# rogerhh/gaussian-splatting-lm

Hardware: AMD Instinct MI355X
Metric: CG matvecs/sec + raster Mpix/s, 1M Gaussians @1080p, 1/2/4/8 GPU (higher is better)
Workload: dtype f32; 1 GPU; LM CG iteration, 1000000 Gaussians SH3, 1x1920x1080 view(s) per GPU (BASELINE configs[2]; configs[3] at 8 GPUs); P=1000000, sh_degree=3, width=1920, height=1080, views_total=1, parallelism=views sharded x1, exchange=none, sh_rest_projected=True

## Files before the change

### gaussian-splatting-lm_amd/csrc/api.hip

```cpp
#include <cstring>
#include <string>
#include "gslm_kernels.hpp"

namespace gslm {

static thread_local std::string g_last_error;
void set_error(const std::string& msg) { g_last_error = msg; }

thread_local DebugSync g_debug;

int launch_failed(hipError_t e, const char* file, int line) {
  const char* base = std::strrchr(file, '/');
  set_error(std::string(g_debug.on ? "kernel failed (debug mode: stream synchronised after the launch at " : "kernel launch (") +
            (base ? base + 1 : file) + ":" + std::to_string(line) + "): " + hipGetErrorString(e));
  return GSLM_ERR_HIP;
}

namespace {

struct Carver {
  char* base;
  size_t off = 0;
  template <typename T>
  T* take(size_t count) {
// ... 600 lines not shown
  if (st) return st;
  if ((st = make_gauss(gi, &b->v, &b->g, false))) return st;
  if (scratch_bytes < gslm_scratch_bytes(b->g.P, N)) {
    set_error("scratch workspace too small");
    return GSLM_ERR_CAPACITY;
  }
  geom_layout(b->g.P, const_cast<void*>(geom), &b->gb);
  bin_layout(N, b->v.gx * b->v.gy, const_cast<void*>(binning), &b->bb);
  img_layout(b->v.H, b->v.W, const_cast<void*>(image), &b->ib);
  scratch_layout(b->g.P, N, scratch, &b->sb);
  return GSLM_OK;
}

int gslm_backward(const gslm_view* view, const gslm_gaussians* gi, const void* geom, const void* binning, int64_t N,
                  const void* image, const float* dL_dcolor, const float* dL_dinvdepth, void* scratch,
                  size_t scratch_bytes, const gslm_grads* out, void* stream) {
  DebugScope dbg_scope(view != nullptr && view->debug != 0, stream);
  Bound b;
  int st = bind_all(view, gi, geom, binning, N, image, scratch, scratch_bytes, &b);
  if (st) return st;
  if (!out || !dL_dcolor) { set_error("backward: NULL dL_dcolor or outputs"); return GSLM_ERR_INVALID; }
  hipStream_t s = (hipStream_t)stream;
  if ((st = launch_render_bwd(b.v, b.gb, b.bb, b.ib, N, dL_dcolor, dL_dinvdepth, b.sb, s))) return st;
  return launch_preprocess_bwd(b.v, b.g, b.gb, b.bb, b.sb, make_gradk(out), true, s);
}

int gslm_jvp(const gslm_view* view, const gslm_gaussians* gi, const gslm_gaussians* tangent,
             const float* means2D_tangent, const void* geom, const void* binning, int64_t N, const void* image,
             void* scratch, size_t scratch_bytes, float* out_color_t, float* out_invdepth_t, void* stream) {
  DebugScope dbg_scope(view != nullptr && view->debug != 0, stream);
  Bound b;
  int st = bind_all(view, gi, geom, binning, N, image, scratch, scratch_bytes, &b);
  if (st) return st;
  if (!out_color_t) { set_error("jvp: NULL out_color_t"); return GSLM_ERR_INVALID; }
  GaussK t;
  if ((st = make_gauss(tangent, &b.v, &t, true))) return st;
  t.P = b.g.P;
  t.raw = b.g.raw;
  t.M = b.g.M;
  return launch_jvp(b.v, b.g, t, means2D_tangent, b.gb, b.bb, b.ib, b.sb, out_color_t, out_invdepth_t,
                    (hipStream_t)stream);
}

static int build_xpby(const gslm_matvec_opts* opts, const gslm_grads* vin, int R, bool mask_xyz, XpbyK* out) {
  const gslm_grads* sv = opts->xpby_s;
  if (!opts->beta_num || !opts->beta_den) {
    set_error("matvec: xpby needs the TANGENT stage and beta_num / beta_den");
    return GSLM_ERR_INVALID;
  }
  if (vin->sh_dc_stride != 3 || sv->sh_dc_stride != 3 || (R > 0 && (vin->sh_rest_stride != R || sv->sh_rest_stride != R))) {
    set_error("matvec: xpby needs contiguous SH groups (dc stride 3, rest stride 3(M-1), or 3 projected)");
    return GSLM_ERR_INVALID;
  }
  XpbyK xp{};
  float* pp[6] = {vin->means3D, vin->sh_dc, vin->sh_rest, vin->scales, vin->rotations, vin->opacities};
  const float* ss[6] = {sv->means3D, sv->sh_dc, sv->sh_rest, sv->scales, sv->rotations, sv->opacities};
  const int ww[6] = {3, 3, R, 3, 4, 1};
  for (int k = 0; k < 6; ++k) {
    if ((pp[k] == nullptr) != (ss[k] == nullptr) || (ww[k] == 0 && pp[k])) {
      set_error("matvec: xpby groups of v and s must match");
      return GSLM_ERR_INVALID;
    }
    xp.p[k] = (ww[k] && !(k == 0 && mask_xyz)) ? pp[k] : nullptr;
    xp.s[k] = ss[k];
    xp.w[k] = ww[k];
  }
  xp.num = opts->beta_num;
  xp.den = opts->beta_den;
  xp.tail_p = opts->xpby_tail_n > 0 ? opts->xpby_tail_v : nullptr;
  xp.tail_s = opts->xpby_tail_s;
  xp.tail_n = opts->xpby_tail_n;
  if (xp.tail_p && !xp.tail_s) { set_error("matvec: xpby tail without s"); return GSLM_ERR_INVALID; }
  xp.anum = opts->alpha_num;
  xp.aden = opts->alpha_den;
  xp.xoff = opts->xpby_x_offset / (int64_t)sizeof(float);
  if (xp.anum && (!xp.aden || opts->xpby_x_offset % (int64_t)sizeof(float) != 0)) {
    set_error("matvec: deferred x update needs alpha_den and a float-aligned xpby_x_offset");
    return GSLM_ERR_INVALID;
  }
  *out = xp;
  return GSLM_OK;
}

static int matvec_view(const gslm_view* view, const gslm_gaussians* gi, const gslm_grads* vin,
                       const float* pixel_weight, int32_t mask_xyz, const void* geom, const void* binning,
                       int64_t N, const void* image, void* scratch, size_t scratch_bytes, const gslm_grads* y,
                       const gslm_matvec_opts* opts, const int32_t* ids, int64_t na, const uint32_t* hrow,
                       void* stream) {
  DebugScope dbg_scope(view != nullptr && view->debug != 0, stream);
  Bound b;
  int st = bind_all(view, gi, geom, binning, N, image, scratch, scratch_bytes, &b);
  if (st) return st;
  if (!vin || !y || !pixel_weight) { set_error("matvec: NULL argument"); return GSLM_ERR_INVALID; }
  const int32_t stages = (opts && opts->stages) ? opts->stages : GSLM_STAGE_ALL;
  const double* damp7 = opts ? opts->damp7 : nullptr;
  double* dot_out = opts ? opts->dot_vy : nullptr;
  const bool active = na >= 0;
  const int64_t rows = active ? na : b.g.P;
  if (active) {
    if (na > b.g.P || (na > 0 && (!ids || !hrow))) {
      set_error("matvec_view_active: 0 <= n_active <= P, a non-NULL list and its row offsets");
      return GSLM_ERR_INVALID;
    }
    if (!mask_xyz || !opts || !(opts->flags & GSLM_MV_TAIL_CLEAN) || (stages & GSLM_STAGE_SCREEN) || opts->trec_in) {
      set_error("matvec_view_active: needs mask_xyz and GSLM_MV_TAIL_CLEAN (the list comes from that row map); "
                "no SCREEN stage, no trec_in");
      return GSLM_ERR_INVALID;
    }
  }
  if (dot_out && (!opts->dot_scratch || opts->dot_scratch_bytes < gslm_dot_scratch_bytes(rows))) {
    set_error("matvec: dot scratch too small");
    return GSLM_ERR_CAPACITY;
  }
  if (!b.g.raw) { set_error("matvec: gaussians must be the raw GaussianModel leaves (raw = 1)"); return GSLM_ERR_INVALID; }
  hipStream_t s = (hipStream_t)stream;
  b.v.stop = opts ? opts->cg_ctl : nullptr;
  if (opts && opts->rest_basis) {
    set_error("matvec: rest_basis is an option of gslm_tangent_views / gslm_gather_screen");
    return GSLM_ERR_INVALID;
  }
  const bool proj = opts && (opts->flags & GSLM_MV_SH_REST_PROJECTED) && b.g.M > 1;
  GaussK t = tangent_from_grads(vin, b.g, mask_xyz != 0);
  if (proj) {
    if (vin->sh_rest && vin->sh_rest_stride != 3) {
      set_error("matvec: a projected SH-rest group has 3 floats per Gaussian (sh_rest_stride 3)");
      return GSLM_ERR_INVALID;
    }
    if (stages & GSLM_STAGE_SCREEN) {
      set_error("matvec: GSLM_MV_SH_REST_PROJECTED is a single-view mode (no SCREEN stage)");
      return GSLM_ERR_INVALID;
    }
    t.rest_proj = 1;
  }
  XpbyK xp{};
  const bool fused_xpby = opts && opts->xpby_s;
  if (fused_xpby) {
    if (!(stages & GSLM_STAGE_TANGENT)) {
      set_error("matvec: xpby needs the TANGENT stage and beta_num / beta_den");
      return GSLM_ERR_INVALID;
    }
    if ((st = build_xpby(opts, vin, proj ? 3 : 3 * (b.g.M - 1), mask_xyz != 0, &xp))) return st;
  }
  if (opts && opts->trec_in) {
    if (stages & GSLM_STAGE_TANGENT) {
      set_error("matvec: trec_in replaces the TANGENT stage");
      return GSLM_ERR_INVALID;
    }
    b.sb.trec = reinterpret_cast<float4*>(const_cast<float*>(opts->trec_in));
  }
  const float* seed = opts ? opts->pixel_seed : nullptr;
  if (seed && (!mask_xyz || fused_xpby || (stages & (GSLM_STAGE_TANGENT | GSLM_STAGE_SCREEN)))) {
    set_error("matvec: pixel_seed (J^T seed) needs mask_xyz and excludes TANGENT / SCREEN / xpby");
    return GSLM_ERR_INVALID;
  }
  if ((stages & GSLM_STAGE_TANGENT) &&
      (st = launch_tangent_pre(b.v, b.g, t, nullptr, b.gb, b.sb, fused_xpby ? &xp : nullptr, s, mask_xyz != 0, ids,
                               na)))
    return st;
  float* jv_out = opts ? opts->jv_out : nullptr;
  if (jv_out) {
    if (seed || (stages & (GSLM_STAGE_GATHER | GSLM_STAGE_SCREEN))) {
      set_error("matvec: jv_out excludes pixel_seed, GATHER and SCREEN");
      return GSLM_ERR_INVALID;
    }
    if (stages & GSLM_STAGE_RENDER) {
      if (N == 0) {
        GSLM_HIP_CHECK(hipMemsetAsync(jv_out, 0, (size_t)3 * b.v.H * b.v.W * sizeof(float), s));
      } else if ((st = launch_render_jv(b.v, t, b.gb, b.bb, b.ib, b.sb, mask_xyz != 0, jv_out, s))) {
        return st;
      }
    }
    return GSLM_OK;
  }
  if (seed) {
    if ((stages & GSLM_STAGE_RENDER) &&
        (st = launch_render_vjp_lm(b.v, b.gb, b.bb, b.ib, N, seed, b.sb, opts->flags & GSLM_MV_TAIL_CLEAN, s)))
      return st;
  } else if ((stages & GSLM_STAGE_RENDER) && N > 0 &&
      (st = launch_matvec_render(b.v, t, b.gb, b.bb, b.ib, b.sb, N, pixel_weight, mask_xyz != 0,
                                 opts && (opts->flags & GSLM_MV_TAIL_CLEAN), s)))
    return st;
  if (stages & GSLM_STAGE_SCREEN) {
    if (!mask_xyz || !opts->screen_out) {
      set_error("matvec: GSLM_STAGE_SCREEN needs mask_xyz and opts->screen_out");
      return GSLM_ERR_INVALID;
    }
    return launch_rowsum_screen(b.g, b.gb, b.sb, opts->screen_out, s);
  }
  if (!(stages & GSLM_STAGE_GATHER)) return GSLM_OK;
  double* part = dot_out ? (double*)opts->dot_scratch : nullptr;
  if ((st = launch_gather_lm(b.v, b.g, b.gb, b.sb, make_gradk(y), make_gradk(vin), damp7,
                             (stages & GSLM_STAGE_OVERWRITE) != 0, mask_xyz != 0, part, s, proj, ids, na, hrow)))
    return st;
  if (dot_out) return gslm_dot_finalize(part, (int32_t)((rows + 255) / 256), dot_out, stream);
  return GSLM_OK;
}

int gslm_matvec_view_ex(const gslm_view* view, const gslm_gaussians* gi, const gslm_grads* vin,
                        const float* pixel_weight, int32_t mask_xyz, const void* geom, const void* binning,
                        int64_t N, const void* image, void* scratch, size_t scratch_bytes, const gslm_grads* y,
                        const gslm_matvec_opts* opts, void* stream) {
  return matvec_view(view, gi, vin, pixel_weight, mask_xyz, geom, binning, N, image, scratch, scratch_bytes, y, opts,
                     nullptr, -1, nullptr, stream);
}

int gslm_matvec_view_active(const gslm_view* view, const gslm_gaussians* gi, const gslm_grads* vin,
                            const float* pixel_weight, int32_t mask_xyz, const void* geom, const void* binning,
                            int64_t N, const void* image, void* scratch, size_t scratch_bytes, const gslm_grads* y,
                            const gslm_matvec_opts* opts, const int32_t* active_ids, const uint32_t* active_rows,
                            int64_t n_active, void* stream) {
  if (n_active < 0) { set_error("matvec_view_active: negative n_active"); return GSLM_ERR_INVALID; }
  return matvec_view(view, gi, vin, pixel_weight, mask_xyz, geom, binning, N, image, scratch, scratch_bytes, y, opts,
                     active_ids, n_active, active_rows, stream);
}

static size_t active_work_layout(int64_t P, void* base, uint32_t** flags, uint32_t** tmp, uint32_t** total) {
  Carver c{(char*)base};
  uint32_t* f = c.take<uint32_t>(P > 0 ? P : 1);
  uint32_t* t = c.take<uint32_t>(scan_tmp_bytes(P > 0 ? P : 1) / 4);
  uint32_t* n = c.take<uint32_t>(4);
  if (flags) { *flags = f; *tmp = t; *total = n; }
  return c.off;
}

size_t gslm_active_list_bytes(int64_t P) { return active_work_layout(P, nullptr, nullptr, nullptr, nullptr); }

int gslm_active_list(const void* geom, int64_t P, int64_t N, const void* scratch, size_t scratch_bytes, void* work,
                     size_t work_bytes, int32_t* ids_dev, uint32_t* rows_dev, int64_t* count_dev, void* stream) {
  if (P < 0 || N < 0 || !geom || !scratch || !work || !count_dev || !rows_dev || (P > 0 && !ids_dev)) {
    set_error("active_list: NULL workspace / output or negative size");
    return GSLM_ERR_INVALID;
  }
  if (scratch_bytes < gslm_scratch_bytes(P, N) || work_bytes < gslm_active_list_bytes(P)) {
    set_error("active_list: scratch or work workspace too small");
    return GSLM_ERR_CAPACITY;
  }
  GeomBufs gb;
  ScratchBufs sb;
  geom_layout(P, const_cast<void*>(geom), &gb);
  scratch_layout(P, N, const_cast<void*>(scratch), &sb);
  uint32_t *flags, *tmp, *total;
  active_work_layout(P, work, &flags, &tmp, &total);
  return launch_active_list(P, N, gb, sb, flags, tmp, total, ids_dev, rows_dev, count_dev, (hipStream_t)stream);
}

int gslm_inspect_rowmap(const void* geom, int64_t P, int64_t N, const void* scratch, size_t scratch_bytes,
                        uint32_t* goff, uint32_t* hscan, void* stream) {
  if (P < 0 || N < 0 || !geom || !scratch) { set_error("inspect_rowmap: NULL workspace or negative size"); return GSLM_ERR_INVALID; }
  if (scratch_bytes < gslm_scratch_bytes(P, N)) { set_error("inspect_rowmap: scratch workspace too small"); return GSLM_ERR_CAPACITY; }
  GeomBufs gb;
  ScratchBufs sb;
  geom_layout(P, const_cast<void*>(geom), &gb);
  scratch_layout(P, N, const_cast<void*>(scratch), &sb);
  hipStream_t s = (hipStream_t)stream;
  if (goff && P > 0) GSLM_HIP_CHECK(hipMemcpyAsync(goff, gb.goff, (size_t)P * 4, hipMemcpyDeviceToDevice, s));
  if (hscan) GSLM_HIP_CHECK(hipMemcpyAsync(hscan, sb.hscan, (size_t)(N + 1) * 4, hipMemcpyDeviceToDevice, s));
  return GSLM_OK;
}

int gslm_active_pack(const float* src, float* dst, const int32_t* active_ids, int64_t n_active, int64_t P,
                     const int32_t* widths, int32_t ngroups, int64_t tail_n, void* stream) {
  return launch_active_pack(true, src, dst, active_ids, n_active, P, widths, ngroups, tail_n, (hipStream_t)stream);
}

int gslm_active_unpack(const float* src, float* dst, const int32_t* active_ids, int64_t n_active, int64_t P,
                       const int32_t* widths, int32_t ngroups, int64_t tail_n, void* stream) {
  return launch_active_pack(false, src, dst, active_ids, n_active, P, widths, ngroups, tail_n, (hipStream_t)stream);
}

int gslm_sh_rest_project(const gslm_view* view, const gslm_gaussians* gi, int32_t mode, const float* in,
                         int64_t in_stride, float* out, int64_t out_stride, void* stream) {
  ViewK v;
  GaussK g;
  int st;
  if (!view || !gi) { set_error("sh_rest_project: NULL view / gaussians"); return GSLM_ERR_INVALID; }
  if ((st = make_view(view, gi->max_coeffs, &v))) return st;
  if ((st = make_gauss(gi, &v, &g, false))) return st;
  if (mode != 0 && mode != 1) { set_error("sh_rest_project: mode must be 0 (expand) or 1 (project)"); return GSLM_ERR_INVALID; }
  if (g.P > 0 && g.M > 1 && (!in || !out || !g.means3D)) { set_error("sh_rest_project: NULL buffer"); return GSLM_ERR_INVALID; }
  const int64_t full = 3 * (int64_t)(g.M - 1);
  if ((mode == 0 && (in_stride < 3 || out_stride < full)) || (mode == 1 && (in_stride < full || out_stride < 3))) {
    set_error("sh_rest_project: strides too small for [P,3] / [P,M-1,3] rows");
    return GSLM_ERR_INVALID;
  }
  return launch_sh_rest_project(v, g, mode, in, in_stride, out, out_stride, (hipStream_t)stream);
}

static int rest_views(const char* who, const gslm_view* views, int32_t nviews, const gslm_gaussians* gi, ViewK* vk,
                      GaussK* g) {
  if (!views || !gi || nviews < 1 || nviews > GSLM_MAX_REST_VIEWS) {
    set_error(std::string(who) + ": NULL views / gaussians or nviews outside 1..GSLM_MAX_REST_VIEWS");
    return GSLM_ERR_INVALID;
  }
  int st;
  for (int b = 0; b < nviews; ++b) {
    if ((st = make_view(&views[b], gi->max_coeffs, &vk[b]))) return st;
// ... 219 lines not shown
```

### gaussian-splatting-lm_amd/csrc/cg.hip

```cpp
#include "gslm_internal.hpp"

namespace gslm {

constexpr int MAXG = 8;
struct Groups {
  int64_t bound[MAXG + 1];
  double damp[MAXG];
  int n;
};

constexpr int DOT_THREADS = 256;
constexpr int DOT_BLOCKS = 1024;

__device__ __forceinline__ double group_w(const Groups& g, int64_t i) {
  double w = 1.0;
  if (g.n > 0) {
    w = 0.0;
#pragma unroll
    for (int k = 0; k < MAXG; ++k)
      if (k < g.n && i >= g.bound[k] && i < g.bound[k + 1]) w = g.damp[k];
  }
  return w;
}

__device__ __forceinline__ double block_sum_d(double x, double* s) {
  const int tid = threadIdx.x, lane = tid & 63, w = tid >> 6;
#pragma unroll
  for (int o = 32; o > 0; o >>= 1) x += __shfl_down(x, o, 64);
  if (lane == 0) s[w] = x;
  __syncthreads();
  double t = 0.0;
  if (tid == 0)
    for (int k = 0; k < DOT_THREADS / 64; ++k) t += s[k];
  return t;
}

__global__ __launch_bounds__(DOT_THREADS) void k_dot_partial(const float* __restrict__ a, const float* __restrict__ b,
                                                             Groups g, int64_t n, double* __restrict__ part) {
  __shared__ double s[DOT_THREADS / 64];
  double acc = 0.0;
  const int64_t stride = (int64_t)gridDim.x * DOT_THREADS;
  if (g.n == 0) {
    for (int64_t i = (int64_t)blockIdx.x * DOT_THREADS + threadIdx.x; i < n; i += stride)
      acc += (double)a[i] * (double)b[i];
  } else {
    for (int k = 0; k < g.n; ++k) {
      double gacc = 0.0;
      const int64_t lo = g.bound[k], hi = min(g.bound[k + 1], n);
      for (int64_t i = lo + (int64_t)blockIdx.x * DOT_THREADS + threadIdx.x; i < hi; i += stride)
        gacc += (double)a[i] * (double)b[i];
      acc += g.damp[k] * gacc;
    }
  }
  const double t = block_sum_d(acc, s);
  if (threadIdx.x == 0) part[blockIdx.x] = t;
}

__global__ __launch_bounds__(DOT_THREADS) void k_dot_final(const double* __restrict__ part, int np,
                                                           double* __restrict__ out) {
  __shared__ double s[DOT_THREADS / 64];
  const double acc = strided_sum_in_order(part, np);
  const double t = block_sum_d(acc, s);
  if (threadIdx.x == 0) *out = t;
}

__global__ __launch_bounds__(DOT_THREADS) void k_dot_final3(const double* __restrict__ part, int np,
                                                            double* __restrict__ o0, double* __restrict__ o1,
                                                            double* __restrict__ o2) {
  __shared__ double s[DOT_THREADS / 64];
  const int b = blockIdx.x;
  const double acc = strided_sum_in_order(part + (int64_t)b * np, np);
  const double t = block_sum_d(acc, s);
  if (threadIdx.x == 0) *(b == 0 ? o0 : (b == 1 ? o1 : o2)) = t;
}

__global__ __launch_bounds__(256) void k_axpy_dev(int64_t n, const double* __restrict__ num,
                                                  const double* __restrict__ den, float sign,
                                                  const float* __restrict__ x, float* __restrict__ y) {
  const double a = den ? (*num) / (*den) : (*num);
  const float af = (float)(a * (double)sign);
  const int64_t stride = (int64_t)gridDim.x * blockDim.x;
  for (int64_t i = (int64_t)blockIdx.x * blockDim.x + threadIdx.x; i < n; i += stride) y[i] = y[i] + af * x[i];
}

__global__ __launch_bounds__(256) void k_xpby_dev(int64_t n, const float* __restrict__ s, const double* __restrict__ num,
                                                  const double* __restrict__ den, float* __restrict__ p) {
  const float b = (float)((*num) / (*den));
  const int64_t stride = (int64_t)gridDim.x * blockDim.x;
  for (int64_t i = (int64_t)blockIdx.x * blockDim.x + threadIdx.x; i < n; i += stride) p[i] = s[i] + b * p[i];
}

template <bool MONITOR>
__global__ __launch_bounds__(DOT_THREADS) void k_cg_update(int64_t n, const double* __restrict__ gam,
                                                           const double* __restrict__ del,
                                                           const float* __restrict__ p, const float* __restrict__ q,
                                                           float* __restrict__ x, float* __restrict__ s,
                                                           const float* __restrict__ g, double* __restrict__ part,
                                                           const double* __restrict__ ctl) {
  __shared__ double sm[DOT_THREADS / 64];
  if (ctl && (ctl[0] != 0.0 || *del < 1e-20 || !isfinite(*del))) return;
  const float a = (float)((*gam) / (*del));
  double acc = 0.0, axg = 0.0, axs = 0.0;
  const int64_t n4 = n / 4;
  const int64_t stride = (int64_t)gridDim.x * DOT_THREADS;
  const float4* p4 = reinterpret_cast<const float4*>(p);
  const float4* q4 = reinterpret_cast<const float4*>(q);
  const float4* g4 = reinterpret_cast<const float4*>(g);
  float4* x4 = reinterpret_cast<float4*>(x);
  float4* s4 = reinterpret_cast<float4*>(s);
  const bool do_x = x != nullptr;
  for (int64_t i = (int64_t)blockIdx.x * DOT_THREADS + threadIdx.x; i < n4; i += stride) {
    const float4 qv = q4[i];
    float4 xv = make_float4(0.f, 0.f, 0.f, 0.f), sv = s4[i];
    float4 gv;
    if (MONITOR) gv = g4[i];
    if (do_x) {
      const float4 pv = p4[i];
      xv = x4[i];
      xv.x += a * pv.x; xv.y += a * pv.y; xv.z += a * pv.z; xv.w += a * pv.w;
      x4[i] = xv;
    }
    sv.x -= a * qv.x; sv.y -= a * qv.y; sv.z -= a * qv.z; sv.w -= a * qv.w;
    s4[i] = sv;
    acc += (double)sv.x * sv.x + (double)sv.y * sv.y + (double)sv.z * sv.z + (double)sv.w * sv.w;
    if (MONITOR) {
      axg += (double)xv.x * gv.x + (double)xv.y * gv.y + (double)xv.z * gv.z + (double)xv.w * gv.w;
      axs += (double)xv.x * sv.x + (double)xv.y * sv.y + (double)xv.z * sv.z + (double)xv.w * sv.w;
    }
  }
  for (int64_t i = 4 * n4 + (int64_t)blockIdx.x * DOT_THREADS + threadIdx.x; i < n; i += stride) {
    float xv = 0.f;
    if (do_x) {
      xv = x[i] + a * p[i];
      x[i] = xv;
    }
    const float sv = s[i] - a * q[i];
    s[i] = sv;
    acc += (double)sv * sv;
    if (MONITOR) {
      axg += (double)xv * g[i];
      axs += (double)xv * sv;
    }
  }
  const double t = block_sum_d(acc, sm);
  if (threadIdx.x == 0) part[blockIdx.x] = t;
  if (MONITOR) {
    __syncthreads();
    const double t1 = block_sum_d(axg, sm);
    if (threadIdx.x == 0) part[gridDim.x + blockIdx.x] = t1;
    __syncthreads();
    const double t2 = block_sum_d(axs, sm);
    if (threadIdx.x == 0) part[2 * gridDim.x + blockIdx.x] = t2;
  }
}

__global__ void k_cg_monitor(const double* __restrict__ gam, const double* __restrict__ gamn,
                             const double* __restrict__ del, const double* __restrict__ xg,
                             const double* __restrict__ xs, const double* __restrict__ b2, double tol, double atol,
                             double* __restrict__ ctl, int max_hist) {
  if (threadIdx.x != 0 || ctl[0] != 0.0) return;
  if (!(isfinite(*gam) && isfinite(*del))) {
    ctl[0] = 4.0;
    return;
  }
  if (*del < 1e-20) {
    ctl[0] = 1.0;
    return;
  }
  if (!(isfinite(*gamn) && isfinite(*xg) && isfinite(*xs))) {
    ctl[0] = 4.0;
    return;
  }
  const double res = (*b2 - *xg) - *xs;
  const int nh = (int)ctl[3];
  if (nh < max_hist) ctl[4 + nh] = res;
  ctl[3] = (double)(nh + 1);
  if (res > ctl[2]) {
    ctl[0] = 2.0;
    return;
  }
  ctl[2] = res;
  if (*gamn < fmax(tol * sqrt(*gam), atol)) {
    ctl[0] = 3.0;
    return;
  }
  ctl[1] += 1.0;
}

__global__ __launch_bounds__(256) void k_damp_add(int64_t n, const float* __restrict__ x, Groups g,
                                                  float* __restrict__ y) {
  const int64_t stride = (int64_t)gridDim.x * blockDim.x;
  for (int64_t i = (int64_t)blockIdx.x * blockDim.x + threadIdx.x; i < n; i += stride)
    y[i] = y[i] + (float)group_w(g, i) * x[i];
}

static int make_groups(const int64_t* bounds, const double* damp, int ng, Groups* g) {
  if (ng < 0 || ng > MAXG) {
    set_error("at most 8 damping groups");
    return GSLM_ERR_INVALID;
  }
  g->n = ng;
  for (int k = 0; k <= MAXG; ++k) g->bound[k] = (k <= ng && bounds) ? bounds[k] : 0;
  for (int k = 0; k < MAXG; ++k) g->damp[k] = (k < ng && damp) ? damp[k] : 0.0;
  return GSLM_OK;
}

static unsigned grid_for(int64_t n) {
  int64_t b = (n + 255) / 256;
  if (b > 4096) b = 4096;
  if (b < 1) b = 1;
  return (unsigned)b;
}

}

using namespace gslm;

extern "C" {

size_t gslm_dot_scratch_bytes(int64_t n) {
  const int64_t per_block = (n + 255) / 256 + 16;
  return (size_t)(per_block > DOT_BLOCKS ? per_block : DOT_BLOCKS) * sizeof(double);
}

int gslm_cg_update(int64_t n, const double* gam_dev, const double* del_dev, const float* p, const float* q, float* x,
                   float* s, void* scratch, double* gam_new_dev, void* stream) {
  if ((reinterpret_cast<uintptr_t>(p) | reinterpret_cast<uintptr_t>(q) | reinterpret_cast<uintptr_t>(x) |
       reinterpret_cast<uintptr_t>(s)) & 15) {
    set_error("gslm_cg_update: vectors must be 16-byte aligned");
    return GSLM_ERR_INVALID;
  }
  hipStream_t st = (hipStream_t)stream;
  hipLaunchKernelGGL(k_cg_update<false>, dim3(DOT_BLOCKS), dim3(DOT_THREADS), 0, st, n, gam_dev, del_dev, p, q, x, s,
                     nullptr, (double*)scratch, (const double*)nullptr);
  hipLaunchKernelGGL(k_dot_final, dim3(1), dim3(DOT_THREADS), 0, st, (const double*)scratch, DOT_BLOCKS, gam_new_dev);
  GSLM_LAUNCH_CHECK();
  return GSLM_OK;
}

int gslm_cg_update_monitor(int64_t n, const double* gam_dev, const double* del_dev, const float* p, const float* q,
                           float* x, float* s, const float* g, void* scratch, size_t scratch_bytes,
                           double* gam_new_dev, double* xg_dev, double* xs_dev, const double* cg_ctl, void* stream) {
  if ((reinterpret_cast<uintptr_t>(p) | reinterpret_cast<uintptr_t>(q) | reinterpret_cast<uintptr_t>(x) |
       reinterpret_cast<uintptr_t>(s) | reinterpret_cast<uintptr_t>(g)) & 15) {
    set_error("gslm_cg_update_monitor: vectors must be 16-byte aligned");
    return GSLM_ERR_INVALID;
  }
  if (scratch_bytes < (size_t)3 * DOT_BLOCKS * sizeof(double)) {
    set_error("gslm_cg_update_monitor: scratch < 3 * 1024 doubles");
    return GSLM_ERR_CAPACITY;
  }
  hipStream_t st = (hipStream_t)stream;
  const double* part = (const double*)scratch;
  hipLaunchKernelGGL(k_cg_update<true>, dim3(DOT_BLOCKS), dim3(DOT_THREADS), 0, st, n, gam_dev, del_dev, p, q, x, s, g,
                     (double*)scratch, cg_ctl);
  hipLaunchKernelGGL(k_dot_final3, dim3(3), dim3(DOT_THREADS), 0, st, part, DOT_BLOCKS, gam_new_dev, xg_dev, xs_dev);
  GSLM_LAUNCH_CHECK();
  return GSLM_OK;
}

int gslm_cg_monitor(const double* gam_dev, const double* gam_new_dev, const double* del_dev, const double* xg_dev,
                    const double* xs_dev, const double* b2_dev, double tol, double atol, double* cg_ctl,
                    int32_t max_hist, void* stream) {
  if (!gam_dev || !gam_new_dev || !del_dev || !xg_dev || !xs_dev || !b2_dev || !cg_ctl || max_hist < 0) {
    set_error("gslm_cg_monitor: NULL scalar / control block or negative max_hist");
    return GSLM_ERR_INVALID;
  }
  hipLaunchKernelGGL(k_cg_monitor, dim3(1), dim3(64), 0, (hipStream_t)stream, gam_dev, gam_new_dev, del_dev, xg_dev,
                     xs_dev, b2_dev, tol, atol, cg_ctl, max_hist);
  GSLM_LAUNCH_CHECK();
  return GSLM_OK;
}

int gslm_dot_finalize(const void* partials, int32_t np, double* out_dev, void* stream) {
  hipLaunchKernelGGL(k_dot_final, dim3(1), dim3(DOT_THREADS), 0, (hipStream_t)stream, (const double*)partials, np,
                     out_dev);
  GSLM_LAUNCH_CHECK();
  return GSLM_OK;
}

int gslm_dot(const float* a, const float* b, const int64_t* group_bounds, const double* group_damp, int32_t ngroups,
             int64_t n, void* scratch, double* out_dev, void* stream) {
  Groups g;
  int st = make_groups(group_bounds, group_damp, ngroups, &g);
  if (st) return st;
  hipStream_t s = (hipStream_t)stream;
  hipLaunchKernelGGL(k_dot_partial, dim3(DOT_BLOCKS), dim3(DOT_THREADS), 0, s, a, b, g, n, (double*)scratch);
  hipLaunchKernelGGL(k_dot_final, dim3(1), dim3(DOT_THREADS), 0, s, (const double*)scratch, DOT_BLOCKS, out_dev);
  GSLM_LAUNCH_CHECK();
  return GSLM_OK;
}

int gslm_axpy_dev(int64_t n, const double* num_dev, const double* den_dev, float sign, const float* x, float* y,
                  void* stream) {
  if (n <= 0) return GSLM_OK;
  hipLaunchKernelGGL(k_axpy_dev, dim3(grid_for(n)), dim3(256), 0, (hipStream_t)stream, n, num_dev, den_dev, sign, x, y);
  GSLM_LAUNCH_CHECK();
  return GSLM_OK;
}

int gslm_xpby_dev(int64_t n, const float* s_, const double* num_dev, const double* den_dev, float* p, void* stream) {
  if (n <= 0) return GSLM_OK;
  hipLaunchKernelGGL(k_xpby_dev, dim3(grid_for(n)), dim3(256), 0, (hipStream_t)stream, n, s_, num_dev, den_dev, p);
  GSLM_LAUNCH_CHECK();
  return GSLM_OK;
}

int gslm_damp_add(int64_t n, const float* x, const int64_t* group_bounds, const double* group_damp, int32_t ngroups,
                  float* y, void* stream) {
  Groups g;
  int st = make_groups(group_bounds, group_damp, ngroups, &g);
  if (st) return st;
  if (n <= 0) return GSLM_OK;
  hipLaunchKernelGGL(k_damp_add, dim3(grid_for(n)), dim3(256), 0, (hipStream_t)stream, n, x, g, y);
  GSLM_LAUNCH_CHECK();
  return GSLM_OK;
}

}
```

### gaussian-splatting-lm_amd/csrc/gather.hip

```cpp
#include "gslm_tile.hpp"
#include "gslm_chain.hpp"
#include "gslm_gather.hpp"

namespace gslm {

template <int ROWF4>
__device__ __forceinline__ void sum_rows(const float4* __restrict__ rows, uint32_t off, uint32_t n, float G2[NV]) {
#pragma unroll
  for (int q = 0; q < NV; ++q) G2[q] = 0.f;
  for (uint32_t t = 0; t < n; ++t) {
    float r[NV];
    load_row<ROWF4>(rows, (size_t)off + t, r);
#pragma unroll
    for (int q = 0; q < NV; ++q) G2[q] += r[q];
  }
}

template <bool RAW>
__global__ __launch_bounds__(256) void k_preprocess_bwd(ViewK v, GaussK g, const uint32_t* __restrict__ clampw,
                                                         const uint32_t* __restrict__ tiles,
                                                         const uint32_t* __restrict__ goff,
                                                         const float4* __restrict__ rows, GradK out, int want_means) {
  extern __shared__ __attribute__((aligned(16))) float s_buf[];
  const int tid = threadIdx.x;
  const int64_t i0 = (int64_t)blockIdx.x * blockDim.x;
  const int64_t i = i0 + tid;
  const int64_t nvalid = min((int64_t)blockDim.x, g.P - i0);
  const uint32_t n = i < g.P ? tiles[i] : 0u;
  float G2[NV];
  {
    const int64_t il = i0 + nvalid - 1;
    const uint32_t R0 = goff[i0], R1 = goff[il] + tiles[il];
    block_sum_rows<3>(rows, R0, R1, i < g.P ? goff[i] : R1, n, reinterpret_cast<float4*>(s_buf), G2);
  }
  const int nc = (v.D + 1) * (v.D + 1);
  const bool sh_out = !g.colors && (out.dc || out.rest);
  const bool dir_term = want_means && out.means3D && !g.colors && v.D > 0;
  ChainOut co;
  if (i < g.P) {
    chain_vjp<RAW, true>(v, g, i, n != 0, n ? clampw[i] : 0u, G2, want_means != 0, co);
    write_grads(g, out, i, co, v.M, nc, want_means != 0 && !dir_term, true);
  }
  if (!sh_out && !dir_term) return;
  float* s_d = s_buf + 256 * SHB_STRIDE;
  float* s_w = s_d + 256 * 4;
  if (i < g.P) {
#pragma unroll
    for (int k = 0; k < 16; ++k) s_buf[tid * SHB_STRIDE + k] = co.shB[k];
#pragma unroll
    for (int ch = 0; ch < 3; ++ch) s_d[tid * 4 + ch] = co.dres[ch];
  }
  __syncthreads();
  if (dir_term) {
    for (int e = tid; e < (int)nvalid * 16; e += blockDim.x) {
      const int ii = e >> 4, k = e & 15;
      float w = 0.f;
      if (k >= 1 && k < nc) {
        const int64_t gi = i0 + ii;
        const float s0 = g.sh(gi, k, 0), s1 = g.sh(gi, k, 1), s2 = g.sh(gi, k, 2);
        w = s_d[ii * 4 + 0] * s0 + s_d[ii * 4 + 1] * s1 + s_d[ii * 4 + 2] * s2;
      }
      s_w[ii * SHB_STRIDE + k] = w;
    }
    __syncthreads();
    if (i < g.P && n != 0) {
      float dm[3] = {co.dmean[0], co.dmean[1], co.dmean[2]};
      add_dir_term(v.D, co.dir, co.dirlen, s_w + tid * SHB_STRIDE, dm);
#pragma unroll
      for (int k = 0; k < 3; ++k) put(&out.means3D[3 * i + k], dm[k], out.accumulate);
    } else if (i < g.P) {
#pragma unroll
      for (int k = 0; k < 3; ++k) put(&out.means3D[3 * i + k], co.dmean[k], out.accumulate);
    }
  }
  if (!sh_out) return;
  const int acc = out.accumulate;
  const int R = 3 * v.M;
  const float invR = 1.0f / (float)R;
  for (int e = tid; e < (int)nvalid * R; e += blockDim.x) {
    const int ii = (int)(((float)e + 0.5f) * invR);
    const int r = e - ii * R, k = r / 3, ch = r - 3 * k;
    const float val = k < nc ? s_buf[ii * SHB_STRIDE + k] * s_d[ii * 4 + ch] : 0.f;
    const int64_t gi = i0 + ii;
    if (k == 0) {
      if (out.dc) put(&out.dc[gi * out.dc_stride + ch], val, acc);
    } else if (out.rest) {
      put(&out.rest[gi * out.rest_stride + 3 * (k - 1) + ch], val, acc);
    }
  }
}

template <bool WANT_MEANS, int ROWF4, bool PROJ, bool ACTIVE = false>
__global__ __launch_bounds__(256, PROJ ? 5 : 1) void k_gather_lm(ViewK v, GaussK g, const uint32_t* __restrict__ clampw,
                                                    const uint32_t* __restrict__ tiles,
                                                    const uint32_t* __restrict__ goff,
                                                    const uint32_t* __restrict__ hscan,
                                                    const float4* __restrict__ rows, FlatK o,
                                                    const int32_t* __restrict__ ids, int64_t na,
                                                    const uint32_t* __restrict__ hrow) {
  o.rest_proj = PROJ ? 1 : 0;
  if (cg_stopped(v)) return;
  extern __shared__ __attribute__((aligned(16))) float s_rest[];
  __shared__ double s_dot[4];
  const int tid = threadIdx.x;
  const int64_t j0 = (int64_t)blockIdx.x * blockDim.x;
  const int64_t j = j0 + tid;
  const int64_t nrows = ACTIVE ? na : g.P;
  const int64_t nvalid = min((int64_t)blockDim.x, nrows - j0);
  const bool valid = j < nrows;
  const int64_t i = ACTIVE ? (valid ? (int64_t)ids[j] : 0) : j;
  const uint32_t n = ACTIVE ? (valid ? 1u : 0u) : (valid ? tiles[i] : 0u);
  float G2[NV];
  if (ACTIVE) {
    const uint32_t R0 = hrow[j0], R1 = hrow[j0 + nvalid];
    const uint32_t h0 = valid ? hrow[j] : R1, h1 = valid ? hrow[j + 1] : R1;
    block_sum_rows<ROWF4>(rows, R0, R1, h0, h1 - h0, reinterpret_cast<float4*>(s_rest), G2);
  } else {
    const int64_t il = j0 + nvalid - 1;
    const uint32_t R0 = hscan[goff[j0]], R1 = hscan[goff[il] + tiles[il]];
    const uint32_t h0 = valid ? hscan[goff[i]] : R1, h1 = valid ? hscan[goff[i] + n] : R1;
    block_sum_rows<ROWF4>(rows, R0, R1, h0, h1 - h0, reinterpret_cast<float4*>(s_rest), G2);
  }
  ChainOut co;
  if (valid) chain_vjp<true>(v, g, i, n != 0, n ? clampw[i] : 0u, G2, WANT_MEANS, co);
  if (ACTIVE) g.P = na;
  lm_epilogue<WANT_MEANS, true>((v.D + 1) * (v.D + 1), g, co, o, s_rest, s_dot);
}

__global__ __launch_bounds__(256) void k_sh_rest_project(ViewK v, GaussK g, int mode, const float* __restrict__ in,
                                                         int64_t in_stride, float* __restrict__ out,
                                                         int64_t out_stride) {
  extern __shared__ __attribute__((aligned(16))) float s_rows[];
  const int R = 3 * (g.M - 1);
  const int64_t i0 = (int64_t)blockIdx.x * blockDim.x;
  const int64_t nv = min((int64_t)blockDim.x, g.P - i0);
  const int64_t i = i0 + threadIdx.x;
  if (mode == 1) {
    for (int64_t e = threadIdx.x; e < nv * R; e += blockDim.x) {
      const int64_t ii = e / R, r = e - ii * R;
      s_rows[e] = in[(i0 + ii) * in_stride + r];
    }
    __syncthreads();
  }
  if (i < g.P) {
    const float x = g.means3D[3 * i + 0], y = g.means3D[3 * i + 1], z = g.means3D[3 * i + 2];
    const float dx = x - v.campos[0], dy = y - v.campos[1], dz = z - v.campos[2];
    const float len = sqrtf((dx * dx + dy * dy) + dz * dz);
    float B[16];
    sh_basis(v.D, dx / len, dy / len, dz / len, B);
    const int nc = (v.D + 1) * (v.D + 1);
    const float nb = sh_rest_norm(B, nc);
    const float inv = nb > 0.f ? 1.f / nb : 0.f;
    float* row = s_rows + (int64_t)threadIdx.x * R;
    if (mode == 0) {
      for (int k = 1; k < g.M; ++k)
#pragma unroll
        for (int c = 0; c < 3; ++c) row[3 * (k - 1) + c] = k < nc ? (B[k] * inv) * in[i * in_stride + c] : 0.f;
    } else {
      float acc[3] = {0.f, 0.f, 0.f};
      for (int k = 1; k < g.M && k < nc; ++k)
#pragma unroll
        for (int c = 0; c < 3; ++c) acc[c] += (B[k] * inv) * row[3 * (k - 1) + c];
#pragma unroll
      for (int c = 0; c < 3; ++c) out[i * out_stride + c] = acc[c];
    }
  }
  if (mode == 0) {
    __syncthreads();
    for (int64_t e = threadIdx.x; e < nv * R; e += blockDim.x) {
      const int64_t ii = e / R, r = e - ii * R;
      out[(i0 + ii) * out_stride + r] = s_rows[e];
    }
  }
}

int launch_sh_rest_project(const ViewK& v, const GaussK& g, int mode, const float* in, int64_t in_stride, float* out,
                           int64_t out_stride, hipStream_t s) {
  if (g.P == 0 || g.M < 2) return GSLM_OK;
  const size_t lds = (size_t)256 * 3 * (g.M - 1) * sizeof(float);
  hipLaunchKernelGGL(k_sh_rest_project, dim3((unsigned)((g.P + 255) / 256)), dim3(256), lds, s, v, g, mode, in,
                     in_stride, out, out_stride);
  GSLM_LAUNCH_CHECK();
  return GSLM_OK;
}

int launch_preprocess_bwd(const ViewK& v, const GaussK& g, const GeomBufs& gb, const BinBufs& bb,
                          const ScratchBufs& sb, const GradK& out, bool want_means, hipStream_t s) {
  (void)bb;
  if (g.P == 0) return GSLM_OK;
  const unsigned nb = (unsigned)((g.P + 255) / 256);
  const size_t sh_lds = (sh_stage_floats<true>(g.M) + (size_t)256 * SHB_STRIDE) * sizeof(float);
  const size_t chunk_lds = (size_t)GATHER_CHUNK * 3 * sizeof(float4);
  const size_t lds = sh_lds > chunk_lds ? sh_lds : chunk_lds;
  if (g.raw)
    hipLaunchKernelGGL(k_preprocess_bwd<true>, dim3(nb), dim3(256), lds, s, v, g, gb.clampw, gb.tiles, gb.goff,
                       sb.contrib, out, want_means ? 1 : 0);
  else
    hipLaunchKernelGGL(k_preprocess_bwd<false>, dim3(nb), dim3(256), lds, s, v, g, gb.clampw, gb.tiles, gb.goff,
                       sb.contrib, out, want_means ? 1 : 0);
  GSLM_LAUNCH_CHECK();
  return GSLM_OK;
}

int launch_gather_lm(const ViewK& v, const GaussK& g, const GeomBufs& gb, const ScratchBufs& sb, const GradK& y,
                     const GradK& vin, const double* damp7, bool overwrite, bool mask_xyz, double* dot_part,
                     hipStream_t s, bool rest_proj, const int32_t* ids, int64_t na, const uint32_t* hrow) {
  const bool active = na >= 0;
  const int64_t nrows = active ? na : g.P;
  if (nrows == 0) return GSLM_OK;
  FlatK o;
  const int st = make_flatk(g, y, vin, damp7, overwrite, dot_part, &o, rest_proj);
  if (st) return st;
  if (active && (!mask_xyz || !ids || !hrow)) {
    set_error("internal: the active-list gather runs on the LM rows (mask_xyz)");
    return GSLM_ERR_INVALID;
  }
  const unsigned nb = (unsigned)((nrows + 255) / 256);
  const size_t rest_lds = sh_stage_floats<true>(g.M) * sizeof(float);
  const size_t chunk_lds = (size_t)GATHER_CHUNK * (mask_xyz ? 2 : 3) * sizeof(float4);
  const size_t lds = (rest_lds > chunk_lds ? rest_lds : chunk_lds) + 16;
  if (active && o.rest_proj)
    hipLaunchKernelGGL((k_gather_lm<false, 2, true, true>), dim3(nb), dim3(256), lds, s, v, g, gb.clampw, gb.tiles,
                       gb.goff, sb.hscan, sb.contrib, o, ids, na, hrow);
  else if (active)
    hipLaunchKernelGGL((k_gather_lm<false, 2, false, true>), dim3(nb), dim3(256), lds, s, v, g, gb.clampw, gb.tiles,
                       gb.goff, sb.hscan, sb.contrib, o, ids, na, hrow);
  else if (mask_xyz && o.rest_proj)
    hipLaunchKernelGGL((k_gather_lm<false, 2, true>), dim3(nb), dim3(256), lds, s, v, g, gb.clampw, gb.tiles, gb.goff,
                       sb.hscan, sb.contrib, o, nullptr, -1, nullptr);
  else if (mask_xyz)
    hipLaunchKernelGGL((k_gather_lm<false, 2, false>), dim3(nb), dim3(256), lds, s, v, g, gb.clampw, gb.tiles, gb.goff,
                       sb.hscan, sb.contrib, o, nullptr, -1, nullptr);
  else if (o.rest_proj)
    hipLaunchKernelGGL((k_gather_lm<true, 3, true>), dim3(nb), dim3(256), lds, s, v, g, gb.clampw, gb.tiles, gb.goff,
                       sb.hscan, sb.contrib, o, nullptr, -1, nullptr);
  else
    hipLaunchKernelGGL((k_gather_lm<true, 3, false>), dim3(nb), dim3(256), lds, s, v, g, gb.clampw, gb.tiles, gb.goff,
                       sb.hscan, sb.contrib, o, nullptr, -1, nullptr);
  GSLM_LAUNCH_CHECK();
  return GSLM_OK;
}

struct PackK {
  int w[8];
  int64_t poff[8];
  int64_t aoff[8];
  int n;
  int wsum;
};
template <bool TO_ACTIVE>
__global__ __launch_bounds__(256) void k_active_pack(PackK k, const int32_t* __restrict__ ids, int64_t na,
                                                      const float* __restrict__ src, float* __restrict__ dst) {
  const int64_t e = (int64_t)blockIdx.x * blockDim.x + threadIdx.x;
  if (e >= na * k.wsum) return;
  const int64_t j = e / k.wsum;
  int c = (int)(e - j * k.wsum), grp = 0;
  while (grp < k.n - 1 && c >= k.w[grp]) c -= k.w[grp++];
  const int64_t full = k.poff[grp] + (int64_t)ids[j] * k.w[grp] + c;
  const int64_t act = k.aoff[grp] + j * k.w[grp] + c;
  if (TO_ACTIVE) dst[act] = src[full];
  else dst[full] = src[act];
}

int launch_active_pack(bool to_active, const float* src, float* dst, const int32_t* ids, int64_t na, int64_t P,
                       const int32_t* widths, int ngroups, int64_t tail_n, hipStream_t s) {
  if (ngroups < 1 || ngroups > 8 || !widths || na < 0 || na > P || tail_n < 0 || !src || !dst || (na > 0 && !ids)) {
    set_error("active pack: 1..8 groups, 0 <= n_active <= P, non-NULL buffers");
    return GSLM_ERR_INVALID;
  }
  PackK k{};
  int64_t po = 0, ao = 0;
  for (int q = 0; q < ngroups; ++q) {
    if (widths[q] < 0) { set_error("active pack: negative group width"); return GSLM_ERR_INVALID; }
    k.w[q] = widths[q];
    k.poff[q] = po;
    k.aoff[q] = ao;
    po += P * widths[q];
    ao += na * widths[q];
    k.wsum += widths[q];
  }
  k.n = ngroups;
  const int64_t src_n = to_active ? po : ao, dst_n = to_active ? ao : po;
  if (!to_active) GSLM_HIP_CHECK(hipMemsetAsync(dst, 0, (size_t)dst_n * sizeof(float), s));
  if (tail_n > 0)
    GSLM_HIP_CHECK(hipMemcpyAsync(dst + dst_n, src + src_n, (size_t)tail_n * sizeof(float), hipMemcpyDeviceToDevice, s));
  const int64_t total = na * k.wsum;
  if (total == 0) return GSLM_OK;
  const unsigned nb = (unsigned)((total + 255) / 256);
  if (to_active) hipLaunchKernelGGL(k_active_pack<true>, dim3(nb), dim3(256), 0, s, k, ids, na, src, dst);
  else hipLaunchKernelGGL(k_active_pack<false>, dim3(nb), dim3(256), 0, s, k, ids, na, src, dst);
  GSLM_LAUNCH_CHECK();
  return GSLM_OK;
}

}
```

### gaussian-splatting-lm_amd/csrc/gslm_device.hpp

```cpp
#pragma once
#include <hip/hip_runtime.h>
#include <stdint.h>
#include "gslm.h"

#if defined(GSLM_EXPERIMENT_COUNT) || defined(GSLM_EXPERIMENT_TIMELINE) || defined(GSLM_EXPERIMENT_SKIP_JVP) || \
    defined(GSLM_EXPERIMENT_SKIP_VJP) || defined(GSLM_EXPERIMENT_NOSYNC)
#error "GSLM_EXPERIMENT_* flags are not part of the product build (libgslm.so)"
#endif

namespace gslm {

constexpr int TILE_X = 16;
constexpr int TILE_Y = 16;
constexpr int TILE_PIX = TILE_X * TILE_Y;
constexpr int REC_F4 = 3;
constexpr int RECS = 4;

__constant__ static const float SH_C0 = 0.28209479177387814f;
__constant__ static const float SH_C1 = 0.4886025119029199f;

struct f3 { float x, y, z; };
__device__ __forceinline__ f3 mk3(float x, float y, float z) { return {x, y, z}; }

struct ViewK {
  int H, W, gx, gy;
  float focal_x, focal_y, limx, limy;
  float view[16];
  float proj[16];
  float campos[3];
  float bg[3];
  float scale_mod;
  int D;
  int M;
  int antialiasing;
  int exhaustive;
  const double* stop = nullptr;
};

template <typename F>
__device__ __forceinline__ F strided_sum_in_order(const F* __restrict__ x, int64_t n) {
  F acc = F(0);
  const int64_t T = blockDim.x;
  for (int64_t i = threadIdx.x; i < n; i += 8 * T) {
    F v[8];
#pragma unroll
    for (int k = 0; k < 8; ++k) v[k] = i + k * T < n ? x[i + k * T] : F(0);
#pragma unroll
    for (int k = 0; k < 8; ++k)
      if (i + k * T < n) acc += v[k];
  }
  return acc;
}

__device__ __forceinline__ float clamp01(float x) { return x < 0.0f ? 0.0f : (x > 1.0f ? 1.0f : x); }

__device__ __forceinline__ bool cg_stopped(const ViewK& v) { return v.stop != nullptr && *v.stop != 0.0; }

__device__ __forceinline__ float tp_row(const float* m, float x, float y, float z, int r) {
  return ((x * m[r] + y * m[4 + r]) + z * m[8 + r]) + m[12 + r];
}

__device__ __forceinline__ void quat_rot(float r, float x, float y, float z, float R[9]) {
  R[0] = 1.f - 2.f * (y * y + z * z); R[1] = 2.f * (x * y - r * z); R[2] = 2.f * (x * z + r * y);
  R[3] = 2.f * (x * y + r * z); R[4] = 1.f - 2.f * (x * x + z * z); R[5] = 2.f * (y * z - r * x);
  R[6] = 2.f * (x * z - r * y); R[7] = 2.f * (y * z + r * x); R[8] = 1.f - 2.f * (x * x + y * y);
}

__device__ __forceinline__ void cov3d_from(float sx, float sy, float sz, const float R[9], float c[6]) {
  const float s[3] = {sx, sy, sz};
  float L[9];
#pragma unroll
  for (int i = 0; i < 3; ++i)
#pragma unroll
    for (int j = 0; j < 3; ++j) L[i * 3 + j] = R[i * 3 + j] * s[j];
  auto dotrow = [&](int a, int b) { return (L[a * 3 + 0] * L[b * 3 + 0] + L[a * 3 + 1] * L[b * 3 + 1]) + L[a * 3 + 2] * L[b * 3 + 2]; };
  c[0] = dotrow(0, 0); c[1] = dotrow(0, 1); c[2] = dotrow(0, 2);
  c[3] = dotrow(1, 1); c[4] = dotrow(1, 2); c[5] = dotrow(2, 2);
}

struct Proj2 {
  float A0[3], A1[3];
  float J00, J02, J11, J12;
  float tz, tcx, tcy;
  bool inx, iny;
};

__device__ __forceinline__ void ewa_jacobian(const ViewK& v, float tx, float ty, float tz, Proj2& p) {
  const float txtz = tx / tz, tytz = ty / tz;
  p.inx = (txtz >= -v.limx) && (txtz <= v.limx);
  p.iny = (tytz >= -v.limy) && (tytz <= v.limy);
  p.tcx = fminf(v.limx, fmaxf(-v.limx, txtz)) * tz;
  p.tcy = fminf(v.limy, fmaxf(-v.limy, tytz)) * tz;
  p.tz = tz;
  p.J00 = v.focal_x / tz;
  p.J02 = -(v.focal_x * p.tcx) / (tz * tz);
  p.J11 = v.focal_y / tz;
  p.J12 = -(v.focal_y * p.tcy) / (tz * tz);
#pragma unroll
  for (int k = 0; k < 3; ++k) {
    p.A0[k] = p.J00 * v.view[4 * k + 0] + p.J02 * v.view[4 * k + 2];
    p.A1[k] = p.J11 * v.view[4 * k + 1] + p.J12 * v.view[4 * k + 2];
  }
}

__device__ __forceinline__ float quad_form(const float a[3], const float c[6], const float b[3]) {
  const float S0[3] = {c[0], c[1], c[2]}, S1[3] = {c[1], c[3], c[4]}, S2[3] = {c[2], c[4], c[5]};
  const float r0 = (S0[0] * b[0] + S0[1] * b[1]) + S0[2] * b[2];
  const float r1 = (S1[0] * b[0] + S1[1] * b[1]) + S1[2] * b[2];
  const float r2 = (S2[0] * b[0] + S2[1] * b[1]) + S2[2] * b[2];
  return (a[0] * r0 + a[1] * r1) + a[2] * r2;
}

__device__ __forceinline__ void sh_basis(int D, float x, float y, float z, float B[16]) {
  B[0] = SH_C0;
  if (D > 0) { B[1] = -SH_C1 * y; B[2] = SH_C1 * z; B[3] = -SH_C1 * x; }
  if (D > 1) {
    const float xx = x * x, yy = y * y, zz = z * z, xy = x * y, yz = y * z, xz = x * z;
    B[4] = 1.0925484305920792f * xy;
    B[5] = -1.0925484305920792f * yz;
    B[6] = 0.31539156525252005f * (2.0f * zz - xx - yy);
    B[7] = -1.0925484305920792f * xz;
    B[8] = 0.5462742152960396f * (xx - yy);
    if (D > 2) {
      B[9] = -0.5900435899266435f * y * (3.0f * xx - yy);
      B[10] = 2.890611442640554f * xy * z;
      B[11] = -0.4570457994644658f * y * (4.0f * zz - xx - yy);
      B[12] = 0.3731763325901154f * z * (2.0f * zz - 3.0f * xx - 3.0f * yy);
      B[13] = -0.4570457994644658f * x * (4.0f * zz - xx - yy);
      B[14] = 1.445305721320277f * z * (xx - yy);
      B[15] = -0.5900435899266435f * x * (xx - 3.0f * yy);
    }
  }
}

// ... 74 lines not shown
```

### gaussian-splatting-lm_amd/csrc/gslm_internal.hpp

```cpp
#pragma once
#include <hip/hip_runtime.h>
#include <stdint.h>
#include <stddef.h>
#include <string>
#include "gslm.h"
#include "gslm_device.hpp"

namespace gslm {

void set_error(const std::string& msg);

#define GSLM_HIP_CHECK(expr)                                                                  \
  do {                                                                                        \
    hipError_t _e = (expr);                                                                   \
    if (_e != hipSuccess) {                                                                   \
      ::gslm::set_error(std::string(#expr) + ": " + hipGetErrorString(_e));                   \
      return GSLM_ERR_HIP;                                                                    \
    }                                                                                         \
  } while (0)

struct DebugSync {
  hipStream_t s = nullptr;
  bool on = false;
};
extern thread_local DebugSync g_debug;
struct DebugScope {
  DebugSync prev;
  DebugScope(bool on, void* stream) : prev(g_debug) {
    if (on) g_debug = DebugSync{(hipStream_t)stream, true};
  }
  ~DebugScope() { g_debug = prev; }
};
int launch_failed(hipError_t e, const char* file, int line);

#define GSLM_LAUNCH_CHECK()                                                                   \
  do {                                                                                        \
    hipError_t _e = hipGetLastError();                                                        \
    if (_e == hipSuccess && ::gslm::g_debug.on) _e = hipStreamSynchronize(::gslm::g_debug.s);  \
    if (_e != hipSuccess) return ::gslm::launch_failed(_e, __FILE__, __LINE__);               \
  } while (0)

inline size_t align_up(size_t x, size_t a = 256) { return (x + a - 1) / a * a; }

constexpr int SORT_THREADS = 256;
constexpr int SORT_ITEMS = 16;
constexpr int SORT_TILE = SORT_THREADS * SORT_ITEMS;
#ifndef GSLM_SORT_ITEMS_SMALL
#define GSLM_SORT_ITEMS_SMALL 8
#endif
constexpr int SORT_ITEMS_SMALL = GSLM_SORT_ITEMS_SMALL;
constexpr int64_t SORT_FULL_BLOCKS = 1024;
constexpr int RADIX = 256;

inline int sort_items(int64_t n, bool payload = false) {
  return !payload && (n + SORT_TILE - 1) / SORT_TILE >= SORT_FULL_BLOCKS ? SORT_ITEMS : SORT_ITEMS_SMALL;
}
inline int64_t sort_blocks(int64_t n, bool payload = false) {
  const int64_t t = (int64_t)SORT_THREADS * sort_items(n, payload);
  return (n + t - 1) / t;
}
inline size_t sort_hist_bytes(int64_t n, bool payload = false) {
  const size_t nb = (size_t)sort_blocks(n, payload);
  return (size_t)RADIX * nb * 4 + 4 * RADIX + 16 + 8 * nb;
}

int radix_sort_pairs(uint32_t* k0, uint32_t* v0, uint32_t* k1, uint32_t* v1, int64_t n, int end_bit,
                     uint32_t* hist, bool* result_in_alt, hipStream_t s, bool iota_values = false,
                     const uint32_t* last_gather = nullptr, const uint32_t* n_dev = nullptr, uint32_t* p0 = nullptr,
                     uint32_t* p1 = nullptr, bool key_range = false);

constexpr int SCAN_THREADS = 256;
#ifndef GSLM_SCAN_ITEMS
#define GSLM_SCAN_ITEMS 8
#endif
constexpr int SCAN_ITEMS = GSLM_SCAN_ITEMS;
constexpr int SCAN_TILE = SCAN_THREADS * SCAN_ITEMS;
inline int64_t scan_blocks(int64_t n) { return (n + SCAN_TILE - 1) / SCAN_TILE; }
#ifndef GSLM_SCAN_INLINE_MAX_BLOCKS
#define GSLM_SCAN_INLINE_MAX_BLOCKS 4096
#endif
constexpr int64_t SCAN_INLINE_MAX_BLOCKS = GSLM_SCAN_INLINE_MAX_BLOCKS;
inline size_t scan_tmp_bytes(int64_t n) { return align_up((size_t)scan_blocks(n) * 8 + 64); }
int exclusive_scan_u32(const uint32_t* in, const uint32_t* idx, uint32_t* out, int64_t n, uint32_t* tmp,
                       uint32_t* total, hipStream_t s, int64_t inline_max_blocks = SCAN_INLINE_MAX_BLOCKS);
int exclusive_scan_u32_dual(const uint32_t* in, const uint32_t* idx, uint32_t* out_a, uint32_t* out_b, int64_t n,
                            uint32_t* tmp, uint32_t* total_a, uint32_t* total_b, hipStream_t s,
                            const uint32_t* in_b = nullptr, int64_t inline_max_blocks = SCAN_INLINE_MAX_BLOCKS);

}
```

### gaussian-splatting-lm_amd/csrc/gslm_kernels.hpp

```cpp
#pragma once
#include "gslm_internal.hpp"

namespace gslm {

struct GaussK {
  int64_t P;
  int raw;
  int M;
  const float* means3D;
  const float* opac;
  const float* scales;
  const float* rot;
  const float* cov3D;
  const float* dc;
  int64_t dc_stride;
  const float* rest;
  int64_t rest_stride;
  const float* colors;
  int64_t rest_base = 0;
  int rest_proj = 0;
  const float* rest_R = nullptr;
  int rest_V = 0;
  int rest_col = 0;
  __device__ __forceinline__ float sh(int64_t i, int k, int c) const {
// ... 365 lines not shown
constexpr int MAX_PRE_VIEWS = 8;
struct PreOutBufs {
  float4* rec;
  uint32_t* depth_key;
  uint32_t* tiles;
  uint2* rect;
  uint32_t* clampw;
  const uint32_t* pos;
};
struct PreViewsK {
  ViewK v[MAX_PRE_VIEWS];
  PreOutBufs out[MAX_PRE_VIEWS];
  int n;
};
int launch_preprocess_views(const PreViewsK& pv, const GaussK& g, const GeomBufs* gbs, hipStream_t s);
int launch_binning(const ViewK& v, int64_t P, const GeomBufs& gb, const BinBufs& bb, int64_t N, hipStream_t s,
                   bool device_count = false, uint32_t* n_out = nullptr);
int launch_ranges(int64_t N, const uint32_t* keys_sorted, uint2* ranges, const uint32_t* n_dev, uint32_t* n_out,
                  hipStream_t s);
constexpr int TILE_ORDER_FLAT = 0, TILE_ORDER_XCD = 1;
int launch_tile_order_form(int form, int ntiles, const uint2* ranges, uint32_t* order, const uint32_t* cost,
                           hipStream_t s);
int launch_lm_rowmap(const ViewK& v, const GeomBufs& gb, const BinBufs& bb, const ImgBufs& ib, const ScratchBufs& sb,
                     int64_t N, hipStream_t s);
int launch_active_list(int64_t P, int64_t N, const GeomBufs& gb, const ScratchBufs& sb, uint32_t* flags,
                       uint32_t* scan_tmp, uint32_t* total, int32_t* ids, uint32_t* hrow, int64_t* count,
                       hipStream_t s);
int launch_point_ids(const uint32_t* point_list, int64_t N, uint32_t* out, hipStream_t s);
int launch_render_loss(const ViewK& v, const GeomBufs& gb, const BinBufs& bb, const float* gt, const float* mask,
                       double* part, double* loss, int accumulate, hipStream_t s, const uint32_t* amask = nullptr,
                       int shift = 0, const uint32_t* nsets = nullptr);
constexpr int MAX_UNION_SETS = 8;
struct UnionSets {
  const float4* rec[MAX_UNION_SETS];
  const uint32_t* tiles[MAX_UNION_SETS];
  const uint2* rect[MAX_UNION_SETS];
  int n;
};
struct UnionMasks {
  uint32_t* m0;
  uint32_t* m1;
  uint32_t* sorted;
  uint32_t* hist;
  uint32_t* nsets;
};
size_t union_masks_layout(int64_t N, int ntiles, void* binning, UnionMasks* out);
struct SetRecsK {
  const float4* rec[MAX_UNION_SETS];
};
struct LossPtrsK {
  double* loss[MAX_UNION_SETS];
};
int launch_render_loss_sets(const ViewK& v, const SetRecsK& sr, int nsets, const BinBufs& bb, const uint32_t* amask,
                            const float* gt, const float* mask, double* part, const LossPtrsK& lp, int accumulate,
                            hipStream_t s, int first_set = 0, const uint32_t* nsets_dev = nullptr);
int launch_union_rect(int64_t P, const UnionSets& u, const GeomBufs& ug, hipStream_t s);
int launch_depth_positions(int64_t P, const uint32_t* order, uint32_t* pos, hipStream_t s);
int launch_union_binning(const ViewK& v, int64_t P, const GeomBufs& ug, const BinBufs& bb, const UnionMasks& um,
                         int64_t N, const UnionSets& u, hipStream_t s);
int launch_render_fwd(const ViewK& v, const GeomBufs& gb, const BinBufs& bb, const ImgBufs& ib, float* out_color,
                      float* out_invdepth, hipStream_t s);

}

namespace gslm {
int launch_render_bwd(const ViewK& v, const GeomBufs& gb, const BinBufs& bb, const ImgBufs& ib, int64_t N,
                      const float* dL_dcolor, const float* dL_dinv, const ScratchBufs& sb, hipStream_t s);
int launch_render_vjp_lm(const ViewK& v, const GeomBufs& gb, const BinBufs& bb, const ImgBufs& ib, int64_t N,
                         const float* dL_dcolor, const ScratchBufs& sb, bool tail_clean, hipStream_t s);
int launch_preprocess_bwd(const ViewK& v, const GaussK& g, const GeomBufs& gb, const BinBufs& bb,
                          const ScratchBufs& sb, const GradK& out, bool want_means, hipStream_t s);
struct XpbyK {
  float* p[6];
  const float* s[6];
  int w[6];
  const double* num;
  const double* den;
  float* tail_p;
  const float* tail_s;
  int64_t tail_n;
  const double* anum;
  const double* aden;
  int64_t xoff;
};
int launch_tangent_pre(const ViewK& v, const GaussK& g, const GaussK& t, const float* m2t, const GeomBufs& gb,
                       const ScratchBufs& sb, const XpbyK* xp, hipStream_t s, bool compact,
                       const int32_t* ids = nullptr, int64_t na = -1);
int launch_rowsum_screen(const GaussK& g, const GeomBufs& gb, const ScratchBufs& sb, float* out, hipStream_t s);
constexpr int MAX_SCREEN_VIEWS = 16;
constexpr int MAX_REST_VIEWS = GSLM_MAX_REST_VIEWS;
__host__ __device__ constexpr int rest_basis_floats(int V) { return V * (V + 1) / 2; }
struct RestK {
  const float* R = nullptr;
  int V = 0;
  int view_base = 0;
};
struct ViewsK {
  ViewK v[MAX_SCREEN_VIEWS];
  int n;
};
int launch_gather_screen(const ViewK* views, int nviews, const GaussK& g, const float* screen, int64_t sstride,
                         const GradK& y, const GradK& vin, const double* damp7, bool overwrite, double* dot_part,
                         hipStream_t s, const RestK& rc = RestK{});
int launch_gather_views(const ViewK* views, const GeomBufs* gbs, const ScratchBufs* sbs, const int64_t* nr,
                        int nviews, const GaussK& g, const GradK& y, const GradK& vin, const double* damp7,
                        bool overwrite, double* dot_part, double* dot_out, hipStream_t s, const RestK& rc = RestK{});
int launch_rest_basis(const ViewK* views, int nviews, const GaussK& g, float* R, hipStream_t s);
int launch_rest_coords(const ViewK* views, int nviews, const GaussK& g, const float* R, int mode, const float* in,
                       int64_t in_stride, float* out, int64_t out_stride, hipStream_t s);
int launch_view_flags(int64_t P, const GeomBufs& gb, uint32_t* out, hipStream_t s);
int launch_tangent_views(const ViewK* views, int nviews, const GaussK& g, const GaussK& t, const uint32_t* vflags,
                         int64_t fstride, float* out, int64_t ostride, const XpbyK* xp, hipStream_t s, bool compact,
                         int view_base = 0);
int launch_jvp(const ViewK& v, const GaussK& g, const GaussK& t, const float* m2t, const GeomBufs& gb,
               const BinBufs& bb, const ImgBufs& ib, const ScratchBufs& sb, float* out_color_t, float* out_inv_t,
               hipStream_t s);
int launch_render_jv(const ViewK& v, const GaussK& t, const GeomBufs& gb, const BinBufs& bb, const ImgBufs& ib,
                     const ScratchBufs& sb, bool mask_xyz, float* jv_out, hipStream_t s);
int launch_matvec_render(const ViewK& v, const GaussK& t, const GeomBufs& gb, const BinBufs& bb, const ImgBufs& ib,
                         const ScratchBufs& sb, int64_t N, const float* weight, bool mask_xyz, bool tail_clean,
                         hipStream_t s);
int launch_gather_lm(const ViewK& v, const GaussK& g, const GeomBufs& gb, const ScratchBufs& sb, const GradK& y,
                     const GradK& vin, const double* damp7, bool overwrite, bool mask_xyz, double* dot_part,
                     hipStream_t s, bool rest_proj = false, const int32_t* ids = nullptr, int64_t na = -1,
                     const uint32_t* hrow = nullptr);
int launch_active_pack(bool to_active, const float* src, float* dst, const int32_t* ids, int64_t na, int64_t P,
                       const int32_t* widths, int ngroups, int64_t tail_n, hipStream_t s);
int launch_sh_rest_project(const ViewK& v, const GaussK& g, int mode, const float* in, int64_t in_stride, float* out,
                           int64_t out_stride, hipStream_t s);
}
```

### gaussian-splatting-lm_amd/csrc/tangent.hip

```cpp
#include "gslm_tile.hpp"
#include "gslm_chain.hpp"

namespace gslm {

__device__ __forceinline__ void block_xpby(const XpbyK& xp, int64_t P, float* s_rest) {
  const float b = (float)((*xp.num) / (*xp.den));
  const bool with_x = xp.anum != nullptr;
  const float a = with_x ? (float)((*xp.anum) / (*xp.aden)) : 0.f;
  const int64_t i0 = (int64_t)blockIdx.x * blockDim.x;
  const int64_t nv = min((int64_t)blockDim.x, P - i0);
  const int tid = threadIdx.x;
  constexpr int MAXW[6] = {3, 3, 3, 3, 4, 1};
  const bool rest_narrow = xp.w[2] <= 3;
  float sv[17], pv[17], xv[17];
  int n = 0;
#pragma unroll
  for (int k = 0; k < 6; ++k) {
#pragma unroll
    for (int j = 0; j < MAXW[k]; ++j, ++n) {
      const int64_t e = (int64_t)j * blockDim.x + tid;
      const bool on = xp.p[k] && (k != 2 || rest_narrow) && e < nv * xp.w[k];
      const int64_t gi = i0 * xp.w[k] + e;
      sv[n] = on ? xp.s[k][gi] : 0.f;
      pv[n] = on ? xp.p[k][gi] : 0.f;
      xv[n] = (on && with_x) ? xp.p[k][xp.xoff + gi] : 0.f;
    }
  }
  n = 0;
#pragma unroll
  for (int k = 0; k < 6; ++k) {
#pragma unroll
    for (int j = 0; j < MAXW[k]; ++j, ++n) {
      const int64_t e = (int64_t)j * blockDim.x + tid;
      const bool on = xp.p[k] && (k != 2 || rest_narrow) && e < nv * xp.w[k];
      if (on) {
        const int64_t gi = i0 * xp.w[k] + e;
        if (with_x) xp.p[k][xp.xoff + gi] = xv[n] + a * pv[n];
        const float r = sv[n] + b * pv[n];
        xp.p[k][gi] = r;
        if (k == 2) s_rest[e] = r;
      }
    }
  }
  if (xp.p[2] && !rest_narrow) {
    float* p = xp.p[2] + i0 * xp.w[2];
    const float* s = xp.s[2] + i0 * xp.w[2];
    const int64_t len = nv * xp.w[2];
    constexpr int U = 8;
    for (int64_t e0 = 0; e0 < len; e0 += (int64_t)U * blockDim.x) {
      float su[U], pu[U], xu[U];
#pragma unroll
      for (int u = 0; u < U; ++u) {
        const int64_t e = e0 + (int64_t)u * blockDim.x + tid;
        su[u] = e < len ? s[e] : 0.f;
        pu[u] = e < len ? p[e] : 0.f;
        xu[u] = (e < len && with_x) ? p[xp.xoff + e] : 0.f;
      }
#pragma unroll
      for (int u = 0; u < U; ++u) {
        const int64_t e = e0 + (int64_t)u * blockDim.x + tid;
        if (e < len) {
          if (with_x) p[xp.xoff + e] = xu[u] + a * pu[u];
          const float r = su[u] + b * pu[u];
          p[e] = r;
          s_rest[e] = r;
        }
      }
    }
  }
  if (blockIdx.x == 0 && xp.tail_p)
    for (int64_t e = threadIdx.x; e < xp.tail_n; e += blockDim.x) {
      const float pvt = xp.tail_p[e];
      if (with_x) xp.tail_p[xp.xoff + e] = xp.tail_p[xp.xoff + e] + a * pvt;
      xp.tail_p[e] = xp.tail_s[e] + b * pvt;
    }
}

__device__ __forceinline__ void store_trec(float4* __restrict__ out, int64_t i, const float T2[10], bool compact) {
  if (compact) {
    out[2 * i + 0] = make_float4(T2[2], T2[3], T2[4], T2[5]);
    out[2 * i + 1] = make_float4(T2[6], T2[7], T2[8], 0.f);
  } else {
    out[3 * i + 0] = make_float4(T2[0], T2[1], T2[2], T2[3]);
    out[3 * i + 1] = make_float4(T2[4], T2[5], T2[6], T2[7]);
    out[3 * i + 2] = make_float4(T2[8], T2[9], 0.f, 0.f);
  }
}

template <bool RAW, bool XPBY, bool ACTIVE = false>
__global__ __launch_bounds__(256) void k_preprocess_jvp(ViewK v, GaussK g, GaussK t, const float* __restrict__ m2t,
                                                         const uint32_t* __restrict__ clampw,
                                                         const uint32_t* __restrict__ tiles,
                                                         float4* __restrict__ trec, XpbyK xp, int compact,
                                                         int lead, const int32_t* __restrict__ ids, int64_t na) {
  extern __shared__ __attribute__((aligned(16))) float s_rest[];
  if (cg_stopped(v)) return;
  const int64_t j = (int64_t)blockIdx.x * blockDim.x + threadIdx.x;
  const int64_t n = ACTIVE ? na : g.P;
  if (!XPBY && !ACTIVE && lead >= 0) {
    stage_sh_rows(g, lead, s_rest);
  }
  if (XPBY) {
    block_xpby(xp, n, s_rest);
    __syncthreads();
    if (t.rest) {
      t.rest = s_rest;
      t.rest_base = (int64_t)blockIdx.x * blockDim.x;
    }
  }
  if (j >= n) return;
  const int64_t i = ACTIVE ? (int64_t)ids[j] : j;
  if (!ACTIVE && tiles[i] == 0) return;
  float T2[10];
  chain_jvp<RAW>(v, g, t, m2t, i, j, clampw[i], T2);
  store_trec(trec, i, T2, compact != 0);
}

int launch_tangent_pre(const ViewK& v, const GaussK& g, const GaussK& t, const float* m2t, const GeomBufs& gb,
                       const ScratchBufs& sb, const XpbyK* xp, hipStream_t s, bool compact, const int32_t* ids,
                       int64_t na) {
  const bool active = na >= 0;
  const int64_t n = active ? na : g.P;
  if (n == 0 && !(xp && xp->tail_p)) return GSLM_OK;
  const unsigned nb = (unsigned)((n + 255) / 256) + (n == 0 ? 1u : 0u);
  XpbyK none{};
  const XpbyK& x = xp ? *xp : none;
  if (active && (!g.raw || m2t || (na > 0 && !ids))) {
    set_error("internal: the active-list tangent runs on raw leaves without a means2D tangent");
    return GSLM_ERR_INVALID;
  }
  if (xp) {
    if (t.rest && (t.rest != xp->p[2] || t.rest_stride != xp->w[2])) {
      set_error("internal: fused xpby expects the tangent's SH-rest group to be p's");
      return GSLM_ERR_INVALID;
    }
    const size_t lds = (size_t)256 * xp->w[2] * sizeof(float);
    if (active)
      hipLaunchKernelGGL((k_preprocess_jvp<true, true, true>), dim3(nb), dim3(256), lds, s, v, g, t, m2t, gb.clampw,
                         gb.tiles, sb.trec, x, compact ? 1 : 0, -1, ids, na);
    else if (g.raw)
      hipLaunchKernelGGL((k_preprocess_jvp<true, true>), dim3(nb), dim3(256), lds, s, v, g, t, m2t, gb.clampw, gb.tiles,
                         sb.trec, x, compact ? 1 : 0, -1, nullptr, -1);
    else
      hipLaunchKernelGGL((k_preprocess_jvp<false, true>), dim3(nb), dim3(256), lds, s, v, g, t, m2t, gb.clampw, gb.tiles,
                         sb.trec, x, compact ? 1 : 0, -1, nullptr, -1);
  } else if (active) {
    hipLaunchKernelGGL((k_preprocess_jvp<true, false, true>), dim3(nb), dim3(256), 0, s, v, g, t, m2t, gb.clampw,
                       gb.tiles, sb.trec, x, compact ? 1 : 0, -1, ids, na);
  } else {
    const int lead = g.P > 0 ? stage_lead(g) : -1;
    const size_t lds = lead >= 0 ? (size_t)256 * g.rest_stride * sizeof(float) : 0;
    if (g.raw)
      hipLaunchKernelGGL((k_preprocess_jvp<true, false>), dim3(nb), dim3(256), lds, s, v, g, t, m2t, gb.clampw, gb.tiles,
                         sb.trec, x, compact ? 1 : 0, lead, nullptr, -1);
    else
      hipLaunchKernelGGL((k_preprocess_jvp<false, false>), dim3(nb), dim3(256), lds, s, v, g, t, m2t, gb.clampw, gb.tiles,
                         sb.trec, x, compact ? 1 : 0, lead, nullptr, -1);
  }
  GSLM_LAUNCH_CHECK();
  return GSLM_OK;
}

template <bool XPBY>
__global__ __launch_bounds__(256) void k_tangent_views(ViewsK vs, GaussK g, GaussK t, const uint32_t* __restrict__ vflags,
                                                        int64_t fstride, float4* __restrict__ out, int64_t ostride,
                                                        XpbyK xp, int compact, int view_base) {
  extern __shared__ __attribute__((aligned(16))) float s_rest[];
  if (cg_stopped(vs.v[0])) return;
  const int64_t i0 = (int64_t)blockIdx.x * blockDim.x;
  const int64_t i = i0 + threadIdx.x;
  if (XPBY) {
    block_xpby(xp, g.P, s_rest);
  } else if (t.rest) {
    const int64_t len = min((int64_t)blockDim.x, g.P - i0) * t.rest_stride;
    const float* src = t.rest + i0 * t.rest_stride;
    for (int64_t e = threadIdx.x; e < len; e += blockDim.x) s_rest[e] = src[e];
  }
  __syncthreads();
  if (t.rest) {
    t.rest = s_rest;
    t.rest_base = i0;
  }
  if (i >= g.P) return;
#pragma unroll 1
  for (int b = 0; b < vs.n; ++b) {
    const uint32_t f = vflags[(int64_t)b * fstride + i];
    if (!(f >> 31)) continue;
    t.rest_col = view_base + b;
    float T2[10];
    chain_jvp<true>(vs.v[b], g, t, nullptr, i, i, f & 7u, T2);
    store_trec(out, (int64_t)b * ostride + i, T2, compact != 0);
  }
}

int launch_tangent_views(const ViewK* views, int nviews, const GaussK& g, const GaussK& t, const uint32_t* vflags,
                         int64_t fstride, float* out, int64_t ostride, const XpbyK* xp, hipStream_t s, bool compact,
                         int view_base) {
  if (nviews < 1 || nviews > MAX_SCREEN_VIEWS) {
    set_error("tangent_views: 1..16 views per call");
    return GSLM_ERR_INVALID;
  }
  if (g.P == 0 && !(xp && xp->tail_p)) return GSLM_OK;
  if (xp && t.rest && (t.rest != xp->p[2] || t.rest_stride != xp->w[2])) {
    set_error("internal: fused xpby expects the tangent's SH-rest group to be p's");
    return GSLM_ERR_INVALID;
  }
  ViewsK vs;
  for (int b = 0; b < nviews; ++b) vs.v[b] = views[b];
  vs.n = nviews;
  const unsigned nb = (unsigned)((g.P + 255) / 256) + (g.P == 0 ? 1u : 0u);
  const size_t lds = t.rest ? (size_t)256 * t.rest_stride * sizeof(float) : 0;
  XpbyK none{};
  float4* o = reinterpret_cast<float4*>(out);
  if (xp)
    hipLaunchKernelGGL(k_tangent_views<true>, dim3(nb), dim3(256), lds, s, vs, g, t, vflags, fstride, o, ostride, *xp,
                       compact ? 1 : 0, view_base);
  else
    hipLaunchKernelGGL(k_tangent_views<false>, dim3(nb), dim3(256), lds, s, vs, g, t, vflags, fstride, o, ostride, none,
                       compact ? 1 : 0, view_base);
  GSLM_LAUNCH_CHECK();
  return GSLM_OK;
}

}
```

### gaussian-splatting-lm_amd/gslm/_lib.py

```python
import ctypes
import math
import os

import torch

_HERE = os.path.dirname(os.path.abspath(__file__))
_DEFAULT_LIB = os.path.join(os.path.dirname(_HERE), "build", "libgslm.so")
LIB_PATH = os.environ.get("GSLM_LIB", _DEFAULT_LIB)

GSLM_OK = 0
GSLM_ERR_INVALID = -1
GSLM_ERR_HIP = -2
GSLM_ERR_CAPACITY = -3
GSLM_MAX_REST_VIEWS = 8


class GslmView(ctypes.Structure):
    _fields_ = [
        ("image_height", ctypes.c_int32), ("image_width", ctypes.c_int32),
        ("tanfovx", ctypes.c_double), ("tanfovy", ctypes.c_double), ("scale_modifier", ctypes.c_double),
        ("viewmatrix", ctypes.c_float * 16), ("projmatrix", ctypes.c_float * 16),
        ("campos", ctypes.c_float * 3), ("bg", ctypes.c_float * 3),
        ("sh_degree", ctypes.c_int32), ("prefiltered", ctypes.c_int32),
        ("antialiasing", ctypes.c_int32), ("debug", ctypes.c_int32),
    ]


class GslmGaussians(ctypes.Structure):
    _fields_ = [
        ("P", ctypes.c_int64), ("max_coeffs", ctypes.c_int32), ("raw", ctypes.c_int32),
        ("means3D", ctypes.c_void_p), ("opacities", ctypes.c_void_p), ("scales", ctypes.c_void_p),
        ("rotations", ctypes.c_void_p), ("cov3D_precomp", ctypes.c_void_p),
        ("sh_dc", ctypes.c_void_p), ("sh_dc_stride", ctypes.c_int64),
        ("sh_rest", ctypes.c_void_p), ("sh_rest_stride", ctypes.c_int64),
        ("colors_precomp", ctypes.c_void_p),
    ]


class GslmGrads(ctypes.Structure):
    _fields_ = [
        ("means2D", ctypes.c_void_p), ("means3D", ctypes.c_void_p), ("opacities", ctypes.c_void_p),
        ("scales", ctypes.c_void_p), ("rotations", ctypes.c_void_p), ("cov3D", ctypes.c_void_p),
        ("sh_dc", ctypes.c_void_p), ("sh_dc_stride", ctypes.c_int64),
        ("sh_rest", ctypes.c_void_p), ("sh_rest_stride", ctypes.c_int64),
        ("colors", ctypes.c_void_p), ("accumulate", ctypes.c_int32),
    ]


class GslmMatvecOpts(ctypes.Structure):
    _fields_ = [
        ("stages", ctypes.c_int32), ("flags", ctypes.c_int32),
        ("damp7", ctypes.POINTER(ctypes.c_double)), ("dot_vy", ctypes.c_void_p),
        ("dot_scratch", ctypes.c_void_p), ("dot_scratch_bytes", ctypes.c_size_t),
        ("xpby_s", ctypes.c_void_p), ("beta_num", ctypes.c_void_p), ("beta_den", ctypes.c_void_p),
        ("xpby_tail_v", ctypes.c_void_p), ("xpby_tail_s", ctypes.c_void_p), ("xpby_tail_n", ctypes.c_int64),
        ("screen_out", ctypes.c_void_p), ("pixel_seed", ctypes.c_void_p), ("jv_out", ctypes.c_void_p),
        ("alpha_num", ctypes.c_void_p), ("alpha_den", ctypes.c_void_p), ("xpby_x_offset", ctypes.c_int64),
        ("trec_in", ctypes.c_void_p), ("screen_stride", ctypes.c_int64),
        ("cg_ctl", ctypes.c_void_p),
        ("rest_basis", ctypes.c_void_p), ("rest_views", ctypes.c_int32), ("view_base", ctypes.c_int32),
    ]


class GslmViewWs(ctypes.Structure):
    _fields_ = [
        ("geom", ctypes.c_void_p), ("scratch", ctypes.c_void_p), ("scratch_bytes", ctypes.c_size_t),
        ("num_rendered", ctypes.c_int64),
    ]


class GslmAdamGroup(ctypes.Structure):
    _fields_ = [
        ("param", ctypes.c_void_p), ("grad", ctypes.c_void_p), ("exp_avg", ctypes.c_void_p),
        ("exp_avg_sq", ctypes.c_void_p), ("n", ctypes.c_int64), ("floats_per_gaussian", ctypes.c_int32),
        ("_pad", ctypes.c_int32), ("lr", ctypes.c_double), ("step", ctypes.c_int64),
    ]


ADAM_MAX_GROUPS = 8


EXPORTS = {
    "gslm_geom_bytes": (ctypes.c_size_t, [ctypes.c_int64]),
    "gslm_image_bytes": (ctypes.c_size_t, [ctypes.c_int32, ctypes.c_int32]),
    "gslm_binning_bytes": (ctypes.c_size_t, [ctypes.c_int64, ctypes.c_int32, ctypes.c_int32]),
    "gslm_scratch_bytes": (ctypes.c_size_t, [ctypes.c_int64, ctypes.c_int64]),
    "gslm_preprocess": (ctypes.c_int, [ctypes.POINTER(GslmView), ctypes.POINTER(GslmGaussians), ctypes.c_void_p,
                                       ctypes.c_size_t, ctypes.c_void_p, ctypes.c_void_p]),
    "gslm_num_rendered": (ctypes.c_int, [ctypes.c_void_p, ctypes.c_int64, ctypes.POINTER(ctypes.c_int64),
                                         ctypes.c_void_p]),
    "gslm_preprocess_ordered": (ctypes.c_int, [ctypes.POINTER(GslmView), ctypes.POINTER(GslmGaussians),
                                               ctypes.c_void_p, ctypes.c_size_t, ctypes.c_void_p, ctypes.c_void_p,
                                               ctypes.c_int32, ctypes.c_void_p]),
    "gslm_preprocess_views": (ctypes.c_int, [ctypes.POINTER(GslmView), ctypes.c_int32, ctypes.POINTER(GslmGaussians),
                                             ctypes.POINTER(ctypes.c_void_p), ctypes.c_size_t,
                                             ctypes.POINTER(ctypes.c_void_p), ctypes.c_void_p]),
    "gslm_depth_positions": (ctypes.c_int, [ctypes.c_void_p, ctypes.c_int64, ctypes.c_void_p, ctypes.c_void_p]),
    "gslm_num_rendered_many": (ctypes.c_int, [ctypes.POINTER(ctypes.c_void_p), ctypes.POINTER(ctypes.c_int64),
                                              ctypes.c_int32, ctypes.POINTER(ctypes.c_int64), ctypes.c_void_p]),
    "gslm_rasterize": (ctypes.c_int, [ctypes.POINTER(GslmView), ctypes.c_int64, ctypes.c_void_p, ctypes.c_void_p,
                                      ctypes.c_size_t, ctypes.c_int64, ctypes.c_void_p, ctypes.c_size_t,
                                      ctypes.c_void_p, ctypes.c_void_p, ctypes.c_void_p]),
    "gslm_loss_scratch_bytes": (ctypes.c_size_t, [ctypes.c_int32, ctypes.c_int32]),
    "gslm_rasterize_loss": (ctypes.c_int, [ctypes.POINTER(GslmView), ctypes.c_int64, ctypes.c_void_p, ctypes.c_void_p,
                                           ctypes.c_size_t, ctypes.c_int64, ctypes.c_void_p, ctypes.c_void_p,
                                           ctypes.c_void_p, ctypes.c_size_t, ctypes.c_void_p, ctypes.c_int32,
                                           ctypes.c_void_p]),
    "gslm_binning_capacity": (ctypes.c_int64, [ctypes.c_size_t, ctypes.c_int32, ctypes.c_int32]),
    "gslm_rasterize_dev": (ctypes.c_int, [ctypes.POINTER(GslmView), ctypes.c_int64, ctypes.c_void_p, ctypes.c_void_p,
                                          ctypes.c_size_t, ctypes.c_void_p, ctypes.c_size_t, ctypes.c_void_p,
                                          ctypes.c_void_p, ctypes.c_void_p, ctypes.c_void_p]),
    "gslm_rasterize_loss_dev": (ctypes.c_int, [ctypes.POINTER(GslmView), ctypes.c_int64, ctypes.c_void_p,
                                               ctypes.c_void_p, ctypes.c_size_t, ctypes.c_void_p, ctypes.c_void_p,
                                               ctypes.c_void_p, ctypes.c_size_t, ctypes.c_void_p, ctypes.c_int32,
                                               ctypes.c_void_p, ctypes.c_void_p]),
    "gslm_num_rendered_copy": (ctypes.c_int, [ctypes.c_void_p, ctypes.c_int64, ctypes.c_void_p, ctypes.c_void_p]),
    "gslm_union_binning_bytes": (ctypes.c_size_t, [ctypes.c_int64, ctypes.c_int32, ctypes.c_int32]),
    "gslm_depth_records_bytes": (ctypes.c_size_t, [ctypes.c_int64]),
    "gslm_union_geometry": (ctypes.c_int, [ctypes.POINTER(GslmView), ctypes.c_int64, ctypes.POINTER(ctypes.c_void_p),
                                           ctypes.c_int32, ctypes.c_size_t, ctypes.c_void_p, ctypes.c_size_t,
                                           ctypes.c_void_p]),
    "gslm_union_binning": (ctypes.c_int, [ctypes.POINTER(GslmView), ctypes.c_int64, ctypes.c_void_p, ctypes.c_void_p,
                                          ctypes.c_size_t, ctypes.c_int64, ctypes.POINTER(ctypes.c_void_p),
                                          ctypes.c_int32, ctypes.c_size_t, ctypes.c_void_p]),
    "gslm_rasterize_loss_slot": (ctypes.c_int, [ctypes.POINTER(GslmView), ctypes.c_int64, ctypes.c_void_p,
                                                ctypes.c_size_t, ctypes.c_void_p, ctypes.c_size_t, ctypes.c_int64,
                                                ctypes.c_int32, ctypes.c_int32, ctypes.c_void_p, ctypes.c_void_p,
                                                ctypes.c_void_p, ctypes.c_size_t, ctypes.c_void_p, ctypes.c_int32,
                                                ctypes.c_void_p]),
    "gslm_loss_sets_scratch_bytes": (ctypes.c_size_t, [ctypes.c_int32, ctypes.c_int32, ctypes.c_int32]),
    "gslm_rasterize_loss_sets": (ctypes.c_int, [ctypes.POINTER(GslmView), ctypes.c_int64,
                                                ctypes.POINTER(ctypes.c_void_p), ctypes.c_int32, ctypes.c_int32,
                                                ctypes.c_size_t,
                                                ctypes.c_void_p, ctypes.c_size_t, ctypes.c_int64, ctypes.c_void_p,
                                                ctypes.c_void_p, ctypes.c_void_p, ctypes.c_size_t,
                                                ctypes.POINTER(ctypes.c_void_p), ctypes.c_int32, ctypes.c_void_p]),
    "gslm_forward": (ctypes.c_int, [ctypes.POINTER(GslmView), ctypes.POINTER(GslmGaussians), ctypes.c_void_p,
                                    ctypes.c_size_t, ctypes.c_void_p, ctypes.c_size_t, ctypes.c_void_p,
                                    ctypes.c_size_t, ctypes.c_void_p, ctypes.c_void_p, ctypes.c_void_p,
                                    ctypes.POINTER(ctypes.c_int64), ctypes.c_void_p]),
    "gslm_backward": (ctypes.c_int, [ctypes.POINTER(GslmView), ctypes.POINTER(GslmGaussians), ctypes.c_void_p,
                                     ctypes.c_void_p, ctypes.c_int64, ctypes.c_void_p, ctypes.c_void_p,
                                     ctypes.c_void_p, ctypes.c_void_p, ctypes.c_size_t,
                                     ctypes.POINTER(GslmGrads), ctypes.c_void_p]),
    "gslm_jvp": (ctypes.c_int, [ctypes.POINTER(GslmView), ctypes.POINTER(GslmGaussians),
                                ctypes.POINTER(GslmGaussians), ctypes.c_void_p, ctypes.c_void_p, ctypes.c_void_p,
                                ctypes.c_int64, ctypes.c_void_p, ctypes.c_void_p, ctypes.c_size_t,
                                ctypes.c_void_p, ctypes.c_void_p, ctypes.c_void_p]),
    "gslm_matvec_view": (ctypes.c_int, [ctypes.POINTER(GslmView), ctypes.POINTER(GslmGaussians),
                                        ctypes.POINTER(GslmGrads), ctypes.c_void_p, ctypes.c_int32,
                                        ctypes.c_void_p, ctypes.c_void_p, ctypes.c_int64, ctypes.c_void_p,
                                        ctypes.c_void_p, ctypes.c_size_t, ctypes.POINTER(GslmGrads),
                                        ctypes.c_void_p]),
    "gslm_matvec_view_ex": (ctypes.c_int, [ctypes.POINTER(GslmView), ctypes.POINTER(GslmGaussians),
                                           ctypes.POINTER(GslmGrads), ctypes.c_void_p, ctypes.c_int32,
                                           ctypes.c_void_p, ctypes.c_void_p, ctypes.c_int64, ctypes.c_void_p,
                                           ctypes.c_void_p, ctypes.c_size_t, ctypes.POINTER(GslmGrads),
                                           ctypes.c_void_p, ctypes.c_void_p]),
    "gslm_sh_rest_project": (ctypes.c_int, [ctypes.POINTER(GslmView), ctypes.POINTER(GslmGaussians), ctypes.c_int32,
                                            ctypes.c_void_p, ctypes.c_int64, ctypes.c_void_p, ctypes.c_int64,
                                            ctypes.c_void_p]),
    "gslm_active_list_bytes": (ctypes.c_size_t, [ctypes.c_int64]),
    "gslm_active_list": (ctypes.c_int, [ctypes.c_void_p, ctypes.c_int64, ctypes.c_int64, ctypes.c_void_p,
                                        ctypes.c_size_t, ctypes.c_void_p, ctypes.c_size_t, ctypes.c_void_p,
                                        ctypes.c_void_p, ctypes.c_void_p, ctypes.c_void_p]),
    "gslm_matvec_view_active": (ctypes.c_int, [ctypes.POINTER(GslmView), ctypes.POINTER(GslmGaussians),
                                               ctypes.POINTER(GslmGrads), ctypes.c_void_p, ctypes.c_int32,
                                               ctypes.c_void_p, ctypes.c_void_p, ctypes.c_int64, ctypes.c_void_p,
                                               ctypes.c_void_p, ctypes.c_size_t, ctypes.POINTER(GslmGrads),
                                               ctypes.c_void_p, ctypes.c_void_p, ctypes.c_void_p, ctypes.c_int64,
                                               ctypes.c_void_p]),
    "gslm_active_pack": (ctypes.c_int, [ctypes.c_void_p, ctypes.c_void_p, ctypes.c_void_p, ctypes.c_int64,
                                        ctypes.c_int64, ctypes.POINTER(ctypes.c_int32), ctypes.c_int32,
                                        ctypes.c_int64, ctypes.c_void_p]),
    "gslm_active_unpack": (ctypes.c_int, [ctypes.c_void_p, ctypes.c_void_p, ctypes.c_void_p, ctypes.c_int64,
                                          ctypes.c_int64, ctypes.POINTER(ctypes.c_int32), ctypes.c_int32,
                                          ctypes.c_int64, ctypes.c_void_p]),
    "gslm_rest_basis": (ctypes.c_int, [ctypes.POINTER(GslmView), ctypes.c_int32, ctypes.POINTER(GslmGaussians),
                                       ctypes.c_void_p, ctypes.c_void_p]),
    "gslm_rest_coords": (ctypes.c_int, [ctypes.POINTER(GslmView), ctypes.c_int32, ctypes.POINTER(GslmGaussians),
                                        ctypes.c_void_p, ctypes.c_int32, ctypes.c_void_p, ctypes.c_int64,
                                        ctypes.c_void_p, ctypes.c_int64, ctypes.c_void_p]),
    "gslm_gather_screen": (ctypes.c_int, [ctypes.POINTER(GslmView), ctypes.c_int32, ctypes.POINTER(GslmGaussians),
                                          ctypes.c_void_p, ctypes.POINTER(GslmGrads), ctypes.POINTER(GslmGrads),
                                          ctypes.c_void_p, ctypes.c_void_p]),
    "gslm_gather_views": (ctypes.c_int, [ctypes.POINTER(GslmView), ctypes.POINTER(GslmViewWs), ctypes.c_int32,
                                         ctypes.POINTER(GslmGaussians), ctypes.POINTER(GslmGrads),
                                         ctypes.POINTER(GslmGrads), ctypes.c_void_p, ctypes.c_void_p]),
    "gslm_view_flags": (ctypes.c_int, [ctypes.c_void_p, ctypes.c_int64, ctypes.c_void_p, ctypes.c_void_p]),
    "gslm_tangent_views": (ctypes.c_int, [ctypes.POINTER(GslmView), ctypes.c_int32, ctypes.POINTER(GslmGaussians),
                                          ctypes.POINTER(GslmGrads), ctypes.c_int32, ctypes.c_void_p, ctypes.c_int64,
                                          ctypes.c_void_p, ctypes.c_int64, ctypes.c_void_p, ctypes.c_void_p]),
    "gslm_cg_update": (ctypes.c_int, [ctypes.c_int64, ctypes.c_void_p, ctypes.c_void_p, ctypes.c_void_p,
                                      ctypes.c_void_p, ctypes.c_void_p, ctypes.c_void_p, ctypes.c_void_p,
                                      ctypes.c_void_p, ctypes.c_void_p]),
    "gslm_cg_update_monitor": (ctypes.c_int, [ctypes.c_int64, ctypes.c_void_p, ctypes.c_void_p, ctypes.c_void_p,
                                              ctypes.c_void_p, ctypes.c_void_p, ctypes.c_void_p, ctypes.c_void_p,
                                              ctypes.c_void_p, ctypes.c_size_t, ctypes.c_void_p, ctypes.c_void_p,
                                              ctypes.c_void_p, ctypes.c_void_p, ctypes.c_void_p]),
    "gslm_cg_monitor": (ctypes.c_int, [ctypes.c_void_p, ctypes.c_void_p, ctypes.c_void_p, ctypes.c_void_p,
                                       ctypes.c_void_p, ctypes.c_void_p, ctypes.c_double, ctypes.c_double,
                                       ctypes.c_void_p, ctypes.c_int32, ctypes.c_void_p]),
    "gslm_dot_finalize": (ctypes.c_int, [ctypes.c_void_p, ctypes.c_int32, ctypes.c_void_p, ctypes.c_void_p]),
    "gslm_dot_scratch_bytes": (ctypes.c_size_t, [ctypes.c_int64]),
    "gslm_dot": (ctypes.c_int, [ctypes.c_void_p, ctypes.c_void_p, ctypes.POINTER(ctypes.c_int64),
                                ctypes.POINTER(ctypes.c_double), ctypes.c_int32, ctypes.c_int64, ctypes.c_void_p,
                                ctypes.c_void_p, ctypes.c_void_p]),
    "gslm_axpy_dev": (ctypes.c_int, [ctypes.c_int64, ctypes.c_void_p, ctypes.c_void_p, ctypes.c_float,
                                     ctypes.c_void_p, ctypes.c_void_p, ctypes.c_void_p]),
    "gslm_xpby_dev": (ctypes.c_int, [ctypes.c_int64, ctypes.c_void_p, ctypes.c_void_p, ctypes.c_void_p,
                                     ctypes.c_void_p, ctypes.c_void_p]),
    "gslm_damp_add": (ctypes.c_int, [ctypes.c_int64, ctypes.c_void_p, ctypes.POINTER(ctypes.c_int64),
                                     ctypes.POINTER(ctypes.c_double), ctypes.c_int32, ctypes.c_void_p,
                                     ctypes.c_void_p]),
    "gslm_comm_id_bytes": (ctypes.c_int32, []),
    "gslm_comm_unique_id": (ctypes.c_int, [ctypes.c_void_p]),
    "gslm_comm_init": (ctypes.c_int, [ctypes.c_void_p, ctypes.c_int32, ctypes.c_int32,
                                      ctypes.POINTER(ctypes.c_void_p)]),
    "gslm_comm_destroy": (ctypes.c_int, [ctypes.c_void_p]),
    "gslm_allreduce_sum_f32": (ctypes.c_int, [ctypes.c_void_p, ctypes.c_void_p, ctypes.c_int64, ctypes.c_void_p]),
    "gslm_allreduce_sum_f64": (ctypes.c_int, [ctypes.c_void_p, ctypes.c_void_p, ctypes.c_int64, ctypes.c_void_p]),
    "gslm_alltoall": (ctypes.c_int, [ctypes.c_void_p, ctypes.c_void_p, ctypes.c_void_p, ctypes.c_int64,
                                     ctypes.c_void_p]),
    "gslm_allgather": (ctypes.c_int, [ctypes.c_void_p, ctypes.c_void_p, ctypes.c_void_p, ctypes.c_int64,
                                      ctypes.c_void_p]),
    "gslm_residual_scratch_bytes": (ctypes.c_size_t, [ctypes.c_int32, ctypes.c_int32]),
    "gslm_lm_residual": (ctypes.c_int, [ctypes.c_int32, ctypes.c_int32, ctypes.c_void_p, ctypes.c_void_p,
                                        ctypes.c_void_p, ctypes.c_void_p, ctypes.c_void_p, ctypes.c_void_p,
                                        ctypes.c_void_p, ctypes.c_size_t, ctypes.c_void_p, ctypes.c_int32,
                                        ctypes.c_void_p]),
    "gslm_ssim_state_bytes": (ctypes.c_size_t, [ctypes.c_int32, ctypes.c_int32]),
    "gslm_ssim_residual": (ctypes.c_int, [ctypes.c_int32, ctypes.c_int32, ctypes.c_void_p, ctypes.c_void_p,
                                          ctypes.c_void_p, ctypes.c_float, ctypes.c_void_p, ctypes.c_size_t,
                                          ctypes.c_void_p, ctypes.c_void_p, ctypes.c_void_p, ctypes.c_void_p,
                                          ctypes.c_int32, ctypes.c_void_p]),
    "gslm_ssim_normal": (ctypes.c_int, [ctypes.c_int32, ctypes.c_int32, ctypes.c_void_p, ctypes.c_void_p,
                                        ctypes.c_void_p, ctypes.c_void_p, ctypes.c_void_p]),
    "gslm_ssim_mean_state_bytes": (ctypes.c_size_t, [ctypes.c_int32, ctypes.c_int32, ctypes.c_int32]),
    "gslm_ssim_mean": (ctypes.c_int, [ctypes.c_int32, ctypes.c_int32, ctypes.c_int32, ctypes.c_void_p, ctypes.c_void_p,
                                      ctypes.c_void_p, ctypes.c_size_t, ctypes.c_void_p, ctypes.c_void_p]),
    "gslm_ssim_mean_backward": (ctypes.c_int, [ctypes.c_int32, ctypes.c_int32, ctypes.c_int32, ctypes.c_void_p,
                                               ctypes.c_void_p, ctypes.c_void_p, ctypes.c_void_p, ctypes.c_void_p,
                                               ctypes.c_void_p]),
    "gslm_knn_scratch_bytes": (ctypes.c_size_t, [ctypes.c_int64]),
    "gslm_knn3_mean_dist": (ctypes.c_int, [ctypes.c_int64, ctypes.c_void_p, ctypes.c_void_p, ctypes.c_void_p,
                                           ctypes.c_size_t, ctypes.c_void_p]),
    "gslm_adam_step": (ctypes.c_int, [ctypes.POINTER(GslmAdamGroup), ctypes.c_int32, ctypes.c_double, ctypes.c_double,
                                      ctypes.c_double, ctypes.c_void_p, ctypes.c_int64, ctypes.c_int32,
                                      ctypes.c_void_p]),
    "gslm_densify_stats": (ctypes.c_int, [ctypes.c_int64, ctypes.c_void_p, ctypes.c_int64, ctypes.c_void_p,
                                          ctypes.c_void_p, ctypes.c_void_p, ctypes.c_void_p, ctypes.c_void_p]),
    "gslm_inspect": (ctypes.c_int, [ctypes.c_void_p, ctypes.c_int64, ctypes.c_void_p, ctypes.c_int64, ctypes.c_int32,
                                    ctypes.c_int32, ctypes.c_void_p, ctypes.c_void_p, ctypes.c_void_p,
                                    ctypes.c_void_p, ctypes.c_void_p, ctypes.c_void_p, ctypes.c_void_p,
                                    ctypes.c_void_p]),
    "gslm_inspect_rowmap": (ctypes.c_int, [ctypes.c_void_p, ctypes.c_int64, ctypes.c_int64, ctypes.c_void_p,
                                           ctypes.c_size_t, ctypes.c_void_p, ctypes.c_void_p, ctypes.c_void_p]),
    "gslm_selftest": (ctypes.c_int, [ctypes.c_int32, ctypes.c_void_p, ctypes.c_void_p, ctypes.c_void_p]),
    "gslm_selftest_scan": (ctypes.c_int, [ctypes.c_void_p, ctypes.c_void_p, ctypes.c_int64, ctypes.c_int32,
                                          ctypes.c_void_p, ctypes.c_size_t, ctypes.c_void_p, ctypes.c_void_p]),
# ... 163 lines not shown
```

### gaussian-splatting-lm_amd/gslm/lm.py

```python
import copy
import ctypes
import math
import os

import torch

from gslm import _lib
from gslm._lib import check, lib
from gslm.params import GROUPS, ParamLayout, raw_gaussians

STAGE_ALL = 7
STAGE_OVERWRITE = 8
MV_TAIL_CLEAN = 1
MV_SH_REST_PROJECTED = 2

DEFAULT_DAMP = {"xyz": 5e2, "features_dc": 5e-2, "features_rest": 5e-2, "scaling": 5e-2, "rotation": 5e-2,
                "opacity": 5e-2, "exposure": 1e1}


class ViewRaster:

    def __init__(self, view, device):
        self.view = view
        self.H, self.W = view.image_height, view.image_width
        self.device = device
        self.N = 0
        self.geom = self.binning = self.image = self.scratch = None
        self._active = None
        self.tail_clean = False
        self.epoch = 0

    @property
    def tail_clean(self):
        return self._tail_clean

    @tail_clean.setter
    def tail_clean(self, value):
        self._tail_clean = bool(value)
        if not value:
            self._active = None

    def active_list(self, P, stream):
        if not self.tail_clean or self.N is None:
            raise RuntimeError("active_list: no current LM row map (run a product or rhs() on this geometry first)")
        if self._active is None:
            dev = self.device
            ids = torch.empty(max(P, 1), dtype=torch.int32, device=dev)
            rows = torch.empty(P + 1, dtype=torch.int32, device=dev)
            count = torch.zeros(1, dtype=torch.int64, device=dev)
            work = _lib.u8(lib.gslm_active_list_bytes(P), dev)
            check(lib.gslm_active_list(self.geom.data_ptr(), P, self.N, self.scratch.data_ptr(), self.scratch.numel(),
                                       work.data_ptr(), work.numel(), ids.data_ptr(), rows.data_ptr(),
                                       count.data_ptr(), stream), "gslm_active_list")
            n = int(count.item())
            self._active = (ids[:n], n)
            self.active_rows = rows[:n + 1]
        return self._active

    def forward(self, g, stream, want_invdepth=True):
        P = g.P
        dev = self.device
        self.tail_clean = False
        self.epoch += 1
        if self.geom is None or self.geom.numel() < lib.gslm_geom_bytes(P):
            self.geom = _lib.u8(lib.gslm_geom_bytes(P), dev)
            self.image = _lib.u8(lib.gslm_image_bytes(self.H, self.W), dev)
            self.color = torch.empty(3, self.H, self.W, dtype=torch.float32, device=dev)
            self.invdepth = torch.empty(1, self.H, self.W, dtype=torch.float32, device=dev)
            self.radii = torch.empty(P, dtype=torch.int32, device=dev)
        check(lib.gslm_preprocess(ctypes.byref(self.view), ctypes.byref(g), self.geom.data_ptr(), self.geom.numel(),
                                  self.radii.data_ptr(), stream), "gslm_preprocess")
        n = ctypes.c_int64(0)
        check(lib.gslm_num_rendered(self.geom.data_ptr(), P, ctypes.byref(n), stream), "gslm_num_rendered")
        self.N = int(n.value)
        need = lib.gslm_binning_bytes(self.N, self.H, self.W)
        if self.binning is None or self.binning.numel() < need:
            self.binning = _lib.u8(int(need * 1.25) + 4096, dev)
        check(lib.gslm_rasterize(ctypes.byref(self.view), P, self.geom.data_ptr(), self.binning.data_ptr(),
                                 self.binning.numel(), self.N, self.image.data_ptr(), self.image.numel(),
                                 self.color.data_ptr(), self.invdepth.data_ptr() if want_invdepth else None, stream),
              "gslm_rasterize")
        need = lib.gslm_scratch_bytes(P, self.N)
        if self.scratch is None or self.scratch.numel() < need:
            self.scratch = _lib.u8(int(need * 1.25) + 4096, dev)
        return self.color


    def forward_dev(self, g, stream, want_invdepth=True, n_out=None):
        if self.binning is None or self.geom is None or self.geom.numel() < lib.gslm_geom_bytes(g.P):
            raise RuntimeError("forward_dev: the workspaces of an earlier forward() at this P are required")
        P = g.P
        self.tail_clean = False
        self.epoch += 1
        self.N = None
        check(lib.gslm_preprocess(ctypes.byref(self.view), ctypes.byref(g), self.geom.data_ptr(), self.geom.numel(),
                                  self.radii.data_ptr(), stream), "gslm_preprocess")
        check(lib.gslm_rasterize_dev(ctypes.byref(self.view), P, self.geom.data_ptr(), self.binning.data_ptr(),
                                     self.binning.numel(), self.image.data_ptr(), self.image.numel(),
                                     self.color.data_ptr(), self.invdepth.data_ptr() if want_invdepth else None,
                                     n_out, stream), "gslm_rasterize_dev")
        return self.color

    def capacity(self):
        return 0 if self.binning is None else int(lib.gslm_binning_capacity(self.binning.numel(), self.H, self.W))


class LMProblem:

    def __init__(self, model, cams, bg, gts=None, alpha_masks=None, mask_xyz=True, damp=None, device="cuda",
                 ssim=False, lambda_dssim=0.2, sh_projection=False):
        self.model = model
        self.ssim, self.lambda_dssim = bool(ssim), float(lambda_dssim)
        if self.ssim and not mask_xyz:
            raise ValueError("the SSIM residual path runs on the LM rows (mask_xyz=True, train_jvp.py:221-227)")
        self.cams = cams
        self.device = device
        self.bg = bg
        self.mask_xyz = bool(mask_xyz)
        P = model._xyz.shape[0]
        K = 1 + model._features_rest.shape[1]
        if sh_projection == "auto":
            sh_projection = len(cams) == 1 and K > 1 and model.active_sh_degree > 0
        if sh_projection and len(cams) != 1:
            raise ValueError("sh_projection is a single-view mode (the Krylov space of one view's J)")
        self.full_layout = ParamLayout(P, K, model._exposure.shape[0])
        self.layout = ParamLayout(P, K, model._exposure.shape[0], rest_projected=bool(sh_projection))
        self.mv_flags = MV_SH_REST_PROJECTED if self.layout.rest_projected else 0
        self.damp = DEFAULT_DAMP if damp is None else damp
        self._bounds, self._damps = self.layout.group_damp_arrays(self.damp)
        self.gts = [c.original_image.to(device) for c in cams] if gts is None else gts
        self.masks = [c.alpha_mask.to(device) for c in cams] if alpha_masks is None else alpha_masks
        self.views = [ViewRaster(_lib.view_from_camera(c, bg, model.active_sh_degree), device) for c in cams]
        self.stream = _lib.stream_handle(device)
        self.dot_scratch = torch.empty(max(lib.gslm_dot_scratch_bytes(max(P, self.layout.numel)) // 8, 3 * 1024) + 8,
                                       dtype=torch.float64, device=device)
        self.weights = [None] * len(cams)
        self.residuals = [None] * len(cams)
        self.seeds = [None] * len(cams)
        self.ssim_state = [None] * len(cams)
        self._jv = [None] * len(cams)
# ... 68 lines not shown

    def _mark_rhs(self, out, fused=True):
        self._rhs_token = (out.data_ptr(), out._version)
        self._rhs_epochs = [vr.epoch for vr in self.views] if fused else None
        return out

    def exposure_is_zero(self, g):
        if self.rhs_is_mine(g):
            return True
        e0, e1 = self.layout.offsets["exposure"]
        return not bool(g[e0:e1].any())

    def rhs_is_mine(self, g):
        return getattr(self, "_rhs_token", None) == (g.data_ptr(), g._version)

    def rhs_full(self, out):
        g = raw_gaussians(self.model)
        out.zero_()
        grads = self.full_layout.grads_struct(out, accumulate=True)
        for b, vr in enumerate(self.views):
            dL = self.seeds[b]
            check(lib.gslm_backward(ctypes.byref(vr.view), ctypes.byref(g), vr.geom.data_ptr(), vr.binning.data_ptr(),
                                    vr.N, vr.image.data_ptr(), dL.data_ptr(), None, vr.scratch.data_ptr(),
                                    vr.scratch.numel(), ctypes.byref(grads), self.stream), "gslm_backward")
            vr.tail_clean = False
        self._apply_mask(out, self.full_layout)
        return out

    def _rest_convert(self, mode, src, dst, src_layout, dst_layout):
        if self.layout.K < 2:
            return
        g = raw_gaussians(self.model)
        a0 = src_layout.offsets["features_rest"][0]
        b0 = dst_layout.offsets["features_rest"][0]
        src_w = 3 * src_layout.shapes["features_rest"][1]
        dst_w = 3 * dst_layout.shapes["features_rest"][1]
        check(lib.gslm_sh_rest_project(ctypes.byref(self.views[0].view), ctypes.byref(g), mode,
                                       src.data_ptr() + 4 * a0, src_w, dst.data_ptr() + 4 * b0, dst_w, self.stream),
              "gslm_sh_rest_project")

    def _copy_other_groups(self, src, dst, src_layout, dst_layout):
        for name in GROUPS:
            if name == "features_rest":
                continue
            a0, a1 = src_layout.offsets[name]
            b0, b1 = dst_layout.offsets[name]
            dst[b0:b1].copy_(src[a0:a1])

    def expand(self, x, out=None):
        if not self.layout.rest_projected:
            return x
        out = torch.empty(self.full_layout.numel, dtype=torch.float32, device=x.device) if out is None else out
        self._copy_other_groups(x, out, self.layout, self.full_layout)
        self._rest_convert(0, x, out, self.layout, self.full_layout)
        return out

    def project(self, x_full, out=None):
        if not self.layout.rest_projected:
            return x_full if out is None else out.copy_(x_full)
        out = torch.empty(self.layout.numel, dtype=torch.float32, device=x_full.device) if out is None else out
        self._copy_other_groups(x_full, out, self.full_layout, self.layout)
        self._rest_convert(1, x_full, out, self.full_layout, self.layout)
        return out

    def _apply_mask(self, vec, layout=None):
        o = (layout or self.layout).offsets
        if self.mask_xyz:
            vec[o["xyz"][0]:o["xyz"][1]].zero_()
        vec[o["exposure"][0]:o["exposure"][1]].zero_()

    def matvec(self, v, y, cg_ctl=None):
        self.matvec_dot(v, y, None, cg_ctl=cg_ctl)
        return y

    supports_exposure_zero = True
    supports_cg_ctl = True

    def matvec_dot(self, v, y, dot_out, pre=None, exposure_zero=False, cg_ctl=None):
        fuse = dot_out is not None and len(self.views) == 1
        self.local_normal_matvec(v, y, damp=True, dot_out=dot_out if fuse else None, pre=pre,
                                 exposure_zero=exposure_zero, cg_ctl=cg_ctl)
        return fuse

    def local_normal_matvec(self, v, y, damp=False, dot_out=None, pre=None, exposure_zero=False, cg_ctl=None):
        g = raw_gaussians(self.model)
        vs = self.layout.grads_struct(v)
        ys = self.layout.grads_struct(y)
        if pre is not None and not self.views:
            self._pre_without_views(v, pre)
            pre = None
        if not self.views:
            y.zero_()
            if damp:
                self.damp_add(v, y)
            return y
        last = len(self.views) - 1
        e0, e1 = self.layout.offsets["exposure"]
        for b, vr in enumerate(self.views):
            opts = _lib.GslmMatvecOpts()
            opts.stages = STAGE_ALL | (STAGE_OVERWRITE if b == 0 else 0)
            opts.flags = (MV_TAIL_CLEAN if vr.tail_clean else 0) | self.mv_flags
            opts.damp7 = self._damps if (damp and b == 0) else None
            opts.cg_ctl = cg_ctl
            if pre is not None and b == 0:
                ss = self._pre_opts(opts, v, pre)
            if dot_out is not None and b == last:
                opts.dot_vy = dot_out
                opts.dot_scratch = self.dot_scratch.data_ptr()
                opts.dot_scratch_bytes = self.dot_scratch.numel() * 8
            if self.ssim:
                self._ssim_product(b, vr, g, vs, ys, opts)
                continue
            self._view_product(vr, g, vs, self.weights[b].data_ptr(), ys, opts, "gslm_matvec_view_ex")
            vr.tail_clean = True
        if exposure_zero:
            pass
        elif damp:
            torch.mul(v[e0:e1], float(self._damps[6]), out=y[e0:e1])
        else:
            y[e0:e1].zero_()
        return y

    def _view_product(self, vr, g, vs, weight, ys, opts, what):
        if self._active is not None:
            ids, na = self._active
            check(lib.gslm_matvec_view_active(ctypes.byref(vr.view), ctypes.byref(g), ctypes.byref(vs), weight,
                                              int(self.mask_xyz), vr.geom.data_ptr(), vr.binning.data_ptr(), vr.N,
                                              vr.image.data_ptr(), vr.scratch.data_ptr(), vr.scratch.numel(),
                                              ctypes.byref(ys), ctypes.byref(opts), ids.data_ptr() if na else None,
                                              vr.active_rows.data_ptr(), na, self.stream),
                  what.replace("_ex", "_active"))
            return
        check(lib.gslm_matvec_view_ex(ctypes.byref(vr.view), ctypes.byref(g), ctypes.byref(vs), weight,
                                      int(self.mask_xyz), vr.geom.data_ptr(), vr.binning.data_ptr(), vr.N,
                                      vr.image.data_ptr(), vr.scratch.data_ptr(), vr.scratch.numel(), ctypes.byref(ys),
                                      ctypes.byref(opts), self.stream), what)

    def _pre_opts(self, opts, v, pre):
        s, num, den = pre[:3]
        e0, e1 = self.layout.offsets["exposure"]
        ss = self.layout.grads_struct(s)
        opts.xpby_s = ctypes.addressof(ss)
        opts.beta_num, opts.beta_den = num, den
        opts.xpby_tail_v = v.data_ptr() + 4 * e0
        opts.xpby_tail_s = s.data_ptr() + 4 * e0
        opts.xpby_tail_n = e1 - e0
        if len(pre) > 3 and pre[3] is not None:
            x, anum, aden = pre[3:]
            opts.alpha_num, opts.alpha_den = anum, aden
            opts.xpby_x_offset = x.data_ptr() - v.data_ptr()
        return ss

    def _pre_without_views(self, v, pre):
        s, num, den = pre[:3]
        if len(pre) > 3 and pre[3] is not None:
            x, anum, aden = pre[3:]
            check(lib.gslm_axpy_dev(v.numel(), anum, aden, 1.0, v.data_ptr(), x.data_ptr(), self.stream),
                  "gslm_axpy_dev")
        check(lib.gslm_xpby_dev(v.numel(), s.data_ptr(), num, den, v.data_ptr(), self.stream), "gslm_xpby_dev")

    def _ssim_product(self, b, vr, g, vs, ys, opts):
        jv, u = self._jv[b], self._u[b]
        o1 = _lib.GslmMatvecOpts()
        o1.stages = 1 | 2
        o1.flags = (MV_TAIL_CLEAN if vr.tail_clean else 0) | self.mv_flags
        o1.jv_out = jv.data_ptr()
        o1.xpby_s, o1.beta_num, o1.beta_den = opts.xpby_s, opts.beta_num, opts.beta_den
        o1.xpby_tail_v, o1.xpby_tail_s, o1.xpby_tail_n = opts.xpby_tail_v, opts.xpby_tail_s, opts.xpby_tail_n
        o1.alpha_num, o1.alpha_den, o1.xpby_x_offset = opts.alpha_num, opts.alpha_den, opts.xpby_x_offset
        o1.cg_ctl = opts.cg_ctl
        self._view_product(vr, g, vs, jv.data_ptr(), ys, o1, "gslm_matvec_view_ex(jv)")
        check(lib.gslm_ssim_normal(vr.H, vr.W, self.gts[b].data_ptr(), self.ssim_state[b].data_ptr(), jv.data_ptr(),
                                   u.data_ptr(), self.stream), "gslm_ssim_normal")
        o2 = _lib.GslmMatvecOpts()
        o2.stages = 2 | 4 | (opts.stages & STAGE_OVERWRITE)
        o2.flags = (MV_TAIL_CLEAN if vr.tail_clean else 0) | self.mv_flags
        o2.pixel_seed = u.data_ptr()
        o2.damp7 = opts.damp7
        o2.dot_vy, o2.dot_scratch, o2.dot_scratch_bytes = opts.dot_vy, opts.dot_scratch, opts.dot_scratch_bytes
        o2.cg_ctl = opts.cg_ctl
        self._view_product(vr, g, vs, u.data_ptr(), ys, o2, "gslm_matvec_view_ex(seed)")
        vr.tail_clean = True

    def views_for(self, cams, pad_to=None):
        vs = [_lib.view_from_camera(c, self.bg, self.model.active_sh_degree) for c in cams]
        vs += [vs[-1]] * max(0, (pad_to or len(vs)) - len(vs))
        arr = (_lib.GslmView * len(vs))()
        for k, vw in enumerate(vs):
            arr[k] = vw
        return arr

    def screen_products(self, v, screen, pre=None, cg_ctl=None):
        g = raw_gaussians(self.model)
        vs = self.layout.grads_struct(v)
        ys = self.layout.grads_struct(v)
        e0, e1 = self.layout.offsets["exposure"]
        if pre is not None and not self.views:
            self._pre_without_views(v, pre)
        for b, vr in enumerate(self.views):
            opts = _lib.GslmMatvecOpts()
            opts.stages = 1 | 2 | 16
            opts.flags = MV_TAIL_CLEAN if vr.tail_clean else 0
            opts.screen_out = screen[b].data_ptr()
            opts.cg_ctl = cg_ctl
            if pre is not None and b == 0:
                ss = self._pre_opts(opts, v, pre)
# ... 292 lines not shown
        self._mark(0)
        for c0 in range(0, V, self.CHUNK):
            c1 = min(V, c0 + self.CHUNK)
            opts = None
            if (pre is not None and c0 == 0) or R is not None or cg_ctl is not None:
                opts = _lib.GslmMatvecOpts()
                opts.cg_ctl = cg_ctl
                if pre is not None and c0 == 0:
                    keep.append(self._pre_opts(opts, v, pre))
                if R is not None:
                    opts.rest_basis, opts.rest_views, opts.view_base = R.data_ptr(), self.rest_views, c0
            check(lib.gslm_tangent_views(self._view_ptr(c0), c1 - c0, ctypes.byref(g), ctypes.byref(vs), 1,
                                         self._flags.data_ptr() + 4 * c0 * P, P,
                                         self._trec.data_ptr() + 32 * c0 * P, P,
                                         None if opts is None else ctypes.byref(opts), self.stream),
                  "gslm_tangent_views")
        self._mark(1)
        for b, vr in enumerate(self.views):
            opts = _lib.GslmMatvecOpts()
            opts.stages = 2
            opts.flags = MV_TAIL_CLEAN if vr.tail_clean else 0
            opts.trec_in = self._trec[b].data_ptr()
            opts.cg_ctl = cg_ctl
            check(lib.gslm_matvec_view_ex(ctypes.byref(vr.view), ctypes.byref(g), ctypes.byref(vs),
                                          self.weights[b].data_ptr(), 1, vr.geom.data_ptr(), vr.binning.data_ptr(),
                                          vr.N, vr.image.data_ptr(), vr.scratch.data_ptr(), vr.scratch.numel(),
                                          ctypes.byref(vs), ctypes.byref(opts), self.stream), "gslm_matvec_view_ex")
            vr.tail_clean = True
        self._mark(2)
        self._gather(g, vs, ys, damp, dot_out, cg_ctl)
        self._mark(3)
        e0, e1 = self.layout.offsets["exposure"]
        if exposure_zero:
            pass
        elif damp:
            torch.mul(v[e0:e1], float(self._damps[6]), out=y[e0:e1])
        else:
            y[e0:e1].zero_()
        return y


class NonFiniteError(AssertionError):
    """A NaN or Inf reached the normal equations.  The reference's only failure detection on the LM path is
    matvec_T's `assert not torch.isnan(self.gaussians._<group>.grad).any(), "NaN detected in gaussians._<group>.grad"`
    (solver/solver_functions.py:125-130), which aborts the step before the parameters move; this is raised at the
    same point of the fused solve (an AssertionError, with the reference's message), before update_params."""


CG_STOP_NONFINITE = 4


def raise_nonfinite(prob, g, what="the normal-equations product (J^T J + D) p"):
    names = []
    try:
        for k, v in prob.layout.views(g).items():
            if k != "exposure" and v.numel() and not bool(torch.isfinite(v).all()):
                names.append(k)
    except (AttributeError, RuntimeError, TypeError):
        pass
    if names:
        raise NonFiniteError("; ".join(f"NaN detected in gaussians._{k}.grad" for k in names))
    raise NonFiniteError(f"NaN detected in {what} during CGLS (J^T b is finite)")


def _active_view_for(prob, g, callback):
    if callback is not None or os.environ.get("GSLM_CG_ACTIVE", "1") == "0":
        return None
    local = prob
    if not isinstance(local, LMProblem):
        from gslm import parallel
        if not (isinstance(local, parallel.ShardedOperator) and not parallel.collectives_on(local.world_size)):
            return None
        local = local.local
        if not isinstance(local, LMProblem):
            return None
    if g.numel() != local.layout.numel:
        return None
    act = local.active_view()
    if act is None or not act.zero_off_active(g):
        return None
    return act


def cgls_fused(prob, g, max_iter=10, restart_iter=10, tol=1e-10, atol=0.0, check_every=True, verbose=False,
               callback=None, host_checks=None):
    act = _active_view_for(prob, g, callback)
    if act is not None:
        gp = act.pack(g)
        if prob.exposure_is_zero(g):
            act._mark_rhs(gp)
        x, info = cgls_fused(act, gp, max_iter=max_iter, restart_iter=restart_iter, tol=tol, atol=atol,
                             check_every=check_every, verbose=verbose, callback=None, host_checks=host_checks)
        return act.unpack(x), info
    n = prob.layout.numel
    dev = prob.device
    st = prob.stream
    lo = (3 * prob.layout.P // 4) * 4 if getattr(prob, "mask_xyz", False) else 0
    na = n - lo
    off = lambda t: t.data_ptr() + 4 * lo
    sc = torch.zeros(16, dtype=torch.float64, device=dev)
    ptr = lambda i: sc.data_ptr() + 8 * i
    GAM, GAMN, DEL, XG, XS = 0, 1, 2, 3, 4
    x = torch.zeros(n, dtype=torch.float32, device=dev)
    s = torch.empty_like(x)
    p = torch.empty_like(x)
    q = torch.zeros_like(x)
    if host_checks is None:
        host_checks = verbose or callback is not None
    on_device = check_every and not host_checks
    ctl = None
    if on_device:
        ctl = torch.full((4 + max_iter,), math.nan, dtype=torch.float64, device=dev)
        ctl[:4] = torch.tensor([0.0, 0.0, math.inf, 0.0], dtype=torch.float64)
        loss = prob.loss
        b2_dev = loss if (torch.is_tensor(loss) and loss.is_cuda and loss.dtype == torch.float64 and
                          loss.numel() == 1) else torch.tensor(float(loss), dtype=torch.float64, device=dev)
    cg_ctl = ctl.data_ptr() if ctl is not None else None
    ctl_kw = {"cg_ctl": cg_ctl} if (cg_ctl is not None and getattr(prob, "supports_cg_ctl", False)) else {}
    b2 = float(prob.loss) if (check_every and not on_device) else None
    iter_total, last_res, history = 0, math.inf, []
    defer = not check_every and callback is None
    pend = None
    red = getattr(prob, "allreduce_scalars", None)

    def reduce(*slots):
        if red is not None:
            red(sc, slots)

    def flush():
        nonlocal pend
        if pend is not None:
            check(lib.gslm_axpy_dev(na, pend[0], pend[1], 1.0, off(p), off(x), st), "gslm_axpy_dev")
            pend = None

    ez = {"exposure_zero": True} if (getattr(prob, "supports_exposure_zero", False) and
                                     prob.exposure_is_zero(g)) else {}
    first = True
    while iter_total < max_iter:
        if first:
            s.copy_(g)
            first = False
        else:
            flush()
            prob.matvec(x, q, **ctl_kw)
            torch.sub(g, q, out=s)
        p.copy_(s)
        prob.dot(s[lo:], s[lo:], ptr(GAM))
        reduce(GAM)
        stop = False
        pre = None
        for _ in range(restart_iter):
            full = None if pre is None else pre + ((x, pend[0], pend[1]) if pend is not None else (None, None, None))
            if full is not None:
                pend = None
            if not prob.matvec_dot(p, q, ptr(DEL), pre=full, **ez, **ctl_kw):
                prob.dot(p[lo:], q[lo:], ptr(DEL))
            reduce(DEL)
            if check_every and not on_device and not math.isfinite(sc[DEL].item()):
                raise_nonfinite(prob, g)
            if check_every and not on_device and sc[DEL].item() < 1e-20:
                if verbose:
                    print("Early termination: delta is too small.")
                stop = True
                break
            if check_every:
                check(lib.gslm_cg_update_monitor(na, ptr(GAM), ptr(DEL), off(p), off(q), off(x), off(s), off(g),
                                                 prob.dot_scratch.data_ptr(), prob.dot_scratch.numel() * 8,
                                                 ptr(GAMN), ptr(XG), ptr(XS), cg_ctl, st))
                reduce(GAMN, XG, XS)
# ... 582 lines not shown
```

### include/gslm.h

```cpp
#ifndef GSLM_H
#define GSLM_H

#include <stddef.h>
#include <stdint.h>

#ifdef __cplusplus
extern "C" {
#endif

#define GSLM_OK 0
#define GSLM_ERR_INVALID (-1)
#define GSLM_ERR_HIP (-2)
#define GSLM_ERR_CAPACITY (-3)

#define GSLM_ABI_VERSION 9

typedef struct gslm_view {
  int32_t image_height;
  int32_t image_width;
  double tanfovx;
  double tanfovy;
  double scale_modifier;
  float viewmatrix[16];
  float projmatrix[16];
// ... 78 lines not shown
                             const float* alpha_mask, void* scratch, size_t scratch_bytes, double* loss_dev,
                             int32_t accumulate, void* stream);
size_t gslm_loss_sets_scratch_bytes(int32_t n, int32_t H, int32_t W);
int gslm_rasterize_loss_sets(const gslm_view* view, int64_t P, const void* const* geoms, int32_t n, int32_t first_set,
                             size_t set_bytes, const void* binning, size_t binning_bytes, int64_t num_rendered,
                             const float* gt, const float* alpha_mask, void* scratch, size_t scratch_bytes,
                             double* const* loss_dev, int32_t accumulate, void* stream);
int gslm_forward(const gslm_view* view, const gslm_gaussians* g, void* geom, size_t geom_bytes,
                 void* binning, size_t binning_bytes, void* image, size_t image_bytes,
                 float* out_color, float* out_invdepth, int32_t* out_radii,
                 int64_t* out_num_rendered, void* stream);

int gslm_backward(const gslm_view* view, const gslm_gaussians* g, const void* geom, const void* binning,
                  int64_t num_rendered, const void* image, const float* dL_dcolor,
                  const float* dL_dinvdepth, void* scratch, size_t scratch_bytes,
                  const gslm_grads* out, void* stream);

int gslm_jvp(const gslm_view* view, const gslm_gaussians* g, const gslm_gaussians* tangent,
             const float* means2D_tangent, const void* geom, const void* binning, int64_t num_rendered,
             const void* image, void* scratch, size_t scratch_bytes, float* out_color_t,
             float* out_invdepth_t, void* stream);

int gslm_matvec_view(const gslm_view* view, const gslm_gaussians* g, const gslm_grads* v,
                     const float* pixel_weight, int32_t mask_xyz, const void* geom, const void* binning,
                     int64_t num_rendered, const void* image, void* scratch, size_t scratch_bytes,
                     const gslm_grads* y, void* stream);

#define GSLM_STAGE_TANGENT 1
#define GSLM_STAGE_RENDER 2
#define GSLM_STAGE_GATHER 4
#define GSLM_STAGE_ALL 7
#define GSLM_STAGE_OVERWRITE 8
#define GSLM_STAGE_SCREEN 16
#define GSLM_MV_TAIL_CLEAN 1
#define GSLM_MV_SH_REST_PROJECTED 2
typedef struct gslm_matvec_opts {
  int32_t stages;
  int32_t flags;
  const double* damp7;
  double* dot_vy;
  void* dot_scratch;
  size_t dot_scratch_bytes;
  const gslm_grads* xpby_s;
  const double* beta_num;
  const double* beta_den;
  float* xpby_tail_v;
  const float* xpby_tail_s;
  int64_t xpby_tail_n;
  float* screen_out;
  const float* pixel_seed;
  float* jv_out;
  const double* alpha_num;
  const double* alpha_den;
  int64_t xpby_x_offset;
  const float* trec_in;
  int64_t screen_stride;
  const double* cg_ctl;
  const float* rest_basis;
  int32_t rest_views;
  int32_t view_base;
} gslm_matvec_opts;
int gslm_matvec_view_ex(const gslm_view* view, const gslm_gaussians* g, const gslm_grads* v,
                        const float* pixel_weight, int32_t mask_xyz, const void* geom, const void* binning,
                        int64_t num_rendered, const void* image, void* scratch, size_t scratch_bytes,
                        const gslm_grads* y, const gslm_matvec_opts* opts, void* stream);

int gslm_sh_rest_project(const gslm_view* view, const gslm_gaussians* g, int32_t mode, const float* in,
                         int64_t in_stride, float* out, int64_t out_stride, void* stream);

size_t gslm_active_list_bytes(int64_t P);
int gslm_active_list(const void* geom, int64_t P, int64_t num_rendered, const void* scratch, size_t scratch_bytes,
                     void* work, size_t work_bytes, int32_t* ids_dev, uint32_t* rows_dev, int64_t* count_dev,
                     void* stream);
int gslm_matvec_view_active(const gslm_view* view, const gslm_gaussians* g, const gslm_grads* v,
                            const float* pixel_weight, int32_t mask_xyz, const void* geom, const void* binning,
                            int64_t num_rendered, const void* image, void* scratch, size_t scratch_bytes,
                            const gslm_grads* y, const gslm_matvec_opts* opts, const int32_t* active_ids,
                            const uint32_t* active_rows, int64_t n_active, void* stream);
int gslm_active_pack(const float* src, float* dst, const int32_t* active_ids, int64_t n_active, int64_t P,
                     const int32_t* widths, int32_t ngroups, int64_t tail_n, void* stream);
int gslm_active_unpack(const float* src, float* dst, const int32_t* active_ids, int64_t n_active, int64_t P,
                       const int32_t* widths, int32_t ngroups, int64_t tail_n, void* stream);

int gslm_gather_screen(const gslm_view* views, int32_t nviews, const gslm_gaussians* g, const float* screen,
                       const gslm_grads* v, const gslm_grads* y, const gslm_matvec_opts* opts, void* stream);

typedef struct gslm_view_ws {
  const void* geom;
  const void* scratch;
  size_t scratch_bytes;
  int64_t num_rendered;
} gslm_view_ws;
int gslm_gather_views(const gslm_view* views, const gslm_view_ws* ws, int32_t nviews, const gslm_gaussians* g,
                      const gslm_grads* v, const gslm_grads* y, const gslm_matvec_opts* opts, void* stream);

int gslm_view_flags(const void* geom, int64_t P, uint32_t* out, void* stream);
int gslm_tangent_views(const gslm_view* views, int32_t nviews, const gslm_gaussians* g, const gslm_grads* v,
                       int32_t mask_xyz, const uint32_t* vflags, int64_t flags_stride, float* trec_out,
                       int64_t trec_stride, const gslm_matvec_opts* opts, void* stream);

#define GSLM_MAX_REST_VIEWS 8
int gslm_rest_basis(const gslm_view* views, int32_t nviews, const gslm_gaussians* g, float* R_out, void* stream);
int gslm_rest_coords(const gslm_view* views, int32_t nviews, const gslm_gaussians* g, const float* R, int32_t mode,
                     const float* in, int64_t in_stride, float* out, int64_t out_stride, void* stream);

size_t gslm_dot_scratch_bytes(int64_t n);
int gslm_dot(const float* a, const float* b, const int64_t* group_bounds, const double* group_damp,
             int32_t ngroups, int64_t n, void* scratch, double* out_dev, void* stream);
int gslm_axpy_dev(int64_t n, const double* num_dev, const double* den_dev, float sign, const float* x,
                  float* y, void* stream);
int gslm_xpby_dev(int64_t n, const float* s, const double* num_dev, const double* den_dev, float* p,
                  void* stream);
int gslm_cg_update(int64_t n, const double* gam_dev, const double* del_dev, const float* p, const float* q,
                   float* x, float* s, void* scratch, double* gam_new_dev, void* stream);
int gslm_cg_update_monitor(int64_t n, const double* gam_dev, const double* del_dev, const float* p, const float* q,
                           float* x, float* s, const float* g, void* scratch, size_t scratch_bytes,
                           double* gam_new_dev, double* xg_dev, double* xs_dev, const double* cg_ctl, void* stream);
#define GSLM_CG_STOP_NONFINITE 4
int gslm_cg_monitor(const double* gam_dev, const double* gam_new_dev, const double* del_dev, const double* xg_dev,
                    const double* xs_dev, const double* b2_dev, double tol, double atol, double* cg_ctl,
                    int32_t max_hist, void* stream);
int gslm_dot_finalize(const void* partials, int32_t np, double* out_dev, void* stream);
int gslm_damp_add(int64_t n, const float* x, const int64_t* group_bounds, const double* group_damp,
                  int32_t ngroups, float* y, void* stream);

int32_t gslm_comm_id_bytes(void);
int gslm_comm_unique_id(void* id_out);
int gslm_comm_init(const void* id, int32_t nranks, int32_t rank, void** comm_out);
int gslm_comm_destroy(void* comm);
int gslm_allreduce_sum_f32(void* comm, float* buf, int64_t n, void* stream);
int gslm_allreduce_sum_f64(void* comm, double* buf, int64_t n, void* stream);
int gslm_alltoall(void* comm, const void* send, void* recv, int64_t bytes_per_rank, void* stream);
int gslm_allgather(void* comm, const void* send, void* recv, int64_t bytes_per_rank, void* stream);

size_t gslm_residual_scratch_bytes(int32_t H, int32_t W);
int gslm_lm_residual(int32_t H, int32_t W, const float* color, const float* gt, const float* alpha_mask,
                     float* residual, float* weight, float* seed, void* scratch, size_t scratch_bytes,
                     double* loss_dev, int32_t accumulate, void* stream);

size_t gslm_ssim_state_bytes(int32_t H, int32_t W);
int gslm_ssim_residual(int32_t H, int32_t W, const float* color, const float* gt, const float* alpha_mask,
                       float lambda_dssim, void* state, size_t state_bytes, float* r1, float* r2, float* seed,
                       double* loss_dev, int32_t accumulate, void* stream);
int gslm_ssim_normal(int32_t H, int32_t W, const float* gt, void* state, const float* jv, float* u, void* stream);

size_t gslm_ssim_mean_state_bytes(int32_t C, int32_t H, int32_t W);
int gslm_ssim_mean(int32_t C, int32_t H, int32_t W, const float* img, const float* gt, void* state,
                   size_t state_bytes, float* ssim_out, void* stream);
int gslm_ssim_mean_backward(int32_t C, int32_t H, int32_t W, const float* img, const float* gt, const void* state,
                            const float* grad_out, float* grad_img, void* stream);

size_t gslm_knn_scratch_bytes(int64_t n);
int gslm_knn3_mean_dist(int64_t n, const float* xyz, float* out, void* scratch, size_t scratch_bytes, void* stream);

#define GSLM_ADAM_MAX_GROUPS 8
typedef struct gslm_adam_group {
  float* param;
  const float* grad;
  float* exp_avg;
  float* exp_avg_sq;
  int64_t n;
  int32_t floats_per_gaussian;
  int32_t _pad;
  double lr;
  int64_t step;
} gslm_adam_group;
// ... 35 lines not shown
```

Baseline: 1756 view-matvec/s (one (J^T J + D) application per 1080p view, 1M Gaussians).

## Add lean CG path with deferred dot partials and compacted active-Gaussian parameters

Adds a lean CGLS loop for the single-view active-list case. The <v,y> and beta dot products stay as per-block partials and are reduced inside the next consuming kernel, which removes separate finalize launches. Parameters and clamp words of the active Gaussians are packed into a contiguous block, so the tangent and gather kernels read them densely. New start/end kernels fuse the initial pack, residual and final unpack. This adds code complexity and a new ABI struct, and the path is on by default through an environment variable.

```diff
diff --git a/gaussian-splatting-lm_amd/csrc/api.hip b/gaussian-splatting-lm_amd/csrc/api.hip
--- a/gaussian-splatting-lm_amd/csrc/api.hip
+++ b/gaussian-splatting-lm_amd/csrc/api.hip
@@ -706,6 +706,8 @@
   return GSLM_OK;
 }
 
+static const uint32_t* active_params_bind(const void* block, int64_t na, GaussK* g);
+
 static int matvec_view(const gslm_view* view, const gslm_gaussians* gi, const gslm_grads* vin,
                        const float* pixel_weight, int32_t mask_xyz, const void* geom, const void* binning,
                        int64_t N, const void* image, void* scratch, size_t scratch_bytes, const gslm_grads* y,
@@ -716,6 +718,10 @@
   int st = bind_all(view, gi, geom, binning, N, image, scratch, scratch_bytes, &b);
   if (st) return st;
   if (!vin || !y || !pixel_weight) { set_error("matvec: NULL argument"); return GSLM_ERR_INVALID; }
+  const gslm_cg_lean* lean = (opts && (opts->flags & GSLM_MV_LEAN))
+                                 ? &reinterpret_cast<const gslm_matvec_opts_lean*>(opts)->lean : nullptr;
+  if (lean && na < 0) { set_error("matvec: GSLM_MV_LEAN is an option of gslm_matvec_view_active"); return GSLM_ERR_INVALID; }
+  const bool dot_defer = lean && lean->dot_defer;
   const int32_t stages = (opts && opts->stages) ? opts->stages : GSLM_STAGE_ALL;
   const double* damp7 = opts ? opts->damp7 : nullptr;
   double* dot_out = opts ? opts->dot_vy : nullptr;
@@ -732,7 +738,11 @@
       return GSLM_ERR_INVALID;
     }
   }
-  if (dot_out && (!opts->dot_scratch || opts->dot_scratch_bytes < gslm_dot_scratch_bytes(rows))) {
+  if (dot_defer && (!opts || dot_out)) {
+    set_error("matvec_view_active (GSLM_MV_LEAN): dot_defer leaves <v, y> as partials in dot_scratch (dot_vy must be NULL)");
+    return GSLM_ERR_INVALID;
+  }
+  if ((dot_out || dot_defer) && (!opts->dot_scratch || opts->dot_scratch_bytes < gslm_dot_scratch_bytes(rows))) {
     set_error("matvec: dot scratch too small");
     return GSLM_ERR_CAPACITY;
   }
@@ -764,6 +774,24 @@
       return GSLM_ERR_INVALID;
     }
     if ((st = build_xpby(opts, vin, proj ? 3 : 3 * (b.g.M - 1), mask_xyz != 0, &xp))) return st;
+    if (lean && lean->beta_partials) {
+      if (lean->beta_np < 0 || lean->beta_partials == opts->dot_scratch) {
+        set_error("matvec_view_active (GSLM_MV_LEAN): beta's partials need a count and a buffer other than dot_scratch");
+        return GSLM_ERR_INVALID;
+      }
+      xp.num_part = (const double*)lean->beta_partials;
+      xp.num_np = lean->beta_np;
+      xp.num_store = lean->beta_store;
+    }
+  } else if (lean && lean->beta_partials) {
+    set_error("matvec_view_active (GSLM_MV_LEAN): beta's partials without the fused direction update (xpby_s)");
+    return GSLM_ERR_INVALID;
+  }
+  GaussK gp = b.g;
+  const uint32_t* clamp_list = nullptr;
+  if (lean && lean->params) {
+    if (!active) { set_error("matvec_view_active (GSLM_MV_LEAN): a parameter block belongs to an active list"); return GSLM_ERR_INVALID; }
+    clamp_list = active_params_bind(lean->params, na, &gp);
   }
   if (opts && opts->trec_in) {
     if (stages & GSLM_STAGE_TANGENT) {
@@ -778,8 +806,8 @@
     return GSLM_ERR_INVALID;
   }
   if ((stages & GSLM_STAGE_TANGENT) &&
-      (st = launch_tangent_pre(b.v, b.g, t, nullptr, b.gb, b.sb, fused_xpby ? &xp : nullptr, s, mask_xyz != 0, ids,
-                               na)))
+      (st = launch_tangent_pre(b.v, gp, t, nullptr, b.gb, b.sb, fused_xpby ? &xp : nullptr, s, mask_xyz != 0, ids,
+                               na, clamp_list)))
     return st;
   float* jv_out = opts ? opts->jv_out : nullptr;
   if (jv_out) {
@@ -812,9 +840,10 @@
     return launch_rowsum_screen(b.g, b.gb, b.sb, opts->screen_out, s);
   }
   if (!(stages & GSLM_STAGE_GATHER)) return GSLM_OK;
-  double* part = dot_out ? (double*)opts->dot_scratch : nullptr;
-  if ((st = launch_gather_lm(b.v, b.g, b.gb, b.sb, make_gradk(y), make_gradk(vin), damp7,
-                             (stages & GSLM_STAGE_OVERWRITE) != 0, mask_xyz != 0, part, s, proj, ids, na, hrow)))
+  double* part = (dot_out || dot_defer) ? (double*)opts->dot_scratch : nullptr;
+  if ((st = launch_gather_lm(b.v, gp, b.gb, b.sb, make_gradk(y), make_gradk(vin), damp7,
+                             (stages & GSLM_STAGE_OVERWRITE) != 0, mask_xyz != 0, part, s, proj, ids, na, hrow,
+                             clamp_list)))
     return st;
   if (dot_out) return gslm_dot_finalize(part, (int32_t)((rows + 255) / 256), dot_out, stream);
   return GSLM_OK;
@@ -836,6 +865,73 @@
   if (n_active < 0) { set_error("matvec_view_active: negative n_active"); return GSLM_ERR_INVALID; }
   return matvec_view(view, gi, vin, pixel_weight, mask_xyz, geom, binning, N, image, scratch, scratch_bytes, y, opts,
                      active_ids, n_active, active_rows, stream);
+}
+
+static size_t active_params_layout(int64_t na, void* base, float** xyz, float** sc, float** rot, float** op,
+                                   uint32_t** cw) {
+  Carver c{(char*)base};
+  const int64_t n = na > 0 ? na : 1;
+  float* a = c.take<float>(3 * n);
+  float* b = c.take<float>(3 * n);
+  float* r = c.take<float>(4 * n);
+  float* o = c.take<float>(n);
+  uint32_t* w = c.take<uint32_t>(n);
+  if (xyz) { *xyz = a; *sc = b; *rot = r; *op = o; *cw = w; }
+  return c.off;
+}
+
+static const uint32_t* active_params_bind(const void* block, int64_t na, GaussK* g) {
+  float *xyz, *sc, *rot, *op;
+  uint32_t* cw;
+  active_params_layout(na, const_cast<void*>(block), &xyz, &sc, &rot, &op, &cw);
+  g->means3D = xyz;
+  g->scales = sc;
+  g->rot = rot;
+  g->opac = op;
+  return cw;
+}
+
+size_t gslm_active_params_bytes(int64_t n_active) {
+  return active_params_layout(n_active, nullptr, nullptr, nullptr, nullptr, nullptr, nullptr);
+}
+
+int gslm_active_params(const gslm_gaussians* gi, const void* geom, int64_t P, const int32_t* active_ids,
+                       int64_t n_active, void* block, size_t block_bytes, int32_t* pos_dev, void* stream) {
+  if (!gi || !geom || P < 0 || n_active < 0 || n_active > P || !block || !pos_dev || (n_active > 0 && !active_ids)) {
+    set_error("active_params: NULL argument or 0 <= n_active <= P violated");
+    return GSLM_ERR_INVALID;
+  }
+  if (block_bytes < gslm_active_params_bytes(n_active)) {
+    set_error("active_params: block smaller than gslm_active_params_bytes(n_active)");
+    return GSLM_ERR_CAPACITY;
+  }
+  if (gi->P != P || !gi->raw || gi->cov3D_precomp || gi->colors_precomp ||
+      (P > 0 && (!gi->means3D || !gi->scales || !gi->rotations || !gi->opacities))) {
+    set_error("active_params: the raw GaussianModel leaves of the P Gaussians the list was built for");
+    return GSLM_ERR_INVALID;
+  }
+  GeomBufs gb;
+  geom_layout(P, const_cast<void*>(geom), &gb);
+  float *xyz, *sc, *rot, *op;
+  uint32_t* cw;
+  active_params_layout(n_active, block, &xyz, &sc, &rot, &op, &cw);
+  return launch_active_params(gi->means3D, gi->scales, gi->rotations, gi->opacities, gb.clampw, active_ids, n_active,
+                              P, xyz, sc, rot, op, cw, pos_dev, (hipStream_t)stream);
+}
+
+int gslm_cg_start_active(const float* g_full, const int32_t* active_ids, int64_t n_active, int64_t P,
+                         const int32_t* widths, int32_t ngroups, int64_t tail_n, int64_t lo, float* s, float* p,
+                         float* q, float* x, void* partials, void* stream) {
+  return launch_cg_start_active(g_full, active_ids, n_active, P, widths, ngroups, tail_n, lo, s, p, q, x,
+                                (double*)partials, (hipStream_t)stream);
+}
+
+int gslm_cg_end_active(const float* x, const float* p, const double* num_dev, const double* den_dev, int64_t lo,
+                       const int32_t* pos_dev, int64_t n_active, int64_t P, const int32_t* widths, int32_t ngroups,
+                       int64_t tail_n, float* out_full, const void* fin_partials, int32_t fin_np, double* fin_dev,
+                       void* stream) {
+  return launch_cg_end_active(x, p, num_dev, den_dev, lo, pos_dev, n_active, P, widths, ngroups, tail_n, out_full,
+                              (const double*)fin_partials, fin_np, fin_dev, (hipStream_t)stream);
 }
 
 static size_t active_work_layout(int64_t P, void* base, uint32_t** flags, uint32_t** tmp, uint32_t** total) {
diff --git a/gaussian-splatting-lm_amd/csrc/cg.hip b/gaussian-splatting-lm_amd/csrc/cg.hip
--- a/gaussian-splatting-lm_amd/csrc/cg.hip
+++ b/gaussian-splatting-lm_amd/csrc/cg.hip
@@ -8,9 +8,6 @@
   double damp[MAXG];
   int n;
 };
-
-constexpr int DOT_THREADS = 256;
-constexpr int DOT_BLOCKS = 1024;
 
 __device__ __forceinline__ double group_w(const Groups& g, int64_t i) {
   double w = 1.0;
@@ -21,18 +18,6 @@
       if (k < g.n && i >= g.bound[k] && i < g.bound[k + 1]) w = g.damp[k];
   }
   return w;
-}
-
-__device__ __forceinline__ double block_sum_d(double x, double* s) {
-  const int tid = threadIdx.x, lane = tid & 63, w = tid >> 6;
-#pragma unroll
-  for (int o = 32; o > 0; o >>= 1) x += __shfl_down(x, o, 64);
-  if (lane == 0) s[w] = x;
-  __syncthreads();
-  double t = 0.0;
-  if (tid == 0)
-    for (int k = 0; k < DOT_THREADS / 64; ++k) t += s[k];
-  return t;
 }
 
 __global__ __launch_bounds__(DOT_THREADS) void k_dot_partial(const float* __restrict__ a, const float* __restrict__ b,
@@ -90,16 +75,20 @@
   for (int64_t i = (int64_t)blockIdx.x * blockDim.x + threadIdx.x; i < n; i += stride) p[i] = s[i] + b * p[i];
 }
 
-template <bool MONITOR>
+template <bool MONITOR, bool PARTS = false>
 __global__ __launch_bounds__(DOT_THREADS) void k_cg_update(int64_t n, const double* __restrict__ gam,
                                                            const double* __restrict__ del,
                                                            const float* __restrict__ p, const float* __restrict__ q,
                                                            float* __restrict__ x, float* __restrict__ s,
                                                            const float* __restrict__ g, double* __restrict__ part,
-                                                           const double* __restrict__ ctl) {
-  __shared__ double sm[DOT_THREADS / 64];
+                                                           const double* __restrict__ ctl, ScalarK gams,
+                                                           ScalarK dels) {
+  __shared__ double sm[DOT_THREADS / 64 + 1];
   if (ctl && (ctl[0] != 0.0 || *del < 1e-20 || !isfinite(*del))) return;
-  const float a = (float)((*gam) / (*del));
+  const double gv = PARTS ? load_scalar(gams, sm) : *gam;
+  const double dv = PARTS ? load_scalar(dels, sm) : *del;
+  if (PARTS) __syncthreads();
+  const float a = (float)(gv / dv);
   double acc = 0.0, axg = 0.0, axs = 0.0;
   const int64_t n4 = n / 4;
   const int64_t stride = (int64_t)gridDim.x * DOT_THREADS;
@@ -232,8 +221,29 @@
   }
   hipStream_t st = (hipStream_t)stream;
   hipLaunchKernelGGL(k_cg_update<false>, dim3(DOT_BLOCKS), dim3(DOT_THREADS), 0, st, n, gam_dev, del_dev, p, q, x, s,
-                     nullptr, (double*)scratch, (const double*)nullptr);
+                     nullptr, (double*)scratch, (const double*)nullptr, ScalarK{}, ScalarK{});
   hipLaunchKernelGGL(k_dot_final, dim3(1), dim3(DOT_THREADS), 0, st, (const double*)scratch, DOT_BLOCKS, gam_new_dev);
+  GSLM_LAUNCH_CHECK();
+  return GSLM_OK;
+}
+
+int gslm_cg_update_lean(int64_t n, double* gam_dev, const void* gam_partials, int32_t gam_np,
+                        const void* del_partials, int32_t del_np, double* del_dev, const float* p, const float* q,
+                        float* s, void* partials_out, void* stream) {
+  if (!gam_dev || gam_np < 0 || !del_partials || del_np < 0 || !partials_out || partials_out == del_partials ||
+      partials_out == gam_partials) {
+    set_error("gslm_cg_update_lean: NULL scalar / partials, or the new partials in a buffer of the old ones");
+    return GSLM_ERR_INVALID;
+  }
+  if ((reinterpret_cast<uintptr_t>(p) | reinterpret_cast<uintptr_t>(q) | reinterpret_cast<uintptr_t>(s)) & 15) {
+    set_error("gslm_cg_update_lean: vectors must be 16-byte aligned");
+    return GSLM_ERR_INVALID;
+  }
+  const ScalarK gams{gam_dev, (const double*)gam_partials, gam_np, gam_dev};
+  const ScalarK dels{nullptr, (const double*)del_partials, del_np, del_dev};
+  hipLaunchKernelGGL((k_cg_update<false, true>), dim3(DOT_BLOCKS), dim3(DOT_THREADS), 0, (hipStream_t)stream, n,
+                     (const double*)gam_dev, (const double*)nullptr, p, q, (float*)nullptr, s, (const float*)nullptr,
+                     (double*)partials_out, (const double*)nullptr, gams, dels);
   GSLM_LAUNCH_CHECK();
   return GSLM_OK;
 }
@@ -253,7 +263,7 @@
   hipStream_t st = (hipStream_t)stream;
   const double* part = (const double*)scratch;
   hipLaunchKernelGGL(k_cg_update<true>, dim3(DOT_BLOCKS), dim3(DOT_THREADS), 0, st, n, gam_dev, del_dev, p, q, x, s, g,
-                     (double*)scratch, cg_ctl);
+                     (double*)scratch, cg_ctl, ScalarK{}, ScalarK{});
   hipLaunchKernelGGL(k_dot_final3, dim3(3), dim3(DOT_THREADS), 0, st, part, DOT_BLOCKS, gam_new_dev, xg_dev, xs_dev);
   GSLM_LAUNCH_CHECK();
   return GSLM_OK;
diff --git a/gaussian-splatting-lm_amd/csrc/gather.hip b/gaussian-splatting-lm_amd/csrc/gather.hip
--- a/gaussian-splatting-lm_amd/csrc/gather.hip
+++ b/gaussian-splatting-lm_amd/csrc/gather.hip
@@ -97,7 +97,8 @@
                                                     const uint32_t* __restrict__ hscan,
                                                     const float4* __restrict__ rows, FlatK o,
                                                     const int32_t* __restrict__ ids, int64_t na,
-                                                    const uint32_t* __restrict__ hrow) {
+                                                    const uint32_t* __restrict__ hrow,
+                                                    const uint32_t* __restrict__ clamp_list) {
   o.rest_proj = PROJ ? 1 : 0;
   if (cg_stopped(v)) return;
   extern __shared__ __attribute__((aligned(16))) float s_rest[];
@@ -122,7 +123,8 @@
     block_sum_rows<ROWF4>(rows, R0, R1, h0, h1 - h0, reinterpret_cast<float4*>(s_rest), G2);
   }
   ChainOut co;
-  if (valid) chain_vjp<true>(v, g, i, n != 0, n ? clampw[i] : 0u, G2, WANT_MEANS, co);
+  const bool listed = ACTIVE && clamp_list != nullptr;
+  if (valid) chain_vjp<true>(v, g, listed ? j : i, n != 0, n ? (listed ? clamp_list[j] : clampw[i]) : 0u, G2, WANT_MEANS, co);
   if (ACTIVE) g.P = na;
   lm_epilogue<WANT_MEANS, true>((v.D + 1) * (v.D + 1), g, co, o, s_rest, s_dot);
 }
@@ -204,7 +206,8 @@
 
 int launch_gather_lm(const ViewK& v, const GaussK& g, const GeomBufs& gb, const ScratchBufs& sb, const GradK& y,
                      const GradK& vin, const double* damp7, bool overwrite, bool mask_xyz, double* dot_part,
-                     hipStream_t s, bool rest_proj, const int32_t* ids, int64_t na, const uint32_t* hrow) {
+                     hipStream_t s, bool rest_proj, const int32_t* ids, int64_t na, const uint32_t* hrow,
+                     const uint32_t* clamp_list) {
   const bool active = na >= 0;
   const int64_t nrows = active ? na : g.P;
   if (nrows == 0) return GSLM_OK;
@@ -221,22 +224,22 @@
   const size_t lds = (rest_lds > chunk_lds ? rest_lds : chunk_lds) + 16;
   if (active && o.rest_proj)
     hipLaunchKernelGGL((k_gather_lm<false, 2, true, true>), dim3(nb), dim3(256), lds, s, v, g, gb.clampw, gb.tiles,
-                       gb.goff, sb.hscan, sb.contrib, o, ids, na, hrow);
+                       gb.goff, sb.hscan, sb.contrib, o, ids, na, hrow, clamp_list);
   else if (active)
     hipLaunchKernelGGL((k_gather_lm<false, 2, false, true>), dim3(nb), dim3(256), lds, s, v, g, gb.clampw, gb.tiles,
-                       gb.goff, sb.hscan, sb.contrib, o, ids, na, hrow);
+                       gb.goff, sb.hscan, sb.contrib, o, ids, na, hrow, clamp_list);
   else if (mask_xyz && o.rest_proj)
     hipLaunchKernelGGL((k_gather_lm<false, 2, true>), dim3(nb), dim3(256), lds, s, v, g, gb.clampw, gb.tiles, gb.goff,
-                       sb.hscan, sb.contrib, o, nullptr, -1, nullptr);
+                       sb.hscan, sb.contrib, o, nullptr, -1, nullptr, nullptr);
   else if (mask_xyz)
     hipLaunchKernelGGL((k_gather_lm<false, 2, false>), dim3(nb), dim3(256), lds, s, v, g, gb.clampw, gb.tiles, gb.goff,
-                       sb.hscan, sb.contrib, o, nullptr, -1, nullptr);
+                       sb.hscan, sb.contrib, o, nullptr, -1, nullptr, nullptr);
   else if (o.rest_proj)
     hipLaunchKernelGGL((k_gather_lm<true, 3, true>), dim3(nb), dim3(256), lds, s, v, g, gb.clampw, gb.tiles, gb.goff,
-                       sb.hscan, sb.contrib, o, nullptr, -1, nullptr);
+                       sb.hscan, sb.contrib, o, nullptr, -1, nullptr, nullptr);
   else
     hipLaunchKernelGGL((k_gather_lm<true, 3, false>), dim3(nb), dim3(256), lds, s, v, g, gb.clampw, gb.tiles, gb.goff,
-                       sb.hscan, sb.contrib, o, nullptr, -1, nullptr);
+                       sb.hscan, sb.contrib, o, nullptr, -1, nullptr, nullptr);
   GSLM_LAUNCH_CHECK();
   return GSLM_OK;
 }
@@ -293,4 +296,200 @@
   return GSLM_OK;
 }
 
-}
+__global__ __launch_bounds__(256) void k_active_params(const float* __restrict__ means3D, const float* __restrict__ scales,
+                                                        const float* __restrict__ rot, const float* __restrict__ opac,
+                                                        const uint32_t* __restrict__ clampw,
+                                                        const int32_t* __restrict__ ids, int64_t na,
+                                                        float* __restrict__ xyz_l, float* __restrict__ scales_l,
+                                                        float* __restrict__ rot_l, float* __restrict__ opac_l,
+                                                        uint32_t* __restrict__ clamp_l, int32_t* __restrict__ pos) {
+  const int64_t j = (int64_t)blockIdx.x * blockDim.x + threadIdx.x;
+  if (j >= na) return;
+  const int64_t i = ids[j];
+#pragma unroll
+  for (int k = 0; k < 3; ++k) {
+    xyz_l[3 * j + k] = means3D[3 * i + k];
+    scales_l[3 * j + k] = scales[3 * i + k];
+  }
+#pragma unroll
+  for (int k = 0; k < 4; ++k) rot_l[4 * j + k] = rot[4 * i + k];
+  opac_l[j] = opac[i];
+  clamp_l[j] = clampw[i];
+  pos[i] = (int32_t)j;
+}
+
+int launch_active_params(const float* means3D, const float* scales, const float* rot, const float* opac,
+                         const uint32_t* clampw, const int32_t* ids, int64_t na, int64_t P, float* xyz_l,
+                         float* scales_l, float* rot_l, float* opac_l, uint32_t* clamp_l, int32_t* pos, hipStream_t s) {
+  if (P > 0) GSLM_HIP_CHECK(hipMemsetAsync(pos, 0xFF, (size_t)P * sizeof(int32_t), s));
+  if (na == 0) return GSLM_OK;
+  hipLaunchKernelGGL(k_active_params, dim3((unsigned)((na + 255) / 256)), dim3(256), 0, s, means3D, scales, rot, opac,
+                     clampw, ids, na, xyz_l, scales_l, rot_l, opac_l, clamp_l, pos);
+  GSLM_LAUNCH_CHECK();
+  return GSLM_OK;
+}
+
+static int make_packk(const char* who, const int32_t* widths, int ngroups, int64_t na, int64_t P, PackK* k, int64_t* po,
+                      int64_t* ao) {
+  if (ngroups < 1 || ngroups > 8 || !widths || na < 0 || na > P) {
+    set_error(std::string(who) + ": 1..8 groups, 0 <= n_active <= P");
+    return GSLM_ERR_INVALID;
+  }
+  *k = PackK{};
+  *po = *ao = 0;
+  for (int q = 0; q < ngroups; ++q) {
+    if (widths[q] < 0) { set_error(std::string(who) + ": negative group width"); return GSLM_ERR_INVALID; }
+    k->w[q] = widths[q];
+    k->poff[q] = *po;
+    k->aoff[q] = *ao;
+    *po += P * widths[q];
+    *ao += na * widths[q];
+    k->wsum += widths[q];
+  }
+  k->n = ngroups;
+  return GSLM_OK;
+}
+
+__device__ __forceinline__ void divmod_w(int64_t r, int w, int64_t& d, int& c) {
+  if (r < ((int64_t)1 << 32)) {
+    const uint32_t d32 = w == 3 ? (uint32_t)r / 3u : w == 4 ? (uint32_t)r / 4u : w == 1 ? (uint32_t)r
+                                                                                         : (uint32_t)r / (uint32_t)w;
+    d = d32;
+    c = (int)((uint32_t)r - d32 * (uint32_t)w);
+  } else {
+    d = r / w;
+    c = (int)(r - d * w);
+  }
+}
+
+__global__ __launch_bounds__(DOT_THREADS) void k_cg_start_active(PackK k, const int32_t* __restrict__ ids, int64_t lo,
+                                                                  int64_t ao, int64_t po, int64_t tail_n,
+                                                                  const float* __restrict__ gf, float* __restrict__ s,
+                                                                  float* __restrict__ p, float* __restrict__ q,
+                                                                  float* __restrict__ x, double* __restrict__ part) {
+  __shared__ double sm[DOT_THREADS / 64];
+  const int64_t n = ao + tail_n;
+  const int64_t stride = (int64_t)gridDim.x * DOT_THREADS;
+  const int64_t t0 = (int64_t)blockIdx.x * DOT_THREADS + threadIdx.x;
+  for (int64_t m = t0; m < lo; m += stride) s[m] = p[m] = q[m] = x[m] = 0.f;
+  double acc = 0.0;
+  constexpr int U = 4;
+  for (int64_t m0 = lo + t0; m0 < n; m0 += U * stride) {
+    float v[U];
+#pragma unroll
+    for (int u = 0; u < U; ++u) {
+      const int64_t m = m0 + u * stride;
+      v[u] = 0.f;
+      if (m >= n) continue;
+      if (m >= ao) {
+        v[u] = gf[po + (m - ao)];
+      } else {
+        int grp = 0;
+        while (grp < k.n - 1 && m >= k.aoff[grp + 1]) ++grp;
+        int64_t j;
+        int c;
+        divmod_w(m - k.aoff[grp], k.w[grp], j, c);
+        v[u] = gf[k.poff[grp] + (int64_t)ids[j] * k.w[grp] + c];
+      }
+    }
+#pragma unroll
+    for (int u = 0; u < U; ++u) {
+      const int64_t m = m0 + u * stride;
+      if (m >= n) continue;
+      s[m] = v[u];
+      p[m] = v[u];
+      q[m] = 0.f;
+      x[m] = 0.f;
+      acc += (double)v[u] * (double)v[u];
+    }
+  }
+  const double t = block_sum_d(acc, sm);
+  if (threadIdx.x == 0) part[blockIdx.x] = t;
+}
+
+int launch_cg_start_active(const float* g_full, const int32_t* ids, int64_t na, int64_t P, const int32_t* widths,
+                           int ngroups, int64_t tail_n, int64_t lo, float* s_, float* p, float* q, float* x,
+                           double* part, hipStream_t s) {
+  PackK k;
+  int64_t po, ao;
+  int st = make_packk("cg_start_active", widths, ngroups, na, P, &k, &po, &ao);
+  if (st) return st;
+  if (!g_full || !s_ || !p || !q || !x || !part || (na > 0 && !ids) || tail_n < 0 || lo < 0 || lo > ao + tail_n) {
+    set_error("cg_start_active: NULL buffer, negative tail or lo outside [0, n]");
+    return GSLM_ERR_INVALID;
+  }
+  hipLaunchKernelGGL(k_cg_start_active, dim3(DOT_BLOCKS), dim3(DOT_THREADS), 0, s, k, ids, lo, ao, po, tail_n, g_full, s_,
+                     p, q, x, part);
+  GSLM_LAUNCH_CHECK();
+  return GSLM_OK;
+}
+
+__global__ __launch_bounds__(DOT_THREADS) void k_cg_end_active(PackK k, const int32_t* __restrict__ pos, int64_t P,
+                                                                int64_t lo, int64_t ao, int64_t po, int64_t tail_n,
+                                                                const float* __restrict__ x, const float* __restrict__ p,
+                                                                const double* __restrict__ num,
+                                                                const double* __restrict__ den, float* __restrict__ out,
+                                                                ScalarK fin) {
+  __shared__ double sm[DOT_THREADS / 64 + 1];
+  if (blockIdx.x == 0 && blockIdx.y == 0 && fin.part) load_scalar(fin, sm);
+  float af = 0.f;
+  if (num) {
+    const double a = den ? (*num) / (*den) : (*num);
+    af = (float)(a * (double)1.0f);
+  }
+  const int grp = blockIdx.y;
+  if (grp == k.n) {
+    const int64_t stride = (int64_t)gridDim.x * DOT_THREADS;
+    for (int64_t e = (int64_t)blockIdx.x * DOT_THREADS + threadIdx.x; e < tail_n; e += stride) {
+      const int64_t m = ao + e;
+      float v = x[m];
+      if (num && m >= lo) v = v + af * p[m];
+      out[po + e] = v;
+    }
+    return;
+  }
+  const int64_t i = (int64_t)blockIdx.x * DOT_THREADS + threadIdx.x;
+  if (i >= P) return;
+  const int w = k.w[grp];
+  const int32_t j = pos[i];
+  float* o = out + k.poff[grp] + i * w;
+  if (j < 0) {
+    for (int c = 0; c < w; ++c) o[c] = 0.f;
+    return;
+  }
+  const int64_t m0 = k.aoff[grp] + (int64_t)j * w;
+  for (int c0 = 0; c0 < w; c0 += 4) {
+    float xv[4], pv[4];
+#pragma unroll
+    for (int c = 0; c < 4; ++c) {
+      const bool on = c0 + c < w;
+      xv[c] = on ? x[m0 + c0 + c] : 0.f;
+      pv[c] = (on && num && m0 + c0 + c >= lo) ? p[m0 + c0 + c] : 0.f;
+    }
+#pragma unroll
+    for (int c = 0; c < 4; ++c)
+      if (c0 + c < w) o[c0 + c] = (num && m0 + c0 + c >= lo) ? xv[c] + af * pv[c] : xv[c];
+  }
+}
+
+int launch_cg_end_active(const float* x, const float* p, const double* num, const double* den, int64_t lo,
+                         const int32_t* pos, int64_t na, int64_t P, const int32_t* widths, int ngroups,
+                         int64_t tail_n, float* out, const double* fin_part, int fin_np, double* fin_dev,
+                         hipStream_t s) {
+  PackK k;
+  int64_t po, ao;
+  int st = make_packk("cg_end_active", widths, ngroups, na, P, &k, &po, &ao);
+  if (st) return st;
+  if (!x || !out || (num && !p) || (P > 0 && !pos) || tail_n < 0 || lo < 0 || (fin_part && (fin_np < 0 || !fin_dev))) {
+    set_error("cg_end_active: NULL buffer, negative tail or lo, or partials without a slot for their sum");
+    return GSLM_ERR_INVALID;
+  }
+  int64_t nb = (P + DOT_THREADS - 1) / DOT_THREADS;
+  nb = nb < 1 ? 1 : nb;
+  hipLaunchKernelGGL(k_cg_end_active, dim3((unsigned)nb, (unsigned)(k.n + 1)), dim3(DOT_THREADS), 0, s, k, pos, P, lo, ao,
+                     po, tail_n, x, p, num, den, out, ScalarK{nullptr, fin_part, fin_np, fin_dev});
+  GSLM_LAUNCH_CHECK();
+  return GSLM_OK;
+}
+
+}
diff --git a/gaussian-splatting-lm_amd/csrc/gslm_device.hpp b/gaussian-splatting-lm_amd/csrc/gslm_device.hpp
--- a/gaussian-splatting-lm_amd/csrc/gslm_device.hpp
+++ b/gaussian-splatting-lm_amd/csrc/gslm_device.hpp
@@ -38,9 +38,8 @@
 };
 
 template <typename F>
-__device__ __forceinline__ F strided_sum_in_order(const F* __restrict__ x, int64_t n) {
+__device__ __forceinline__ F strided_sum_in_order(const F* __restrict__ x, int64_t n, int64_t T) {
   F acc = F(0);
-  const int64_t T = blockDim.x;
   for (int64_t i = threadIdx.x; i < n; i += 8 * T) {
     F v[8];
 #pragma unroll
@@ -50,6 +49,10 @@
       if (i + k * T < n) acc += v[k];
   }
   return acc;
+}
+template <typename F>
+__device__ __forceinline__ F strided_sum_in_order(const F* __restrict__ x, int64_t n) {
+  return strided_sum_in_order(x, n, (int64_t)blockDim.x);
 }
 
 __device__ __forceinline__ float clamp01(float x) { return x < 0.0f ? 0.0f : (x > 1.0f ? 1.0f : x); }
diff --git a/gaussian-splatting-lm_amd/csrc/gslm_internal.hpp b/gaussian-splatting-lm_amd/csrc/gslm_internal.hpp
--- a/gaussian-splatting-lm_amd/csrc/gslm_internal.hpp
+++ b/gaussian-splatting-lm_amd/csrc/gslm_internal.hpp
@@ -41,6 +41,48 @@
   } while (0)
 
 inline size_t align_up(size_t x, size_t a = 256) { return (x + a - 1) / a * a; }
+
+constexpr int DOT_THREADS = 256;
+constexpr int DOT_BLOCKS = 1024;
+
+__device__ __forceinline__ double block_sum_d(double x, double* s) {
+  const int tid = threadIdx.x, lane = tid & 63, w = tid >> 6;
+#pragma unroll
+  for (int o = 32; o > 0; o >>= 1) x += __shfl_down(x, o, 64);
+  if (lane == 0) s[w] = x;
+  __syncthreads();
+  double t = 0.0;
+  if (tid == 0)
+    for (int k = 0; k < DOT_THREADS / 64; ++k) t += s[k];
+  return t;
+}
+
+struct ScalarK {
+  const double* v;
+  const double* part;
+  int np;
+  double* store;
+};
+inline ScalarK scalar_of(const double* v) { return ScalarK{v, nullptr, 0, nullptr}; }
+
+__device__ __forceinline__ double load_scalar(const ScalarK& k, double* sm) {
+  if (!k.part) return *k.v;
+  const int tid = threadIdx.x, lane = tid & 63, w = tid >> 6;
+  double acc = 0.0;
+  if (tid < DOT_THREADS) acc = strided_sum_in_order(k.part, k.np, DOT_THREADS);
+#pragma unroll
+  for (int o = 32; o > 0; o >>= 1) acc += __shfl_down(acc, o, 64);
+  if (lane == 0 && w < DOT_THREADS / 64) sm[w] = acc;
+  __syncthreads();
+  if (tid == 0) {
+    double t = 0.0;
+    for (int q = 0; q < DOT_THREADS / 64; ++q) t += sm[q];
+    sm[DOT_THREADS / 64] = t;
+    if (k.store && blockIdx.x == 0) *k.store = t;
+  }
+  __syncthreads();
+  return sm[DOT_THREADS / 64];
+}
 
 constexpr int SORT_THREADS = 256;
 constexpr int SORT_ITEMS = 16;
diff --git a/gaussian-splatting-lm_amd/csrc/gslm_kernels.hpp b/gaussian-splatting-lm_amd/csrc/gslm_kernels.hpp
--- a/gaussian-splatting-lm_amd/csrc/gslm_kernels.hpp
+++ b/gaussian-splatting-lm_amd/csrc/gslm_kernels.hpp
@@ -471,10 +471,13 @@
   const double* anum;
   const double* aden;
   int64_t xoff;
+  const double* num_part;
+  int num_np;
+  double* num_store;
 };
 int launch_tangent_pre(const ViewK& v, const GaussK& g, const GaussK& t, const float* m2t, const GeomBufs& gb,
                        const ScratchBufs& sb, const XpbyK* xp, hipStream_t s, bool compact,
-                       const int32_t* ids = nullptr, int64_t na = -1);
+                       const int32_t* ids = nullptr, int64_t na = -1, const uint32_t* clamp_list = nullptr);
 int launch_rowsum_screen(const GaussK& g, const GeomBufs& gb, const ScratchBufs& sb, float* out, hipStream_t s);
 constexpr int MAX_SCREEN_VIEWS = 16;
 constexpr int MAX_REST_VIEWS = GSLM_MAX_REST_VIEWS;
@@ -512,7 +515,17 @@
 int launch_gather_lm(const ViewK& v, const GaussK& g, const GeomBufs& gb, const ScratchBufs& sb, const GradK& y,
                      const GradK& vin, const double* damp7, bool overwrite, bool mask_xyz, double* dot_part,
                      hipStream_t s, bool rest_proj = false, const int32_t* ids = nullptr, int64_t na = -1,
-                     const uint32_t* hrow = nullptr);
+                     const uint32_t* hrow = nullptr, const uint32_t* clamp_list = nullptr);
+int launch_active_params(const float* means3D, const float* scales, const float* rot, const float* opac,
+                         const uint32_t* clampw, const int32_t* ids, int64_t na, int64_t P, float* xyz_l,
+                         float* scales_l, float* rot_l, float* opac_l, uint32_t* clamp_l, int32_t* pos, hipStream_t s);
+int launch_cg_start_active(const float* g_full, const int32_t* ids, int64_t na, int64_t P, const int32_t* widths,
+                           int ngroups, int64_t tail_n, int64_t lo, float* s_, float* p, float* q, float* x,
+                           double* part, hipStream_t s);
+int launch_cg_end_active(const float* x, const float* p, const double* num, const double* den, int64_t lo,
+                         const int32_t* pos, int64_t na, int64_t P, const int32_t* widths, int ngroups,
+                         int64_t tail_n, float* out, const double* fin_part, int fin_np, double* fin_dev,
+                         hipStream_t s);
 int launch_active_pack(bool to_active, const float* src, float* dst, const int32_t* ids, int64_t na, int64_t P,
                        const int32_t* widths, int ngroups, int64_t tail_n, hipStream_t s);
 int launch_sh_rest_project(const ViewK& v, const GaussK& g, int mode, const float* in, int64_t in_stride, float* out,
diff --git a/gaussian-splatting-lm_amd/csrc/tangent.hip b/gaussian-splatting-lm_amd/csrc/tangent.hip
--- a/gaussian-splatting-lm_amd/csrc/tangent.hip
+++ b/gaussian-splatting-lm_amd/csrc/tangent.hip
@@ -4,7 +4,8 @@
 namespace gslm {
 
 __device__ __forceinline__ void block_xpby(const XpbyK& xp, int64_t P, float* s_rest) {
-  const float b = (float)((*xp.num) / (*xp.den));
+  __shared__ double s_fin[DOT_THREADS / 64 + 1];
+  const float b = (float)(load_scalar(ScalarK{xp.num, xp.num_part, xp.num_np, xp.num_store}, s_fin) / (*xp.den));
   const bool with_x = xp.anum != nullptr;
   const float a = with_x ? (float)((*xp.anum) / (*xp.aden)) : 0.f;
   const int64_t i0 = (int64_t)blockIdx.x * blockDim.x;
@@ -92,7 +93,8 @@
                                                          const uint32_t* __restrict__ clampw,
                                                          const uint32_t* __restrict__ tiles,
                                                          float4* __restrict__ trec, XpbyK xp, int compact,
-                                                         int lead, const int32_t* __restrict__ ids, int64_t na) {
+                                                         int lead, const int32_t* __restrict__ ids, int64_t na,
+                                                         const uint32_t* __restrict__ clamp_list) {
   extern __shared__ __attribute__((aligned(16))) float s_rest[];
   if (cg_stopped(v)) return;
   const int64_t j = (int64_t)blockIdx.x * blockDim.x + threadIdx.x;
@@ -112,13 +114,14 @@
   const int64_t i = ACTIVE ? (int64_t)ids[j] : j;
   if (!ACTIVE && tiles[i] == 0) return;
   float T2[10];
-  chain_jvp<RAW>(v, g, t, m2t, i, j, clampw[i], T2);
+  const bool listed = ACTIVE && clamp_list != nullptr;
+  chain_jvp<RAW>(v, g, t, m2t, listed ? j : i, j, listed ? clamp_list[j] : clampw[i], T2);
   store_trec(trec, i, T2, compact != 0);
 }
 
 int launch_tangent_pre(const ViewK& v, const GaussK& g, const GaussK& t, const float* m2t, const GeomBufs& gb,
                        const ScratchBufs& sb, const XpbyK* xp, hipStream_t s, bool compact, const int32_t* ids,
-                       int64_t na) {
+                       int64_t na, const uint32_t* clamp_list) {
   const bool active = na >= 0;
   const int64_t n = active ? na : g.P;
   if (n == 0 && !(xp && xp->tail_p)) return GSLM_OK;
@@ -137,25 +140,25 @@
     const size_t lds = (size_t)256 * xp->w[2] * sizeof(float);
     if (active)
       hipLaunchKernelGGL((k_preprocess_jvp<true, true, true>), dim3(nb), dim3(256), lds, s, v, g, t, m2t, gb.clampw,
-                         gb.tiles, sb.trec, x, compact ? 1 : 0, -1, ids, na);
+                         gb.tiles, sb.trec, x, compact ? 1 : 0, -1, ids, na, clamp_list);
     else if (g.raw)
       hipLaunchKernelGGL((k_preprocess_jvp<true, true>), dim3(nb), dim3(256), lds, s, v, g, t, m2t, gb.clampw, gb.tiles,
-                         sb.trec, x, compact ? 1 : 0, -1, nullptr, -1);
+                         sb.trec, x, compact ? 1 : 0, -1, nullptr, -1, nullptr);
     else
       hipLaunchKernelGGL((k_preprocess_jvp<false, true>), dim3(nb), dim3(256), lds, s, v, g, t, m2t, gb.clampw, gb.tiles,
-                         sb.trec, x, compact ? 1 : 0, -1, nullptr, -1);
+                         sb.trec, x, compact ? 1 : 0, -1, nullptr, -1, nullptr);
   } else if (active) {
     hipLaunchKernelGGL((k_preprocess_jvp<true, false, true>), dim3(nb), dim3(256), 0, s, v, g, t, m2t, gb.clampw,
-                       gb.tiles, sb.trec, x, compact ? 1 : 0, -1, ids, na);
+                       gb.tiles, sb.trec, x, compact ? 1 : 0, -1, ids, na, clamp_list);
   } else {
     const int lead = g.P > 0 ? stage_lead(g) : -1;
     const size_t lds = lead >= 0 ? (size_t)256 * g.rest_stride * sizeof(float) : 0;
     if (g.raw)
       hipLaunchKernelGGL((k_preprocess_jvp<true, false>), dim3(nb), dim3(256), lds, s, v, g, t, m2t, gb.clampw, gb.tiles,
-                         sb.trec, x, compact ? 1 : 0, lead, nullptr, -1);
+                         sb.trec, x, compact ? 1 : 0, lead, nullptr, -1, nullptr);
     else
       hipLaunchKernelGGL((k_preprocess_jvp<false, false>), dim3(nb), dim3(256), lds, s, v, g, t, m2t, gb.clampw, gb.tiles,
-                         sb.trec, x, compact ? 1 : 0, lead, nullptr, -1);
+                         sb.trec, x, compact ? 1 : 0, lead, nullptr, -1, nullptr);
   }
   GSLM_LAUNCH_CHECK();
   return GSLM_OK;
diff --git a/gaussian-splatting-lm_amd/gslm/_lib.py b/gaussian-splatting-lm_amd/gslm/_lib.py
--- a/gaussian-splatting-lm_amd/gslm/_lib.py
+++ b/gaussian-splatting-lm_amd/gslm/_lib.py
@@ -60,6 +60,17 @@
         ("cg_ctl", ctypes.c_void_p),
         ("rest_basis", ctypes.c_void_p), ("rest_views", ctypes.c_int32), ("view_base", ctypes.c_int32),
     ]
+
+
+class GslmCgLean(ctypes.Structure):
+    _fields_ = [
+        ("beta_partials", ctypes.c_void_p), ("beta_np", ctypes.c_int32), ("dot_defer", ctypes.c_int32),
+        ("beta_store", ctypes.c_void_p), ("params", ctypes.c_void_p),
+    ]
+
+
+class GslmMatvecOptsLean(ctypes.Structure):
+    _fields_ = [("base", GslmMatvecOpts), ("lean", GslmCgLean)]
 
 
 class GslmViewWs(ctypes.Structure):
@@ -176,6 +187,22 @@
     "gslm_active_unpack": (ctypes.c_int, [ctypes.c_void_p, ctypes.c_void_p, ctypes.c_void_p, ctypes.c_int64,
                                           ctypes.c_int64, ctypes.POINTER(ctypes.c_int32), ctypes.c_int32,
                                           ctypes.c_int64, ctypes.c_void_p]),
+    "gslm_active_params_bytes": (ctypes.c_size_t, [ctypes.c_int64]),
+    "gslm_active_params": (ctypes.c_int, [ctypes.POINTER(GslmGaussians), ctypes.c_void_p, ctypes.c_int64,
+                                          ctypes.c_void_p, ctypes.c_int64, ctypes.c_void_p, ctypes.c_size_t,
+                                          ctypes.c_void_p, ctypes.c_void_p]),
+    "gslm_cg_start_active": (ctypes.c_int, [ctypes.c_void_p, ctypes.c_void_p, ctypes.c_int64, ctypes.c_int64,
+                                            ctypes.POINTER(ctypes.c_int32), ctypes.c_int32, ctypes.c_int64,
+                                            ctypes.c_int64, ctypes.c_void_p, ctypes.c_void_p, ctypes.c_void_p,
+                                            ctypes.c_void_p, ctypes.c_void_p, ctypes.c_void_p]),
+    "gslm_cg_update_lean": (ctypes.c_int, [ctypes.c_int64, ctypes.c_void_p, ctypes.c_void_p, ctypes.c_int32,
+                                           ctypes.c_void_p, ctypes.c_int32, ctypes.c_void_p, ctypes.c_void_p,
+                                           ctypes.c_void_p, ctypes.c_void_p, ctypes.c_void_p, ctypes.c_void_p]),
+    "gslm_cg_end_active": (ctypes.c_int, [ctypes.c_void_p, ctypes.c_void_p, ctypes.c_void_p, ctypes.c_void_p,
+                                          ctypes.c_int64, ctypes.c_void_p, ctypes.c_int64, ctypes.c_int64,
+                                          ctypes.POINTER(ctypes.c_int32), ctypes.c_int32, ctypes.c_int64,
+                                          ctypes.c_void_p, ctypes.c_void_p, ctypes.c_int32, ctypes.c_void_p,
+                                          ctypes.c_void_p]),
     "gslm_rest_basis": (ctypes.c_int, [ctypes.POINTER(GslmView), ctypes.c_int32, ctypes.POINTER(GslmGaussians),
                                        ctypes.c_void_p, ctypes.c_void_p]),
     "gslm_rest_coords": (ctypes.c_int, [ctypes.POINTER(GslmView), ctypes.c_int32, ctypes.POINTER(GslmGaussians),
diff --git a/gaussian-splatting-lm_amd/gslm/lm.py b/gaussian-splatting-lm_amd/gslm/lm.py
--- a/gaussian-splatting-lm_amd/gslm/lm.py
+++ b/gaussian-splatting-lm_amd/gslm/lm.py
@@ -13,6 +13,7 @@
 STAGE_OVERWRITE = 8
 MV_TAIL_CLEAN = 1
 MV_SH_REST_PROJECTED = 2
+MV_LEAN = 4
 
 DEFAULT_DAMP = {"xyz": 5e2, "features_dc": 5e-2, "features_rest": 5e-2, "scaling": 5e-2, "rotation": 5e-2,
                 "opacity": 5e-2, "exposure": 1e1}
@@ -27,6 +28,7 @@
         self.N = 0
         self.geom = self.binning = self.image = self.scratch = None
         self._active = None
+        self._params = None
         self.tail_clean = False
         self.epoch = 0
 
@@ -39,6 +41,7 @@
         self._tail_clean = bool(value)
         if not value:
             self._active = None
+            self._params = None
 
     def active_list(self, P, stream):
         if not self.tail_clean or self.N is None:
@@ -56,6 +59,20 @@
             self._active = (ids[:n], n)
             self.active_rows = rows[:n + 1]
         return self._active
+
+    def active_params(self, model, P, stream):
+        ids, na = self.active_list(P, stream)
+        leaves = (model._xyz, model._scaling, model._rotation, model._opacity)
+        key = tuple((t.data_ptr(), t._version) for t in leaves)
+        if self._params is None or self._params[0] != key:
+            dev = self.device
+            block = _lib.u8(lib.gslm_active_params_bytes(na), dev)
+            pos = torch.empty(max(P, 1), dtype=torch.int32, device=dev)
+            g = raw_gaussians(model)
+            check(lib.gslm_active_params(ctypes.byref(g), self.geom.data_ptr(), P, ids.data_ptr() if na else None, na,
+                                         block.data_ptr(), block.numel(), pos.data_ptr(), stream), "gslm_active_params")
+            self._params = (key, block, pos)
+        return self._params[1], self._params[2]
 
     def forward(self, g, stream, want_invdepth=True):
         P = g.P
@@ -290,7 +307,8 @@
                                  exposure_zero=exposure_zero, cg_ctl=cg_ctl)
         return fuse
 
-    def local_normal_matvec(self, v, y, damp=False, dot_out=None, pre=None, exposure_zero=False, cg_ctl=None):
+    def local_normal_matvec(self, v, y, damp=False, dot_out=None, pre=None, exposure_zero=False, cg_ctl=None,
+                            lean=None):
         g = raw_gaussians(self.model)
         vs = self.layout.grads_struct(v)
         ys = self.layout.grads_struct(y)
@@ -316,10 +334,13 @@
                 opts.dot_vy = dot_out
                 opts.dot_scratch = self.dot_scratch.data_ptr()
                 opts.dot_scratch_bytes = self.dot_scratch.numel() * 8
+            if lean is not None and lean.dot_defer:
+                opts.dot_scratch = self.dot_scratch.data_ptr()
+                opts.dot_scratch_bytes = self.dot_scratch.numel() * 8
             if self.ssim:
                 self._ssim_product(b, vr, g, vs, ys, opts)
                 continue
-            self._view_product(vr, g, vs, self.weights[b].data_ptr(), ys, opts, "gslm_matvec_view_ex")
+            self._view_product(vr, g, vs, self.weights[b].data_ptr(), ys, opts, "gslm_matvec_view_ex", lean=lean)
             vr.tail_clean = True
         if exposure_zero:
             pass
@@ -329,7 +350,13 @@
             y[e0:e1].zero_()
         return y
 
-    def _view_product(self, vr, g, vs, weight, ys, opts, what):
+    def _view_product(self, vr, g, vs, weight, ys, opts, what, lean=None):
+        if lean is not None:
+            ext = _lib.GslmMatvecOptsLean()
+            ctypes.memmove(ctypes.addressof(ext.base), ctypes.addressof(opts), ctypes.sizeof(opts))
+            ext.base.flags |= MV_LEAN
+            ext.lean = lean
+            opts = ext
         if self._active is not None:
             ids, na = self._active
             check(lib.gslm_matvec_view_active(ctypes.byref(vr.view), ctypes.byref(g), ctypes.byref(vs), weight,
@@ -788,9 +815,86 @@
     return act
 
 
+def _lean_applies(act, check_every, max_iter):
+    return (not check_every and max_iter >= 1 and not act.ssim and getattr(act, "allreduce_scalars", None) is None
+            and os.environ.get("GSLM_CG_LEAN", "1") != "0")
+
+
+def _cgls_lean(prob, act, g, max_iter, restart_iter):
+    full = act._full
+    vr = act.views[0]
+    ids, Pa = act._active
+    n = act.layout.numel
+    dev, st = act.device, act.stream
+    P = full.layout.P
+    lo = (3 * Pa // 4) * 4
+    na = n - lo
+    w, ng, tail = act._pack_args()
+    block, pos = vr.active_params(act.model, P, st)
+    sc = torch.zeros(16, dtype=torch.float64, device=dev)
+    ptr = lambda i: sc.data_ptr() + 8 * i
+    off = lambda t: t.data_ptr() + 4 * lo
+    GAM, GAMN, DEL = 0, 1, 2
+    NB = 1024
+    x, s, p, q = (torch.empty(n, dtype=torch.float32, device=dev) for _ in range(4))
+    part_g0 = torch.empty(NB, dtype=torch.float64, device=dev)
+    part_gn = torch.empty(NB, dtype=torch.float64, device=dev)
+    part_d = act.dot_scratch
+    npd = (Pa + 255) // 256
+    ids_ptr = ids.data_ptr() if Pa else None
+    ez = prob.exposure_is_zero(g)
+    check(lib.gslm_cg_start_active(g.data_ptr(), ids_ptr, Pa, P, w, ng, tail, lo, s.data_ptr(), p.data_ptr(),
+                                   q.data_ptr(), x.data_ptr(), part_g0.data_ptr(), st), "gslm_cg_start_active")
+    gam_part = part_g0.data_ptr()
+    gp = None
+    pend = pre = None
+    iter_total = 0
+    first = True
+    while iter_total < max_iter:
+        if not first:
+            check(lib.gslm_axpy_dev(na, pend[0], pend[1], 1.0, off(p), off(x), st), "gslm_axpy_dev")
+            pend = pre = None
+            if gp is None:
+                gp = act.pack(g)
+            act.matvec(x, q)
+            torch.sub(gp, q, out=s)
+            p.copy_(s)
+            act.dot(s[lo:], s[lo:], ptr(GAM))
+            gam_part = None
+        first = False
+        for _ in range(restart_iter):
+            lean = _lib.GslmCgLean()
+            lean.dot_defer = 1
+            lean.params = block.data_ptr()
+            fpre = None
+            if pre is not None:
+                fpre = pre + (x, pend[0], pend[1])
+                pend = None
+                lean.beta_partials, lean.beta_np, lean.beta_store = part_gn.data_ptr(), NB, pre[1]
+            act.local_normal_matvec(p, q, damp=True, pre=fpre, exposure_zero=ez, lean=lean)
+            check(lib.gslm_cg_update_lean(na, ptr(GAM), gam_part, NB if gam_part else 0, part_d.data_ptr(), npd,
+                                          ptr(DEL), off(p), off(q), off(s), part_gn.data_ptr(), st),
+                  "gslm_cg_update_lean")
+            gam_part = None
+            pend = (ptr(GAM), ptr(DEL))
+            pre = (s, ptr(GAMN), ptr(GAM))
+            GAM, GAMN = GAMN, GAM
+            iter_total += 1
+            if iter_total >= max_iter:
+                break
+    out = torch.empty(full.layout.numel, dtype=torch.float32, device=dev)
+    check(lib.gslm_cg_end_active(x.data_ptr(), p.data_ptr(), pend[0], pend[1], lo, pos.data_ptr(), Pa, P, w, ng, tail,
+                                 out.data_ptr(), part_gn.data_ptr(), NB, ptr(GAM), st), "gslm_cg_end_active")
+    act._full._lean_state = {"sc": sc, "gamma": GAM, "delta": DEL, "gamma_partials": part_gn,
+                             "delta_partials": part_d[:npd], "s": s, "p": p, "q": q, "lo": lo}
+    return out, {"iters": iter_total, "residuals": []}
+
+
 def cgls_fused(prob, g, max_iter=10, restart_iter=10, tol=1e-10, atol=0.0, check_every=True, verbose=False,
                callback=None, host_checks=None):
     act = _active_view_for(prob, g, callback)
+    if act is not None and _lean_applies(act, check_every, max_iter):
+        return _cgls_lean(prob, act, g, max_iter, restart_iter)
     if act is not None:
         gp = act.pack(g)
         if prob.exposure_is_zero(g):
diff --git a/include/gslm.h b/include/gslm.h
--- a/include/gslm.h
+++ b/include/gslm.h
@@ -184,6 +184,32 @@
 int gslm_active_unpack(const float* src, float* dst, const int32_t* active_ids, int64_t n_active, int64_t P,
                        const int32_t* widths, int32_t ngroups, int64_t tail_n, void* stream);
 
+typedef struct gslm_cg_lean {
+  const void* beta_partials;
+  int32_t beta_np;
+  int32_t dot_defer;
+  double* beta_store;
+  const void* params;
+} gslm_cg_lean;
+#define GSLM_MV_LEAN 4
+typedef struct gslm_matvec_opts_lean {
+  gslm_matvec_opts base;
+  gslm_cg_lean lean;
+} gslm_matvec_opts_lean;
+size_t gslm_active_params_bytes(int64_t n_active);
+int gslm_active_params(const gslm_gaussians* g, const void* geom, int64_t P, const int32_t* active_ids,
+                       int64_t n_active, void* block, size_t block_bytes, int32_t* pos_dev, void* stream);
+int gslm_cg_start_active(const float* g_full, const int32_t* active_ids, int64_t n_active, int64_t P,
+                         const int32_t* widths, int32_t ngroups, int64_t tail_n, int64_t lo, float* s, float* p,
+                         float* q, float* x, void* partials, void* stream);
+int gslm_cg_update_lean(int64_t n, double* gam_dev, const void* gam_partials, int32_t gam_np,
+                        const void* del_partials, int32_t del_np, double* del_dev, const float* p, const float* q,
+                        float* s, void* partials_out, void* stream);
+int gslm_cg_end_active(const float* x, const float* p, const double* num_dev, const double* den_dev, int64_t lo,
+                       const int32_t* pos_dev, int64_t n_active, int64_t P, const int32_t* widths, int32_t ngroups,
+                       int64_t tail_n, float* out_full, const void* fin_partials, int32_t fin_np, double* fin_dev,
+                       void* stream);
+
 int gslm_gather_screen(const gslm_view* views, int32_t nviews, const gslm_gaussians* g, const float* screen,
                        const gslm_grads* v, const gslm_grads* y, const gslm_matvec_opts* opts, void* stream);
 
```

After: 1794 view-matvec/s (one (J^T J + D) application per 1080p view, 1M Gaussians) (median of 6 runs). 1.02x the previous value.
